# mlee03/FRE-NCtools

Hardware: AMD Instinct MI355X
Metric: exchange-cells/s (higher is better)
Workload: dtype f64; 1 GPU; C384 cubed sphere (6 tiles) -> 1440x720 lat-lon, conservative_order2: exchange-grid search + centroid pass + CSR build per step; nxgrid=4160000, parallelism=1 latitude band(s) of the target, one per GPU, world_size=1

## Files before the change

### fre-nctools_amd/_lib.py

```python
import ctypes as C
import os

_HERE = os.path.dirname(os.path.abspath(__file__))
_LIB = None


class FregridHipError(RuntimeError):
    def __init__(self, code, msg):
        super().__init__(f"libfregrid_hip error {code}: {msg}")
        self.code = code


def lib_path():
    return os.environ.get("FREGRID_HIP_LIB") or os.path.join(_HERE, "libfregrid_hip.so")


EXPORTS = [
    "get_maxxgrid", "get_grid_area", "create_xgrid_2dx2d_order1", "create_xgrid_2dx2d_order2", "conserve_interp",
    "clip_2dx2d", "poly_area", "poly_ctrlon", "poly_ctrlat", "fix_lon", "pimod",
    "fg_clip_2dx2d_batch", "fg_poly_op_batch",
    "get_maxxgrid_", "get_grid_area_", "create_xgrid_2dx2d_order1_", "create_xgrid_2dx2d_order2_",
    "fg_last_error", "fg_device_count", "fg_plan_create", "fg_plan_create_dev", "fg_plan_create_empty",
    "fg_plan_destroy", "fg_plan_set_stream", "fg_pool_release", "fg_plan_nxgrid", "fg_plan_ncells_in",
    "fg_plan_cell_sums_dev", "fg_plan_copy_cell_sums", "fg_plan_accumulate_cell_sums", "fg_plan_accumulate_cell_sums_async", "fg_dev_gather_f64", "fg_dev_scatter_f64", "fg_plan_finalize", "fg_plan_get_xgrid", "fg_plan_get_polygons", "fg_plan_create_polylist", "fg_plan_get_cell_struct",
    "fg_plan_get_cell_area", "fg_plan_set_xgrid", "fg_plan_apply", "fg_plan_apply_interleaved", "fg_plan_apply_records", "fg_plan_apply_levels", "fg_plan_apply_records_levels", "fg_plan_levels_capacity", "fg_plan_apply_levels_ex", "fg_plan_apply_records_levels_ex", "fg_plan_levels_ex_capacity", "fg_plan_apply_ex", "fg_plan_mono_begin",
    "fg_plan_mono_minmax_dev", "fg_plan_mono_copy_minmax", "fg_plan_mono_end",
    "fg_plan_apply_levels_mono", "fg_plan_mono_levels_begin", "fg_plan_mono_levels_copy_minmax", "fg_plan_mono_levels_end",
    "fg_plan_apply_records_levels_mono", "fg_plan_mono_records_reset", "fg_plan_mono_records_begin", "fg_plan_mono_records_copy_minmax",
    "fg_plan_mono_records_end", "fg_c2l_records_levels_mono", "fg_sweep_run_levels_mono",
    "fg_plan_create_great_circle", "fg_plan_create_great_circle_dev", "fg_latlon2xyz", "create_xgrid_great_circle",
    "create_xgrid_great_circle_", "get_grid_great_circle_area", "get_grid_great_circle_area_", "clip_2dx2d_great_circle",
    "great_circle_area", "fg_gc_clip_batch", "conserve_interp_great_circle", "fg_sincos_batch",
    "create_xgrid_1dx2d_order1", "create_xgrid_1dx2d_order2", "create_xgrid_2dx1d_order1", "create_xgrid_2dx1d_order2",
    "create_xgrid_1dx2d_order1_", "create_xgrid_1dx2d_order2_", "create_xgrid_2dx1d_order1_", "create_xgrid_2dx1d_order2_",
    "clip", "box_ctrlat", "box_ctrlon", "get_grid_area_no_adjust", "get_grid_area_no_adjust_", "fg_plan_stream", "fg_plan_sync",
    "fg_c2l_create", "fg_c2l_destroy", "fg_c2l_ncells", "fg_c2l_halo_size", "fg_c2l_set_stream", "fg_c2l_sync",
    "fg_c2l_get_centres", "fg_c2l_fill_halo", "fg_c2l_gradient", "fg_c2l_gradient_records", "fg_c2l_records", "fg_c2l_records_levels", "fg_c2l_grid_info", "fg_find_contacts", "fg_halo_map",
    "fg_gnomonic_ed_grid", "fg_tripolar_corners", "fg_remap_write", "fg_remap_write_interp", "fg_remap_read_size", "fg_remap_read", "fg_remap_last_error",
    "fg_plan_trim", "fg_plan_ncells_out", "fg_plan_order", "fg_plan_device", "fg_dev_alloc", "fg_dev_free", "fg_dev_upload", "fg_dev_download",
    "fg_nc_open", "fg_nc_create", "fg_nc_def_dim", "fg_nc_def_var", "fg_nc_put_att_text", "fg_nc_put_att_double", "fg_nc_enddef",
    "fg_nc_inq_ndims", "fg_nc_inq_nvars", "fg_nc_inq_numrecs", "fg_nc_inq_dimid", "fg_nc_inq_dim", "fg_nc_inq_varid", "fg_nc_inq_var",
    "fg_nc_get_att_double", "fg_nc_get_att_text", "fg_nc_get_vara", "fg_nc_get_vara_double", "fg_nc_put_vara", "fg_nc_put_vara_double",
    "fg_nc_close", "fg_nc_last_error", "fg_dev_widen", "fg_dev_narrow", "fg_sweep_create", "fg_sweep_run", "fg_sweep_run_levels", "fg_sweep_run_levels_ex", "fg_sweep_destroy", "fg_host_alloc", "fg_host_free",
    "fg_plan_stats", "fg_set_search_mode", "fg_set_search_cull", "fg_set_search_finalize", "fg_set_search_async", "fg_set_search_rect", "fg_set_search_wide_cap", "fg_set_search_frame", "fg_set_apply_xcd", "fg_set_apply_vec", "fg_set_apply_ep", "fg_set_gc_split", "fg_set_profiling", "fg_plan_phase_ms", "fg_gnomonic_ed_corners", "fg_latlon_corners",
    "fg_bilin_create", "fg_bilin_create_from_weights", "fg_bilin_destroy", "fg_bilin_get_index_weight", "fg_bilin_npoints_fine",
    "fg_bilin_nlon_fine", "fg_bilin_nlat_fine", "fg_bilin_nlon", "fg_bilin_nlat", "fg_bilin_ncells", "fg_bilin_set_stream",
    "fg_bilin_sync", "fg_bilin_apply_scalar", "fg_bilin_apply_vector", "fg_bilin_remap_write", "fg_bilin_remap_read",
    "fg_unit_vect_latlon", "fg_bilin_fine_grid", "fg_bilin_ambiguous_ties",
    "fg_bilin_sweep_create", "fg_bilin_sweep_run_scalar", "fg_bilin_sweep_run_vector", "fg_bilin_sweep_destroy",
    "fg_extrap_create", "fg_extrap_destroy", "fg_extrap_set_stream", "fg_extrap_stream", "fg_extrap_run_dev", "fg_extrap_run",
    "fg_extrap_last_syncs", "fg_extrap_get_coef", "fg_extrap_coef_host", "fg_set_extrap_batch", "fg_set_extrap_coef",
    "fg_setup_vertical_interp", "fg_dev_vertical_interp",
    "fg_extrap_run_batch_dev", "fg_column_create", "fg_column_run", "fg_column_destroy", "fg_set_column_records",
    "fg_dev_latlon2xyz", "fg_plan_create_great_circle_lonlat", "fg_plan_create_great_circle_lonlat_dev",
    "fg_plan_create_polylist_gc",
    "fg_runoff_create", "fg_runoff_create_from_xgrid", "fg_runoff_destroy", "fg_runoff_nxgrid", "fg_runoff_get_xgrid",
    "fg_runoff_get_maps", "fg_runoff_get_xyz", "fg_runoff_search_stats", "fg_runoff_phase_ms", "fg_runoff_stream", "fg_runoff_apply", "fg_runoff_apply_dev",
    "fg_nearest_unmasked", "fg_set_runoff_prune", "fg_runoff_tile",
    "fg_rland_create", "fg_rland_destroy", "fg_rland_stream", "fg_rland_search", "fg_rland_search_sface", "fg_rland_stats",
    "fg_rland_phase_ms", "fg_set_rland_prune", "fg_rland_tile",
    "fg_river_create", "fg_river_destroy", "fg_river_stream", "fg_river_run", "fg_river_get", "fg_river_get_max_suba",
    "fg_river_stats", "fg_river_phase_ms", "fg_set_river_prune", "fg_river_qsort_index",
    "fg_topog_default_opts", "fg_topog_create", "fg_topog_destroy", "fg_topog_stream", "fg_topog_set_source", "fg_topog_get_source",
    "fg_topog_remap", "fg_topog_filter", "fg_topog_process", "fg_topog_run", "fg_topog_set_depth", "fg_topog_get", "fg_topog_stats",
    "fg_topog_phase_ms", "fg_plan_apply_frac_dev", "fg_set_topog_sweep",
    "fg_coupler_create", "fg_coupler_create_gc", "fg_coupler_destroy", "fg_coupler_stream", "fg_coupler_run", "fg_coupler_count", "fg_coupler_get",
    "fg_coupler_get_cells", "fg_coupler_write", "fg_coupler_write_xgrid", "fg_coupler_write_mask", "fg_coupler_stats", "fg_coupler_phase_ms",
]


class TopogOpts(C.Structure):
    _fields_ = [("scale_factor", C.c_double)] + \
        [(k, C.c_int) for k in ("tripolar_grid", "cyclic_x", "cyclic_y", "fill_first_row", "filter_topog", "num_filter_pass",
                                "smooth_topo_allow_deepening", "round_shallow", "fill_shallow", "deepen_shallow", "full_cell", "flat_bottom",
                                "adjust_topo", "fill_isolated_cells", "dont_change_landmask", "kmt_min")] + \
        [("min_thickness", C.c_double), ("open_very_this_cell", C.c_int), ("fraction_full_cell", C.c_double),
         ("use_great_circle_algorithm", C.c_int), ("on_grid", C.c_int)]


class FieldConv(C.Structure):
    _fields_ = [("scale", C.c_double), ("offset", C.c_double), ("missing", C.c_double)]


class ApplyOpts(C.Structure):
    _fields_ = [("has_missing", C.c_int), ("missing", C.c_double), ("weight", C.c_void_p),
                ("cell_methods_sum", C.c_int), ("field_area", C.c_void_p), ("area_missing", C.c_double),
                ("cell_area_in", C.c_void_p), ("cell_area_out", C.c_void_p), ("monotonic", C.c_int)]


def lib():
    global _LIB
    if _LIB is not None:
        return _LIB
    path = lib_path()
    if not os.path.exists(path):
        raise ImportError(
            f"{path} not found: build the HIP extension first (make -C fre-nctools_amd/csrc, or "
            "python -c 'import __graft_entry__ as g; g.build()').  There is no CPU fallback.")
    try:
        import torch
    except ImportError:
        pass
    L = C.CDLL(path)
    dp, ip, vp = C.POINTER(C.c_double), C.POINTER(C.c_int), C.c_void_p
    dpp = C.POINTER(dp)
    cip = C.POINTER(C.c_int)

    L.get_maxxgrid.restype = C.c_int
    L.get_grid_area.argtypes = [cip, cip, dp, dp, dp]
    L.get_grid_area.restype = None
    L.create_xgrid_2dx2d_order1.argtypes = [cip] * 4 + [dp] * 5 + [ip] * 4 + [dp]
    L.create_xgrid_2dx2d_order1.restype = C.c_int
    L.create_xgrid_2dx2d_order2.argtypes = [cip] * 4 + [dp] * 5 + [ip] * 4 + [dp] * 3
    L.create_xgrid_2dx2d_order2.restype = C.c_int
    L.conserve_interp.argtypes = [C.c_int] * 4 + [dp] * 7
    L.conserve_interp.restype = None

    L.clip_2dx2d.argtypes = [dp, dp, C.c_int, dp, dp, C.c_int, dp, dp]
    L.clip_2dx2d.restype = C.c_int
    L.poly_area.argtypes = [dp, dp, C.c_int]
    L.poly_area.restype = C.c_double
    L.poly_ctrlon.argtypes = [dp, dp, C.c_int, C.c_double]
    L.poly_ctrlon.restype = C.c_double
    L.poly_ctrlat.argtypes = [dp, dp, C.c_int]
    L.poly_ctrlat.restype = C.c_double
    L.fix_lon.argtypes = [dp, dp, C.c_int, C.c_double]
    L.fix_lon.restype = C.c_int
# ... 470 lines not shown
```

### fre-nctools_amd/conserve_interp.py

```python
import ctypes as C
from dataclasses import dataclass, field
from typing import List, Optional

import numpy as np

from . import _lib
from ._lib import lib, check

CONSERVE_ORDER1 = 1
CONSERVE_ORDER2 = 2
TARGET = 16
READ = 256
WRITE = 512
CHECK_CONSERVE = 1024
LEGACY_CLIP = 2048
GREAT_CIRCLE = 4096
MONOTONIC = 16384
CELL_METHODS_MEAN = 0
CELL_METHODS_SUM = 1
MAXVAL = 1.0e20


def _f64(a):
    return np.ascontiguousarray(a, dtype=np.float64)
# ... 111 lines not shown
                                                              (lon_out_t, lat_out_t), mean_dlat, mean_dlon, device, stream), C.byref(h)))
        return cls(h.value, order, device)

    @classmethod
    def create_great_circle(cls, grids_in, grid_out, masks=None, device=0):
        _lib.require_gpu()
        args, keep = _host_grid_args(grids_in, grid_out, masks)
        h = C.c_void_p()
        check(lib().fg_plan_create_great_circle(*args, device, C.byref(h)))
        return cls(h.value, 1, device, True)

    @classmethod
    def create_great_circle_dev(cls, nx_in, ny_in, xyz_in_t, nx_out, ny_out, xyz_out_t, mean_dlat=0.0, mean_dlon=0.0,
                                device=0, stream=None, masks_t=None):
        h = C.c_void_p()
        tables = [[t[k] for t in xyz_in_t] for k in range(3)]
        check(lib().fg_plan_create_great_circle_dev(*_dev_grid_args(nx_in, ny_in, tables, masks_t, nx_out, ny_out, [xyz_out_t[k] for k in range(3)],
                                                                    mean_dlat, mean_dlon, device, stream), C.byref(h)))
        return cls(h.value, 1, device, True)

    @classmethod
    def create_great_circle_lonlat(cls, grids_in, grid_out, masks=None, device=0):
        _lib.require_gpu()
        args, keep = _host_grid_args(grids_in, grid_out, masks)
        h = C.c_void_p()
        check(lib().fg_plan_create_great_circle_lonlat(*args, device, C.byref(h)))
        return cls(h.value, 1, device, True)

    @classmethod
    def create_great_circle_lonlat_dev(cls, nx_in, ny_in, lon_in_t, lat_in_t, nx_out, ny_out, lon_out_t, lat_out_t,
                                       mean_dlat=0.0, mean_dlon=0.0, device=0, stream=None, masks_t=None):
        h = C.c_void_p()
        check(lib().fg_plan_create_great_circle_lonlat_dev(*_dev_grid_args(nx_in, ny_in, (lon_in_t, lat_in_t), masks_t, nx_out, ny_out,
                                                                           (lon_out_t, lat_out_t), mean_dlat, mean_dlon, device, stream),
                                                           C.byref(h)))
        return cls(h.value, 1, device, True)

    @classmethod
    def create_empty(cls, order, nx_in, ny_in, nx_out, ny_out, device=0):
        _lib.require_gpu()
        nt = len(nx_in)
        h = C.c_void_p()
        check(lib().fg_plan_create_empty(order, nt, (C.c_int * nt)(*nx_in), (C.c_int * nt)(*ny_in),
                                         nx_out, ny_out, device, C.byref(h)))
        return cls(h.value, order, device)

    def destroy(self):
        if self._h is not None and self._h.value:
            lib().fg_plan_destroy(self._h)
        self._h = None

    def __del__(self):
        try:
            self.destroy()
        except Exception:
            pass

    @property
    def nxgrid(self):
        return int(lib().fg_plan_nxgrid(self._h))

    @property
    def ncells_in(self):
        return int(lib().fg_plan_ncells_in(self._h))

    def cell_sums_ptr(self):
        return lib().fg_plan_cell_sums_dev(self._h)

    def copy_cell_sums(self, dst_t):
        check(lib().fg_plan_copy_cell_sums(self._h, C.c_void_p(dst_t.data_ptr())))

    def accumulate_cell_sums(self, total_t, cells_t=None):
        args = (self._h, C.c_void_p(total_t.data_ptr()), C.c_void_p(cells_t.data_ptr()) if cells_t is not None else None,
                int(cells_t.numel()) if cells_t is not None else 0)
        if getattr(total_t, "is_cuda", False):
            cur = _torch().cuda.current_stream(total_t.device)
            if int(self.stream() or 0) == int(cur.cuda_stream):
                check(lib().fg_plan_accumulate_cell_sums_async(*args))
                return
            cur.synchronize()
        check(lib().fg_plan_accumulate_cell_sums(*args))

    def stats(self):
        s = (C.c_long * 11)()
        check(lib().fg_plan_stats(self._h, s, 11))
        names = ["pairs", "nonempty", "nxgrid", "borderline", "bins", "bin_entries", "deferred", "heavy", "below", "exact_mode", "rare"]
        return dict(zip(names, [int(v) for v in s]))

    PHASES = ["cell_struct", "bins", "candidates", "clip_quad", "clip_general", "compact", "rows",
              "search_total", "finalize", "apply"]

    def phase_ms(self):
        ms = (C.c_float * 10)()
        check(lib().fg_plan_phase_ms(self._h, ms, 10))
        return dict(zip(self.PHASES, [float(v) for v in ms]))

    def finalize(self, total_sums_ptr=None):
        check(lib().fg_plan_finalize(self._h, C.c_void_p(total_sums_ptr or 0)))

    def sync(self):
        check(lib().fg_plan_sync(self._h))

    def stream(self):
        return lib().fg_plan_stream(self._h)

    def set_stream(self, stream):
        check(lib().fg_plan_set_stream(self._h, C.c_void_p(int(stream))))

    def get_xgrid(self):
        n = self.nxgrid
        ints = {k: np.empty(n, dtype=np.int32) for k in ("t_in", "i_in", "j_in", "i_out", "j_out")}
        area = np.empty(n, dtype=np.float64)
        c1 = np.empty(n, dtype=np.float64) if self.order == 2 else None
        c2 = np.empty(n, dtype=np.float64) if self.order == 2 else None
        check(lib().fg_plan_get_xgrid(self._h, _ip(ints["t_in"]), _ip(ints["i_in"]), _ip(ints["j_in"]),
                                      _ip(ints["i_out"]), _ip(ints["j_out"]), _dp(area), _dp(c1), _dp(c2)))
        out = dict(ints)
        out["area"] = area
        if self.order == 2:
            out["c1"], out["c2"] = c1, c2
        return out

    def get_polygons(self, maxv=16):
        nx = self.nxgrid
        n = np.zeros(nx, dtype=np.int32)
        v = [np.zeros((nx, maxv)) for _ in range(3)]
        check(lib().fg_plan_get_polygons(self._h, maxv, _ip(n), _dp(v[0]), _dp(v[1]), _dp(v[2])))
        if self.great_circle:
            return {"n": n, "x": v[0], "y": v[1], "z": v[2]}
        return {"n": n, "lon": v[0], "lat": v[1]}

    @classmethod
    def create_polylist(cls, order, n, lon, lat, lon_avg, area_ref, grid_out, device=0):
        _lib.require_gpu()
        n = np.ascontiguousarray(n, dtype=np.int32)
        lon, lat = _f64(lon), _f64(lat)
        assert lon.shape == (n.size, 8) == lat.shape
        lon_avg, area_ref = _f64(lon_avg), _f64(area_ref)
        lo, la = _f64(grid_out.lonc).reshape(-1), _f64(grid_out.latc).reshape(-1)
        h = C.c_void_p()
        check(lib().fg_plan_create_polylist(order, n.size, _ip(n), _dp(lon), _dp(lat), _dp(lon_avg), _dp(area_ref), grid_out.nx, grid_out.ny,
                                            _dp(lo), _dp(la), device, C.byref(h)))
        return cls(h.value, order, device)

    @classmethod
    def create_polylist_gc(cls, n, x, y, z, area_ref, grid_out, device=0):
        _lib.require_gpu()
        n = np.ascontiguousarray(n, dtype=np.int32)
        x, y, z = (_f64(v).reshape(n.size, 8) for v in (x, y, z))
        area_ref = _f64(area_ref).reshape(n.size)
        lo, la = _f64(grid_out.lonc).reshape(-1), _f64(grid_out.latc).reshape(-1)
        h = C.c_void_p()
        check(lib().fg_plan_create_polylist_gc(n.size, _ip(n), _dp(x), _dp(y), _dp(z), _dp(area_ref), grid_out.nx, grid_out.ny,
                                               _dp(lo), _dp(la), device, C.byref(h)))
        return cls(h.value, 1, device, True)

    @classmethod
    def create_polylist_gc_dev(cls, n_t, x_t, y_t, z_t, area_ref_t, nx_out, ny_out, xyz_out_t, mean_dlat=0.0, mean_dlon=0.0,
                               device=0, stream=None):
        h = C.c_void_p()
        ptr = lambda t: C.c_void_p(t.data_ptr())
        check(lib().fg_plan_create_polylist_gc_dev(int(n_t.numel()), ptr(n_t), ptr(x_t), ptr(y_t), ptr(z_t), ptr(area_ref_t), nx_out, ny_out,
                                                   ptr(xyz_out_t[0]), ptr(xyz_out_t[1]), ptr(xyz_out_t[2]), mean_dlat, mean_dlon, device,
                                                   C.c_void_p(int(stream or 0)), 0 if stream is None else 1, C.byref(h)))
        return cls(h.value, 1, device, True)

    def get_cell_area(self, ncells_out):
        a_in = np.empty(self.ncells_in, dtype=np.float64)
        a_out = np.empty(ncells_out, dtype=np.float64)
# ... 438 lines not shown
```

### fre-nctools_amd/csrc/geom.hip.h

```cpp
#pragma once
#include <hip/hip_runtime.h>

#define G_PI      3.14159265358979323846
#define G_TPI     (2.0 * G_PI)
#define G_HPI     (0.5 * G_PI)
#define G_RADIUS  6371000.0
#define G_SMALL   1.e-10
#define G_POLETOL 1.e-6
#define G_MAXV    8
#define G_FIXCAP  12

#define G_ERRBIT_MAXV     1u
#define G_ERRBIT_PARALLEL 2u
#define G_ERRBIT_OVERFLOW 4u
#define G_ERRBIT_BADLAT   8u

#include "sincos_glibc.h"
__device__ __forceinline__ double d_sin_lat(double x) { return fgs_sin(x); }
__device__ __forceinline__ double d_cos_lat(double x) { return fgs_cos(x); }
__device__ __forceinline__ void d_sincos_lat(double x, double *s, double *c) { fgs_sincos(x, s, c); }

__device__ __forceinline__ bool d_is_pole(double lat) { return fabs(lat) >= G_HPI - G_POLETOL; }

__device__ inline int d_fix_lon(double *x, double *y, int n, double tlon)
// ... 1 lines not shown
  int nn = n;
  for (int i = 0; i < nn; i++) {
    if (!d_is_pole(y[i])) continue;
    int im = (i + nn - 1) % nn, ip = (i + 1) % nn;
    if (y[im] == y[i] && y[ip] == y[i]) {
      for (int k = i; k < nn - 1; k++) { x[k] = x[k + 1]; y[k] = y[k + 1]; }
      nn--; i--;
    } else if (y[im] != y[i] && y[ip] != y[i]) {
      if (nn + 1 > G_FIXCAP) return -1;
      for (int k = nn - 1; k >= i; k--) { x[k + 1] = x[k]; y[k + 1] = y[k]; }
      nn++; i++;
    }
  }
  for (int i = 0; i < nn; i++) {
    if (!d_is_pole(y[i])) continue;
    int im = (i + nn - 1) % nn, ip = (i + 1) % nn;
    if (y[im] != y[i]) x[i] = x[im];
    if (y[ip] != y[i]) x[i] = x[ip];
  }
  for (int i = 0; i < nn; i++) {
    int im = (i + nn - 1) % nn;
    double dx = x[i] - x[im];
    if (fabs(dx + G_PI) < G_SMALL || fabs(dx - G_PI) < G_SMALL) {
      if (nn + 2 > G_FIXCAP) return -1;
      double xa = x[im], xb = x[i];
      double ypole = G_HPI;
      if (y[i] < 0.0) ypole = -G_HPI;
      for (int k = nn - 1; k >= i; k--) { x[k + 2] = x[k]; y[k + 2] = y[k]; }
      x[i] = xa; y[i] = ypole;
      x[i + 1] = xb; y[i + 1] = ypole;
      nn += 2;
      break;
    }
  }
  if (!nn) return 0;
  double x_sum = x[0];
  for (int i = 1; i < nn; i++) {
    double dx = x[i] - x[i - 1];
    if (dx < -G_PI)     dx = dx + G_TPI;
    else if (dx > G_PI) dx = dx - G_TPI;
    x_sum += (x[i] = x[i - 1] + dx);
  }
  double d = (x_sum / nn) - tlon;
  if (d < -G_PI)     for (int i = 0; i < nn; i++) x[i] += G_TPI;
  else if (d > G_PI) for (int i = 0; i < nn; i++) x[i] -= G_TPI;
  return nn;
}

__device__ __forceinline__ int d_fix_lon_quad_fast(double *x, const double *y, double tlon)
{
  if (d_is_pole(y[0]) || d_is_pole(y[1]) || d_is_pole(y[2]) || d_is_pole(y[3])) return -1;
  {
    const double d0 = x[0] - x[3], d1 = x[1] - x[0], d2 = x[2] - x[1], d3 = x[3] - x[2];
    if (fabs(d0 + G_PI) < G_SMALL || fabs(d0 - G_PI) < G_SMALL || fabs(d1 + G_PI) < G_SMALL || fabs(d1 - G_PI) < G_SMALL ||
        fabs(d2 + G_PI) < G_SMALL || fabs(d2 - G_PI) < G_SMALL || fabs(d3 + G_PI) < G_SMALL || fabs(d3 - G_PI) < G_SMALL) return -1;
  }
  double x_sum = x[0];
#pragma unroll
  for (int i = 1; i < 4; i++) {
    double dx = x[i] - x[i - 1];
    if (dx < -G_PI)     dx = dx + G_TPI;
    else if (dx > G_PI) dx = dx - G_TPI;
    x_sum += (x[i] = x[i - 1] + dx);
  }
  const double d = (x_sum / 4) - tlon;
  if (d < -G_PI)     { x[0] += G_TPI; x[1] += G_TPI; x[2] += G_TPI; x[3] += G_TPI; }
  else if (d > G_PI) { x[0] -= G_TPI; x[1] -= G_TPI; x[2] -= G_TPI; x[3] -= G_TPI; }
  return 4;
}

__device__ __forceinline__ int d_inside_edge(double x0, double y0, double x1, double y1, double x, double y)
{
  double product = (x - x0) * (y1 - y0) + (x0 - x1) * (y - y0);
  return (product <= 1.e-12) ? 1 : 0;
}

__device__ __forceinline__ double d_pimod1(double v)
{
  if (v < -G_PI)     v += G_TPI;
  else if (v > G_PI) v -= G_TPI;
  return v;
}

template <int S>
__device__ inline double d_poly_area(const double *x, const double *y, int n)
{
  double area = 0.0;
  for (int i = 0; i < n; i++) {
    int ip = (i + 1 == n) ? 0 : i + 1;
    double dx = (x[ip * S] - x[i * S]);
    double lat1 = y[ip * S], lat2 = y[i * S];
    if (dx > G_PI)  dx = dx - 2.0 * G_PI;
    if (dx < -G_PI) dx = dx + 2.0 * G_PI;
    if (fabs(dx + G_PI) < G_SMALL || fabs(dx - G_PI) < G_SMALL) { area += G_PI; continue; }
    if (fabs(lat1 - lat2) < G_SMALL)
      area -= dx * d_sin_lat(0.5 * (lat1 + lat2));
    else {
      double dy = 0.5 * (lat1 - lat2);
      double dat = d_sin_lat(dy) / dy;
      area -= dx * d_sin_lat(0.5 * (lat1 + lat2)) * dat;
    }
  }
  if (area < 0) return -area * G_RADIUS * G_RADIUS;
  return area * G_RADIUS * G_RADIUS;
}

template <int S>
__device__ inline double d_poly_ctrlat(const double *x, const double *y, int n)
{
  double ctrlat = 0.0;
  for (int i = 0; i < n; i++) {
    int ip = (i + 1 == n) ? 0 : i + 1;
    double dx = (x[ip * S] - x[i * S]);
    double lat1 = y[ip * S], lat2 = y[i * S];
    double dy = lat2 - lat1;
    double hdy = dy * 0.5;
    double avg_y = (lat1 + lat2) * 0.5;
    if (dx == 0.0) continue;
    if (dx > G_PI)   dx = dx - 2.0 * G_PI;
    if (dx <= -G_PI) dx = dx + 2.0 * G_PI;
    const double cl1 = d_cos_lat(lat1);
    if (fabs(hdy) < G_SMALL)
      ctrlat -= dx * (2 * d_cos_lat(avg_y) + lat2 * d_sin_lat(avg_y) - cl1);
    else {
      double sa, ca;
      d_sincos_lat(avg_y, &sa, &ca);
      ctrlat -= dx * ((d_sin_lat(hdy) / hdy) * (2 * ca + lat2 * sa) - cl1);
    }
  }
  return (ctrlat * G_RADIUS * G_RADIUS);
}

template <int S>
__device__ inline double d_poly_ctrlon(const double *x, const double *y, int n, double clon)
{
  double ctrlon = 0.0;
  for (int i = 0; i < n; i++) {
    int ip = (i + 1 == n) ? 0 : i + 1;
    double phi1 = x[ip * S], phi2 = x[i * S];
    double lat1 = y[ip * S], lat2 = y[i * S];
    double dphi = phi1 - phi2;
    if (dphi == 0.0) continue;
    double sl1, cl1, sl2, cl2;
    d_sincos_lat(lat1, &sl1, &cl1);
    d_sincos_lat(lat2, &sl2, &cl2);
    double f1 = 0.5 * (cl1 * sl1 + lat1);
    double f2 = 0.5 * (cl2 * sl2 + lat2);
    if (dphi > G_PI)  dphi = dphi - 2.0 * G_PI;
    if (dphi < -G_PI) dphi = dphi + 2.0 * G_PI;
    double dphi1 = phi1 - clon;
    if (dphi1 > G_PI)  dphi1 -= 2.0 * G_PI;
    if (dphi1 < -G_PI) dphi1 += 2.0 * G_PI;
    double dphi2 = phi2 - clon;
    if (dphi2 > G_PI)  dphi2 -= 2.0 * G_PI;
    if (dphi2 < -G_PI) dphi2 += 2.0 * G_PI;
    if (fabs(dphi2 - dphi1) < G_PI) {
      ctrlon -= dphi * (dphi1 * f1 + dphi2 * f2) / 2.0;
    } else {
      double fac = (dphi1 > 0.0) ? G_PI : -G_PI;
      double fint = f1 + (f2 - f1) * (fac - dphi1) / fabs(dphi);
      ctrlon -= 0.5 * dphi1 * (dphi1 - fac) * f1 - 0.5 * dphi2 * (dphi2 + fac) * f2
                + 0.5 * fac * (dphi1 + dphi2) * fint;
    }
  }
  return (ctrlon * G_RADIUS * G_RADIUS);
}

__device__ __forceinline__ double d_dphi_clon(double phi, double clon)
{
  double d = phi - clon;
  if (d > G_PI)  d -= 2.0 * G_PI;
  if (d < -G_PI) d += 2.0 * G_PI;
  return d;
}

template <int S>
__device__ inline void d_poly_area_ctr(const double *x, const double *y, int n, double clon,
                                       double *area_out, double *ctrlon_out, double *ctrlat_out)
{
  double area = 0.0, ctrlat = 0.0, ctrlon = 0.0;
  double s0, c0, cp_first;
  fgs_trig<FGS_COS_F | FGS_SIN_N | FGS_COS_N>(y[0], nullptr, &cp_first, &s0, &c0);
  const double f_first = 0.5 * (c0 * s0 + y[0]), dphi_first = d_dphi_clon(x[0], clon);
  double f2 = f_first, dphi2 = dphi_first;
  for (int i = 0; i < n; i++) {
    const bool last = (i + 1 == n);
    int ip = last ? 0 : i + 1;
    double phi1 = x[ip * S], phi2 = x[i * S];
    double lat1 = y[ip * S], lat2 = y[i * S];
    double f1, dphi1, cp1;
    if (last) { f1 = f_first; dphi1 = dphi_first; cp1 = cp_first; }
    else {
      double s1, c1;
      fgs_trig<FGS_COS_F | FGS_SIN_N | FGS_COS_N>(lat1, nullptr, &cp1, &s1, &c1);
      f1 = 0.5 * (c1 * s1 + lat1);
      dphi1 = d_dphi_clon(phi1, clon);
    }
    double dx0 = phi1 - phi2;
    double avg_y = (lat1 + lat2) * 0.5;
    double savg, cavg, sa, ca;
    fgs_trig<FGS_ALL>(avg_y, &savg, &cavg, &sa, &ca);
    double dyh = 0.5 * (lat1 - lat2);
    bool flat = fabs(lat1 - lat2) < G_SMALL;
    double dat = flat ? 1.0 : d_sin_lat(dyh) / dyh;

    {
      double dx = dx0;
      if (dx > G_PI)  dx = dx - 2.0 * G_PI;
      if (dx < -G_PI) dx = dx + 2.0 * G_PI;
      if (fabs(dx + G_PI) < G_SMALL || fabs(dx - G_PI) < G_SMALL) area += G_PI;
      else area -= dx * savg * dat;
    }
    if (dx0 != 0.0) {
      double dx = dx0;
      if (dx > G_PI)   dx = dx - 2.0 * G_PI;
      if (dx <= -G_PI) dx = dx + 2.0 * G_PI;
      double hdy = (lat2 - lat1) * 0.5;
      const double t = (fabs(hdy) < G_SMALL) ? (2 * cavg + lat2 * savg) : dat * (2 * ca + lat2 * sa);
      ctrlat -= dx * (t - cp1);
    }
    if (dx0 != 0.0) {
      double dphi = dx0;
      if (dphi > G_PI)  dphi = dphi - 2.0 * G_PI;
      if (dphi < -G_PI) dphi = dphi + 2.0 * G_PI;
      if (fabs(dphi2 - dphi1) < G_PI) {
        ctrlon -= dphi * (dphi1 * f1 + dphi2 * f2) / 2.0;
      } else {
        double fac = (dphi1 > 0.0) ? G_PI : -G_PI;
        double fint = f1 + (f2 - f1) * (fac - dphi1) / fabs(dphi);
        ctrlon -= 0.5 * dphi1 * (dphi1 - fac) * f1 - 0.5 * dphi2 * (dphi2 + fac) * f2
                  + 0.5 * fac * (dphi1 + dphi2) * fint;
      }
    }
    f2 = f1; dphi2 = dphi1;
  }
  *area_out = (area < 0) ? -area * G_RADIUS * G_RADIUS : area * G_RADIUS * G_RADIUS;
  *ctrlat_out = ctrlat * G_RADIUS * G_RADIUS;
  *ctrlon_out = ctrlon * G_RADIUS * G_RADIUS;
}
```

### fre-nctools_amd/csrc/plan.hip

```cpp
#include <hip/hip_runtime.h>
#include <math.h>
#include <stdio.h>
#include <stdlib.h>
#include <string.h>
#include <algorithm>
#include <map>
#include <mutex>
#include <string>
#include <type_traits>
#include <vector>
#include "fg_host.h"
#include "plan_internal.h"
#include "xgrid_device.h"

static thread_local std::string g_err;
extern "C" const char *fg_last_error(void) { return g_err.c_str(); }
void fg_set_last_error(const char *msg) { g_err = msg ? msg : ""; }

extern "C" int fg_device_count(void)
{
  int n = 0;
  hipError_t e = hipGetDeviceCount(&n);
  if (e != hipSuccess) { fg_fail(FG_ERR_HIP, "hipGetDeviceCount: %s", hipGetErrorString(e)); return FG_ERR_HIP; }
  return n;
// ... 381 lines not shown
  c->lon_avg = pl->alloc<double>(n); c->area = pl->alloc<double>(n);
  c->nv = pl->alloc<int>(n);
  c->verts = pl->alloc<double>(n * (compact ? FG_VSTRIDE_QUAD : 16));
  if (compact) {
    const size_t cap = n / 16 + 64;
    c->vstride = FG_VSTRIDE_QUAD;
    c->wide_cap = (int)(g_wide_cap >= 0 ? std::min<size_t>((size_t)g_wide_cap, cap) : cap);
    c->wide = pl->alloc<double>(16 * (size_t)std::max(c->wide_cap, 1));
    if (!c->wide) return false;
  }
  return c->lat_min && c->lat_max && (compact || (c->lon_min && c->lon_max)) && c->lon_avg && c->area && c->nv && c->verts;
}

static int plan_base(int order, int ntiles_in, const int *nx_in, const int *ny_in, int nx_out, int ny_out,
                     int device, fg_plan **out)
{
  if (order != FG_CONSERVE_ORDER1 && order != FG_CONSERVE_ORDER2) return fg_fail(FG_ERR_ARG, "order must be 1 or 2");
  if (ntiles_in < 1 || !nx_in || !ny_in || nx_out < 1 || ny_out < 1 || !out) return fg_fail(FG_ERR_ARG, "bad grid sizes");
  if (int rc = fg_use_device("fg_plan", device)) return rc;
  fg_plan *pl = new fg_plan();
  pl->order = order; pl->device = device; pl->ntiles = ntiles_in;
  long off = 0, foff = 0;
  for (int m = 0; m < ntiles_in; m++) {
    if (nx_in[m] < 1 || ny_in[m] < 1) { delete pl; return fg_fail(FG_ERR_ARG, "bad source tile size"); }
    pl->nx_in.push_back(nx_in[m]); pl->ny_in.push_back(ny_in[m]); pl->cell_off.push_back((int)off);
    off += (long)nx_in[m] * ny_in[m];
    foff += (order == 2) ? (long)(nx_in[m] + 2) * (ny_in[m] + 2) : (long)nx_in[m] * ny_in[m];
  }
  if (off > 2000000000L || (long)nx_out * ny_out > 2000000000L) { delete pl; return fg_fail(FG_ERR_ARG, "grid too large for 32-bit cell indices"); }
  pl->nsrc = (int)off; pl->f_stride = foff;
  pl->nx_out = nx_out; pl->ny_out = ny_out; pl->ndst = nx_out * ny_out;
  pl->stream = g_handles.get_stream(device);
  if (!pl->stream) { delete pl; return fg_fail(FG_ERR_HIP, "hipStreamCreate failed"); }
  *out = pl;
  return 0;
}

extern "C" void fg_plan_destroy(fg_plan *pl)
{
  if (!pl) return;
  (void)hipSetDevice(pl->device);
  const bool drain = !pl->async || !pl->apply_pt.spans.empty();
  if (drain && (pl->stream || !pl->own_stream)) (void)hipStreamSynchronize(pl->stream);
  if (pl->stream_b) { if (drain) (void)hipStreamSynchronize(pl->stream_b); g_handles.put_stream(pl->device, pl->stream_b); }
  { float junk[PH_COUNT] = {0}; pl->apply_pt.collect(junk); }
  if (pl->async) g_pool.put(pl->owned, pl->stream, !pl->own_stream);
  else for (void *p : pl->owned) g_pool.put(p);
  if (pl->stream && pl->own_stream) g_handles.put_stream(pl->device, pl->stream);
  delete pl;
}

static void choose_bins(const fg_plan *pl, double mean_dlat, double mean_dlon, FgBins *b)
{
  const double PI = 3.14159265358979323846;
  double h = 1.25 * mean_dlat, w = 1.25 * mean_dlon;
  int nblat = (h > 0) ? (int)ceil(PI / h) : 1;
  int nblon = (w > 0) ? (int)ceil(2.0 * PI / w) : 1;
  if (nblat < 1) nblat = 1; if (nblat > 8192) nblat = 8192;
  if (nblon < 1) nblon = 1; if (nblon > 16384) nblon = 16384;
  (void)pl;
  b->nblat = nblat; b->nblon = nblon;
  b->inv_wlat = nblat / PI;
  b->inv_wlon = nblon / (2.0 * PI);
}

struct PinnedCounters { FgCounters c; unsigned long long mark; };
static FgCounters *pinned_counters()
{
  static thread_local PinnedCounters *h = nullptr;
  if (!h) { if (hipHostMalloc((void **)&h, sizeof(PinnedCounters), hipHostMallocCoherent) != hipSuccess) h = nullptr; else h->mark = 0; }
  return h ? &h->c : nullptr;
}

struct GcXyz { const double *x, *y, *z; };
struct BoxMode { FgBox box; const double *mask_quad; int no_adjust; };
struct SearchIn {
  const double *const *lon_in = nullptr, *const *lat_in = nullptr, *const *mask_in = nullptr;
  const double *lon_out = nullptr, *lat_out = nullptr;
  const GcXyz *gc_in = nullptr, *gc_out = nullptr;
  const BoxMode *boxm = nullptr;
  double mean_dlat = 0, mean_dlon = 0;
  int rect_hint = 1;
};
struct SearchOpts { bool exact, cull, finalize, rect, dst_frame; int gc_split; bool profile, async; };
__global__ __launch_bounds__(64) void k_counters_out(const unsigned *src, unsigned *dst, int nwords, unsigned long long *mark, unsigned long long seq)
{
  for (int k = threadIdx.x; k < nwords; k += 64) dst[k] = src[k];
  __threadfence_system();
  __syncthreads();
  if (threadIdx.x == 0) __hip_atomic_store(mark, seq, __ATOMIC_RELEASE, __HIP_MEMORY_SCOPE_SYSTEM);
}
static_assert(sizeof(FgCounters) % sizeof(unsigned) == 0 && offsetof(PinnedCounters, mark) == sizeof(FgCounters), "FgCounters travels as 32-bit words, the mark behind them");
static hipError_t wait_counters(const FgCounters *hc, unsigned long long seq, hipStream_t st)
{
  const unsigned long long *mark = &((const PinnedCounters *)hc)->mark;
  for (unsigned spin = 1;; spin++) {
    if (__atomic_load_n(mark, __ATOMIC_ACQUIRE) == seq) return hipSuccess;
    __builtin_ia32_pause();
    if (spin % 65536 == 0) {
      const hipError_t e = hipStreamQuery(st);
      if (e == hipErrorNotReady) (void)hipGetLastError();
      if (e == hipSuccess) return __atomic_load_n(mark, __ATOMIC_ACQUIRE) == seq ? hipSuccess : hipErrorUnknown;
      if (e != hipErrorNotReady) return e;
    }
  }
}
static const char *gc_clip_error(int code)
{
  switch (code) {
    case 3: return "firstIntersect is not in the grid1List";
    case 4: return " not found the next intersection ";
    case 5: return "not return back to the first intersection";
    case 6: return "After clipping, nintersect should be 0";
    case 7: return "inserAfter: point (x,y,z) is not found in the list";
    case 8: return "Error from create_xgrid.c: temp is not in list1";
    case 11: return "clip_2dx2d_great_circle: insertIntersect finds no node that is not an intersection (the reference's loop over "
                    "the list, mosaic_util.c:1352, does not end on this pair of cells)";
    default: return "clip_2dx2d_great_circle: more intersections than two convex polygons can have (the list capacity of the device "
                    "clip, not a check of the reference)";
  }
}

static int g_search_cull = 0;
static int g_search_finalize = 0;
static int g_gc_split = 1;
extern "C" void fg_set_gc_split(int on) { g_gc_split = on < 0 ? 0 : on; }
struct SearchCaps { unsigned long long entries; int regcap, nreg; bool rect; };
static int g_search_rect = 1;
extern "C" void fg_set_search_rect(int on) { g_search_rect = on ? 1 : 0; }
static int g_dst_frame = 0;
extern "C" void fg_set_search_frame(int coupler) { g_dst_frame = coupler ? 1 : 0; }
static thread_local int tl_dst_frame = -1;
static bool host_says_not_rect(int nx, int ny, const double *lon, const double *lat)
{
  const long nxp = nx + 1;
  const int js[3] = {ny, ny / 2, 1}, is[3] = {nx, nx / 2, 1};
  for (int a = 0; a < 3; a++)
    for (int b = 0; b < 3; b++) {
      const long e = (long)js[a] * nxp + is[b];
      if (memcmp(&lon[e], &lon[is[b]], sizeof(double)) || memcmp(&lat[e], &lat[(long)js[a] * nxp], sizeof(double))) return true;
    }
  return false;
}
#define FG_RETRY (-1000L)
struct Carve {
  size_t n = 0;
  size_t operator()(size_t size) { const size_t at = n; n += size; return at; }
};
struct SearchBlocks {
  fg_plan *pl;
  bool ok = true;
  std::vector<void *> scratch;
  template <typename T> T *keep(size_t count) { T *p = pl->alloc<T>(count); ok = ok && p; return p; }
  template <typename T> T *get(size_t count) { T *p = keep<T>(count); if (p) scratch.push_back(p); return p; }
  void release() { for (void *p : scratch) pl->release(p); scratch.clear(); }
};
static long plan_search_core(fg_plan *pl, const SearchIn &in, const SearchOpts &opt, SearchCaps *caps)
{
  const bool gc = in.gc_in != nullptr;
  const BoxMode *const boxm = in.boxm;
  pl->great_circle = gc;
  hipStream_t st = pl->stream;
  const int nsrc = pl->nsrc, ndst = pl->ndst, order = pl->order;
  FgCounters *hc = pinned_counters();
  if (!hc) return fg_fail(FG_ERR_HIP, "hipHostMalloc failed");

  std::vector<FgTile> &th = pl->tiles_host;
  th.resize(pl->ntiles + 1);
  for (int m = 0; m < pl->ntiles; m++) th[m] = FgTile{gc ? nullptr : in.lon_in[m], gc ? nullptr : in.lat_in[m], pl->nx_in[m], pl->ny_in[m], pl->cell_off[m]};
  th[pl->ntiles] = FgTile{in.lon_out, in.lat_out, pl->nx_out, pl->ny_out, 0};
  pl->tiles_dev = pl->alloc<FgTile>(pl->ntiles + 1);
  if (!pl->tiles_dev) return fg_fail(FG_ERR_HIP, "out of device memory");
  FgTileSet ts; ts.n = 0;
  const bool by_value = !gc && pl->ntiles + 1 <= FG_TILESET_MAX;
  if (by_value) { ts.n = pl->ntiles + 1; for (int m = 0; m <= pl->ntiles; m++) ts.t[m] = th[m]; }
  else FGCHK(hipMemcpyAsync(pl->tiles_dev, th.data(), sizeof(FgTile) * th.size(), hipMemcpyHostToDevice, st));
  FgTileXyz *gct_dev = nullptr;
  std::vector<FgTileXyz> gct;
  if (gc) {
    gct.resize(pl->ntiles + 1);
    for (int m = 0; m < pl->ntiles; m++) gct[m] = FgTileXyz{in.gc_in[m].x, in.gc_in[m].y, in.gc_in[m].z, pl->nx_in[m], pl->ny_in[m], pl->cell_off[m]};
    gct[pl->ntiles] = FgTileXyz{in.gc_out->x, in.gc_out->y, in.gc_out->z, pl->nx_out, pl->ny_out, 0};
    gct_dev = pl->alloc<FgTileXyz>(pl->ntiles + 1);
    if (!gct_dev) return fg_fail(FG_ERR_HIP, "out of device memory");
    FGCHK(hipMemcpyAsync(gct_dev, gct.data(), sizeof(FgTileXyz) * gct.size(), hipMemcpyHostToDevice, st));
  }

  bool any_mask = false;
  if (in.mask_in) for (int m = 0; m < pl->ntiles; m++) if (in.mask_in[m]) any_mask = true;
  if (any_mask) {
    pl->mask_dev = pl->alloc<double>(nsrc);
    if (!pl->mask_dev) return fg_fail(FG_ERR_HIP, "out of device memory");
    std::vector<double> ones;
    for (int m = 0; m < pl->ntiles; m++) {
      size_t nc = (size_t)pl->nx_in[m] * pl->ny_in[m];
      if (in.mask_in[m]) FGCHK(hipMemcpyAsync(pl->mask_dev + pl->cell_off[m], in.mask_in[m], nc * sizeof(double), hipMemcpyDeviceToDevice, st));
      else {
        ones.assign(nc, 1.0);
        FGCHK(hipMemcpyAsync(pl->mask_dev + pl->cell_off[m], ones.data(), nc * sizeof(double), hipMemcpyHostToDevice, st));
        FGCHK(hipStreamSynchronize(st));
      }
    }
  }

  const bool rect = caps->rect && !gc && !boxm;
  pl->rect = rect;
  const double dst_tlon = opt.dst_frame ? (double)NAN : 3.14159265358979323846;
  FgBins bins;
  choose_bins(pl, in.mean_dlat, in.mean_dlon, &bins);
  if (rect) { bins.nblat = 0; bins.nblon = 0; }
  const long nbins = (long)bins.nblat * bins.nblon;
  const long nslots = nbins + bins.nblat;
  const unsigned long long nentries = rect ? 0ull : caps->entries;
  const int ecap = (int)std::min<unsigned long long>(nentries, 2147483647ull);
  FgPairSpace ps{};
  ps.nreg = caps->nreg; ps.regcap = caps->regcap;
  const long npairs = fgd_pairs_total(ps);
  const long nx_alloc = npairs;

  if (!alloc_cells(pl, &pl->S, nsrc, rect && !pl->polys.npoly)) return fg_fail(FG_ERR_HIP, "out of device memory");
  SearchBlocks blk{pl};
  const bool gc_poly = gc && pl->gcpolys.npoly > 0;
  if (gc_poly) pl->gc_prec = blk.keep<double>((size_t)nsrc * FG_GC_PREC);
  struct { double *hdr, *lat_ax, *lon_ax, *col, *row, *col_min, *col_max, *col_avg; } rt{};
  if (rect) {
    pl->D = FgCells{};
    pl->D.area = blk.keep<double>(ndst);
    Carve at;
    const size_t o_hdr = at(8), o_lat = at((size_t)pl->ny_out + 1), o_lon = at((size_t)pl->nx_out + 1), o_col = at(8 * (size_t)pl->nx_out),
                 o_row = at(4 * ((size_t)pl->ny_out + 1)), o_cmin = at((size_t)pl->nx_out), o_cmax = at((size_t)pl->nx_out), o_cavg = at((size_t)pl->nx_out);
    double *rect_blk = blk.keep<double>(at.n);
    if (!blk.ok) return fg_fail(FG_ERR_HIP, "out of device memory");
    rt = {rect_blk + o_hdr, rect_blk + o_lat, rect_blk + o_lon, rect_blk + o_col, rect_blk + o_row, rect_blk + o_cmin, rect_blk + o_cmax, rect_blk + o_cavg};
  } else if (!alloc_cells(pl, &pl->D, ndst)) return fg_fail(FG_ERR_HIP, "out of device memory");
  const long t_bins = fgd_scan_tiles(nslots), t_rows = fgd_scan_tiles(ndst), t_comp = fgd_scan_tiles(nsrc);
  const size_t zreg = (size_t)FG_NREG * FG_FILL_STRIDE * sizeof(unsigned);
  Carve z;
  const size_t z_dc = z((sizeof(FgCounters) + 127) / 128 * 128), z_fill = z(zreg), z_tick = z(128);
  const size_t z_lb_bins = z(t_bins * sizeof(unsigned long long)), z_lb_rows = z(t_rows * sizeof(unsigned long long)),
               z_lb_comp = z(t_comp * sizeof(unsigned long long));
  const size_t z_bin_cnt = z((size_t)(nslots + 1) * sizeof(int)), z_bin_fill = z((size_t)(nslots + 1) * sizeof(int)),
               z_row_cnt = z((size_t)(ndst + 1) * sizeof(int)), z_nacc = z((size_t)(nsrc + 1) * sizeof(int));
  z((16 - (z.n - z_bin_cnt) % 16) % 16);
  const size_t z_gc_ntask = z(gc ? zreg : 0), z_gc_ocnt = z(gc ? zreg : 0);
  const size_t zbytes = z.n;
  char *zero_blk = blk.get<char>(zbytes);
  int *bin_start = blk.get<int>(nslots + 1);
  int *heavy_list = blk.get<int>(nsrc + 1);
  int *rare_list = blk.get<int>(rect ? nsrc + 1 : 1);
  int *big_list = blk.get<int>(nsrc + 1);
  int *pair_beg = blk.get<int>(nsrc + 1), *pair_cnt = blk.get<int>(nsrc + 1);
  FgBinEntry *bin_entries = blk.get<FgBinEntry>(nentries ? nentries : 1);
  ps.src = blk.get<int>(npairs + 1); ps.dst = blk.get<int>(npairs + 1);
  double *tmp_area = blk.get<double>(npairs + 1);
  double *tmp_clon = (order == 2) ? blk.get<double>(npairs + 1) : nullptr;
  double *tmp_clat = (order == 2) ? blk.get<double>(npairs + 1) : nullptr;
  int *defer_list = blk.get<int>(npairs + 1);
  const bool early_rows = !gc && !boxm;
  int *tmp_rowpos = early_rows ? blk.get<int>(npairs + 1) : nullptr;
  const bool gc_split = gc && !gc_poly && opt.gc_split && npairs < (1L << 28);
  const long tcap_want = (opt.gc_split == 2) ? npairs / 64 : 3 * npairs;
  const long tcap_reg = gc_split ? std::min<long>((tcap_want / FG_NREG + 255) / 256 * 256, 0x7ffffff0L / FG_NREG) : 0;
  const long tcap_all = tcap_reg * FG_NREG;
  unsigned *gc_meta = gc_split ? blk.get<unsigned>(npairs + 1) : nullptr;
  int *gc_tbase = gc_split ? blk.get<int>(npairs + 1) : nullptr;
  int *gc_order = gc_split ? blk.get<int>(npairs + 1) : nullptr;
  unsigned *gc_task = gc_split ? blk.get<unsigned>(tcap_all + 1) : nullptr;
  double *gc_res = gc_split ? blk.get<double>(2 * (size_t)tcap_all + 2) : nullptr;
  pl->xoff = blk.keep<int>(nsrc + 1);
  pl->x_src = blk.keep<int>(nx_alloc + 1); pl->x_dst = blk.keep<int>(nx_alloc + 1);
  pl->x_area = blk.keep<double>(nx_alloc + 1);
  if (order == 2) { pl->x_c1 = blk.keep<double>(nx_alloc + 1); pl->x_c2 = blk.keep<double>(nx_alloc + 1); pl->sums = blk.keep<double>(3 * (size_t)nsrc); }
  int *x_rowpos = blk.get<int>(nx_alloc + 1);
  pl->perm = blk.keep<FgRowEnt>(nx_alloc + 1);
  pl->csr.row_ptr = blk.keep<int>(ndst + 1);
  if (!pl->src_idx_f) pl->src_idx_f = blk.keep<int>(nsrc + 1);
  if (!blk.ok) return fg_fail(FG_ERR_HIP, "out of device memory");
  FgCounters *dc = (FgCounters *)(zero_blk + z_dc);
  ps.fill = (unsigned *)(zero_blk + z_fill);
  unsigned *tickets = (unsigned *)(zero_blk + z_tick);
  unsigned long long *lb_bins = (unsigned long long *)(zero_blk + z_lb_bins), *lb_rows = (unsigned long long *)(zero_blk + z_lb_rows),
                     *lb_comp = (unsigned long long *)(zero_blk + z_lb_comp);
  int *bin_cnt = (int *)(zero_blk + z_bin_cnt), *bin_fill = (int *)(zero_blk + z_bin_fill), *row_cnt = (int *)(zero_blk + z_row_cnt);
  int *nacc = (int *)(zero_blk + z_nacc);
  FGCHK(hipMemsetAsync(zero_blk, 0, zbytes, st));
  if (pl->ll_err) FGCHK(hipMemcpyAsync(&dc->err[2], pl->ll_err, sizeof(unsigned), hipMemcpyDeviceToDevice, st));

  PhaseTimer pt, ptot;
  pt.start(opt.profile, st); ptot.start(opt.profile, st);
  for (int k = 0; k < PH_COUNT; k++) pl->phase_ms[k] = 0;
  ptot.begin(PH_SEARCH_TOTAL);
  pt.begin(PH_CELL_STRUCT);
  if (gc) {
    fgd_gc_cell_struct(gct_dev + pl->ntiles, 1, ndst, pl->D, st, opt.cull ? dc->band_keys : nullptr, 1);
    if (gc_poly) fgd_gc_poly_records(pl->gcpolys, pl->S, pl->gc_prec, dc->err, st);
    else fgd_gc_cell_struct(gct_dev, pl->ntiles, nsrc, pl->S, st, opt.cull ? dc->band_keys : nullptr, 2);
    fgd_src_field_index(order, pl->tiles_dev, pl->ntiles, nsrc, pl->src_idx_f, st);
  } else if (rect) {
    FgRect &R = pl->rect_tab;
    R.hdr = rt.hdr; R.lat_ax = rt.lat_ax; R.lon_ax = rt.lon_ax; R.col = rt.col; R.row = rt.row;
    R.col_min = rt.col_min; R.col_max = rt.col_max; R.col_avg = rt.col_avg;
    R.bad = &dc->rect_bad; R.nx = pl->nx_out; R.ny = pl->ny_out;
    fgd_rect_tables(in.lon_out, in.lat_out, pl->nx_out, pl->ny_out, rt.hdr, rt.lat_ax, rt.lon_ax, rt.col, rt.col_min, rt.col_max, rt.col_avg, rt.row,
                    &dc->rect_bad, dc->err, st, dst_tlon);
    if (pl->polys.npoly) fgd_polylist_records(pl->polys, pl->S, pl->src_idx_f, pl->sums, &R, heavy_list, &dc->heavy_cnt, dc->err, st);
    fgd_cell_struct2r(ts, pl->tiles_dev, pl->tiles_dev, pl->ntiles, pl->polys.npoly ? 0 : nsrc, ndst, pl->S, pl->D.area, R, pl->mask_dev, order,
                      pl->src_idx_f, pl->sums, dc->err, st, dc->band_keys, (opt.cull && !pl->polys.npoly) ? 2 : 0, heavy_list, &dc->heavy_cnt,
                      rare_list, &dc->rare_cnt, ps, pair_beg, pair_cnt, big_list, &dc->big_cnt);
  } else if (opt.cull && !boxm && !pl->polys.npoly) {
    fgd_band_keys(in.lat_out, (long)(pl->nx_out + 1) * (pl->ny_out + 1), dc->band_keys, st);
    fgd_cell_struct2(ts, pl->tiles_dev, pl->tiles_dev, pl->ntiles, nsrc, ndst, pl->S, pl->D, bins, bin_cnt, order, pl->src_idx_f, pl->sums, dc->err, st, dc->band_keys, 2, dst_tlon);
  } else if (pl->polys.npoly) {
    fgd_polylist_records(pl->polys, pl->S, pl->src_idx_f, pl->sums, nullptr, nullptr, nullptr, dc->err, st);
    fgd_cell_struct2(ts, pl->tiles_dev, pl->tiles_dev, pl->ntiles, 0, ndst, pl->S, pl->D, bins, bin_cnt, order, pl->src_idx_f, pl->sums, dc->err, st, nullptr, 0, dst_tlon);
  } else
    fgd_cell_struct2(ts, pl->tiles_dev, pl->tiles_dev, pl->ntiles, nsrc, ndst, pl->S, pl->D, bins, bin_cnt, order, pl->src_idx_f, pl->sums, dc->err, st, nullptr, 0, dst_tlon);
  if (boxm) fgd_box_cell_boxes(boxm->box, pl->S, st);
  if (boxm && boxm->no_adjust) fgd_box_area_no_adjust(boxm->box, pl->S.area, st);
  pt.end();
  pl->have_geom = true;

  if (!rect) {
    pt.begin(PH_BINS);
    if (gc) fgd_bin_count(ndst, pl->D, bins, bin_cnt, st);
    fgd_exclusive_scan1(bin_cnt, nslots, bin_start, lb_bins, &tickets[0], &dc->total[0], dc->err, st);
    fgd_bin_fill(ndst, pl->D, bins, bin_fill, bin_start, bin_entries, ecap, nsrc, pl->S, pl->mask_dev, heavy_list, &dc->heavy_cnt, st);
    pt.end();
  }

  pt.begin(PH_CANDIDATES);
  if (rect)
    fgd_candidates_rect(nsrc, pl->S, pl->mask_dev, pl->rect_tab, ps, pair_beg, pair_cnt, heavy_list, &dc->heavy_cnt, big_list, &dc->big_cnt, st,
                        pl->polys.npoly ? 0 : 1,
                        rare_list, &dc->rare_cnt, dc->err, pl->polys.npoly ? nullptr : pl->sums);
  else
    fgd_candidates1(nsrc, pl->S, pl->mask_dev, bins, bin_start, bin_entries, ecap, ps, pair_beg, pair_cnt, heavy_list, &dc->heavy_cnt, big_list,
                    &dc->big_cnt, st);
  pt.end();
  hipEvent_t gc_e1 = nullptr, gc_e2 = nullptr;
  struct EvReturn {
    hipEvent_t &a, &b;
    ~EvReturn() { g_handles.put_sync_event(a); g_handles.put_sync_event(b); a = b = nullptr; }
  } ev_return{gc_e1, gc_e2};
  if (boxm) {
    pt.begin(PH_CLIP_GENERAL);
    fgd_clip_box(order, ps, boxm->box, th[pl->ntiles], pl->S, pl->D, pl->mask_dev, boxm->mask_quad, tmp_area, tmp_clon, tmp_clat, nacc, dc->stats, dc->err, st);
    pt.end();
  } else if (gc) {
    pt.begin(PH_CLIP_GENERAL);
    if (gc_poly)
      fgd_gc_clip_poly(ps, pl->S, pl->gc_prec, pl->D, tmp_area, nacc, dc->stats, dc->err, st);
    else if (gc_split) {
      if (!pl->stream_b) pl->stream_b = g_handles.get_stream(pl->device);
      gc_e1 = g_handles.get_sync_event(); gc_e2 = g_handles.get_sync_event();
      GcSplit g{gc_meta, gc_tbase, gc_task, gc_res, (unsigned)tcap_reg, (unsigned *)(zero_blk + z_gc_ntask), defer_list, &dc->defer_cnt,
                &dc->gc_list2_cnt, npairs, gc_order, (unsigned *)(zero_blk + z_gc_ocnt)};
      fgd_gc_clip_split(ps, pl->S, pl->mask_dev, pl->D, tmp_area, nacc, g, dc->stats, dc->err, st, pl->stream_b, gc_e1, gc_e2);
    } else
      fgd_gc_clip(ps, pl->S, pl->mask_dev, pl->D, tmp_area, nacc, defer_list, &dc->defer_cnt, dc->stats, dc->err, st);
    pt.end();
  } else {
    pt.begin(PH_CLIP_QUAD);
    fgd_clip_quad(order, ps, pl->S, pl->mask_dev, pl->D, tmp_area, tmp_clon, tmp_clat, nacc, defer_list, &dc->defer_cnt, dc->stats, dc->err, st,
                  rect ? &pl->rect_tab : nullptr, row_cnt, tmp_rowpos);
    pt.end();
    pt.begin(PH_CLIP_GENERAL);
    fgd_clip_general(order, ps, pl->S, pl->mask_dev, pl->D, tmp_area, tmp_clon, tmp_clat, nacc, defer_list, &dc->defer_cnt, dc->stats, dc->err, st,
                     rect ? &pl->rect_tab : nullptr, row_cnt, tmp_rowpos);
    pt.end();
  }
  pt.begin(PH_COMPACT);
  FgCompactIo io{};
  io.pair_beg = pair_beg; io.pair_cnt = pair_cnt;
  io.tmp_area = tmp_area; io.tmp_clon = tmp_clon; io.tmp_clat = tmp_clat;
  io.xoff = pl->xoff; io.x_src = pl->x_src; io.x_dst = pl->x_dst; io.x_area = pl->x_area; io.x_c1 = pl->x_c1; io.x_c2 = pl->x_c2;
  io.row_cnt = row_cnt; io.x_rowpos = x_rowpos; io.sums = pl->sums; io.big_list = big_list; io.big_cnt = &dc->big_cnt;
  io.tmp_rowpos = tmp_rowpos; io.row_ptr = pl->csr.row_ptr; io.perm = pl->perm;
  io.dc = dc; io.xcap = nx_alloc;
  if (early_rows)
    fgd_exclusive_scan2(nacc, nsrc, pl->xoff, lb_comp, &tickets[2], &dc->xtot, row_cnt, ndst, pl->csr.row_ptr, lb_rows, &tickets[1], &dc->rows_total, dc->err, st);
  else
    fgd_exclusive_scan1(nacc, nsrc, pl->xoff, lb_comp, &tickets[2], &dc->xtot, dc->err, st);
  fgd_compact(order, nsrc, ps, io, st);
  pt.end();
  if (!early_rows) {
    pt.begin(PH_ROWS);
    fgd_exclusive_scan1(row_cnt, ndst, pl->csr.row_ptr, lb_rows, &tickets[1], &dc->rows_total, dc->err, st);
    fgd_csr_fill_pos(nx_alloc, &dc->xtot, pl->x_src, pl->x_dst, pl->csr.row_ptr, x_rowpos, pl->perm, st);
    pt.end();
  }
  ptot.end();
  const bool fuse = opt.finalize && early_rows && !pl->polys.npoly;
  const bool stream_ordered = fuse && opt.async && !opt.profile;
  static thread_local unsigned long long rb_seq = 0;
  int *fused_tmp = nullptr;
  if (fuse) {
    if (order == 2) { pl->cen = pl->alloc<FgSrcRec>((size_t)nsrc + 1); pl->csr.e2 = pl->alloc<FgCsrEntry2>(nx_alloc + 1); }
    else pl->csr.e1 = pl->alloc<FgCsrEntry1>(nx_alloc + 1);
    if ((order == 2 && !pl->cen) || (!pl->csr.e1 && !pl->csr.e2)) return fg_fail(FG_ERR_HIP, "out of device memory");
    fused_tmp = pl->alloc<int>(3 * (size_t)(nx_alloc + 1));
  }
  if (stream_ordered) {
    unsigned *hc_dev = nullptr;
    if (hipHostGetDevicePointer((void **)&hc_dev, hc, 0) != hipSuccess || !hc_dev) return fg_fail(FG_ERR_HIP, "the counters' host block is not mapped");
    const int nwords = (int)(sizeof(FgCounters) / sizeof(unsigned));
    k_counters_out<<<1, 64, 0, st>>>((const unsigned *)dc, hc_dev, nwords, (unsigned long long *)(hc_dev + nwords), ++rb_seq);
    FGCHK(hipGetLastError());
  }
  if (fuse) {
    pt.begin(PH_FINALIZE);
    if (order == 2) fgd_centroids(nsrc, pl->S, pl->sums, pl->cen, st);
    fgd_csr_sortgather(order, ndst, (long)nsrc + ndst, pl->perm, pl->x_area, pl->x_c1, pl->x_c2, pl->src_idx_f,
                       order == 2 ? pl->cen : nullptr, pl->csr, st, fused_tmp, nx_alloc + 1);
    pt.end();
  }
  if (stream_ordered) {
    if (hipError_t e = hipGetLastError()) {
      (void)hipStreamSynchronize(st);
      return fg_fail(FG_ERR_HIP, "a launch of the search failed: %s", hipGetErrorString(e));
    }
    FGCHK(wait_counters(hc, rb_seq, st));
  } else {
    FGCHK(hipMemcpyAsync(hc, dc, sizeof(FgCounters), hipMemcpyDeviceToHost, st));
    FGCHK(hipStreamSynchronize(st));
  }
  pt.collect(pl->phase_ms); ptot.collect(pl->phase_ms);
  FGCHK(hipGetLastError());
  if (rect && hc->rect_bad) { caps->rect = false; return FG_RETRY; }
  if (rect && (hc->err[0] & G_ERRBIT_WIDECAP)) { caps->rect = false; return FG_RETRY; }
  if (hc->total[0] > nentries) { caps->entries = hc->total[0]; return FG_RETRY; }
  if (hc->total[0] > 2000000000ull) return fg_fail(FG_ERR_ARG, "bin table too large");
  if (hc->total[3] > (unsigned long long)ps.regcap) {
    if (hc->total[3] > 2000000000ull / (unsigned long long)ps.nreg) return fg_fail(FG_ERR_CAPACITY, "candidate pair list exceeds 2^31 entries");
    caps->regcap = (int)((hc->total[3] + FG_REG_ALIGN - 1) / FG_REG_ALIGN * FG_REG_ALIGN);
    return FG_RETRY;
  }
  if (hc->err[2] & G_ERRBIT_LL2X) return fg_fail(FG_ERR_ARG, "latlon2xyz: a grid corner is not finite, or its latitude (|lat| >= 2.4262) or longitude "
                                                          "(|lon| > 1024) lies outside the range of the device trig (radians expected)");
  if (hc->err[0] & 8u) return fg_fail(FG_ERR_ARG, "a grid corner latitude lies outside [-pi/2, pi/2] (radians expected)");
  if (hc->err[0] & 1u) return fg_fail(FG_ERR_MAXV, "create_xgrid.c: n2_in is greater than MAX_V");
  if (hc->err[0] & 2u) return fg_fail(FG_ERR_PARALLEL, "the line between <x1_0,y1_0> and  <x1_1,y1_1> should not parallel to "
                                                    "the line between <x2_0,y2_0> and  <x2_1,y2_1>");
  if (hc->err[0] & 4u) return fg_fail(FG_ERR_MAXV, "clipped polygon exceeds 16 vertices");
  if (hc->err[0] & G_ERRBIT_GC_CONVEX1) return fg_fail(FG_ERR_GEOM, "create_xgrid.c(clip_2dx2d_great_circle): grid box 1 is not convex");
  if (hc->err[0] & G_ERRBIT_GC_CONVEX2) return fg_fail(FG_ERR_GEOM, "create_xgrid.c(clip_2dx2d_great_circle): grid box 2 is not convex");
  if (hc->err[0] & G_ERRBIT_GC_POLYN) return fg_fail(FG_ERR_MAXV, "a polygon of the list has more than 8 vertices");
  if (hc->err[0] & G_ERRBIT_GC_CLIP) return fg_fail(FG_ERR_GEOM, "%s", gc_clip_error((int)hc->err[1]));
  if (hc->err[0] & G_ERRBIT_LOOKBACK) return fg_fail(FG_ERR_HIP, "single-pass scan: a tile waited too long for its predecessor");
  pl->nx = (long)hc->xtot;
  pl->stats[FG_STAT_PAIRS] = (long)hc->total[1];
  pl->stats[FG_STAT_NONEMPTY] = (long)(hc->xtot + hc->stats[FG_STAT_BELOW]);
  pl->stats[FG_STAT_NXGRID] = pl->nx;
  pl->stats[FG_STAT_BORDERLINE] = (long)hc->stats[FG_STAT_BORDERLINE];
  pl->stats[FG_STAT_BINS] = nbins;
  pl->stats[FG_STAT_BIN_ENTRIES] = (long)hc->total[0];
  pl->stats[FG_STAT_DEFERRED] = hc->defer_cnt + hc->gc_list2_cnt;
  pl->stats[FG_STAT_HEAVY] = hc->heavy_cnt;
  pl->stats[FG_STAT_RARE] = hc->rare_cnt;
  pl->stats[FG_STAT_BELOW] = (long)hc->stats[FG_STAT_BELOW];

  pl->rect_tab.bad = nullptr;
  if (stream_ordered) {
    blk.scratch.push_back(pl->perm); blk.scratch.push_back(fused_tmp);
    pl->release_on_stream(blk.scratch); blk.scratch.clear();
    pl->perm = nullptr; fused_tmp = nullptr;
  }
  blk.release();
  pl->rows_built = true;
  pl->searched = true;
  if (fuse) {
    pl->release(pl->perm); pl->perm = nullptr; pl->release(fused_tmp);
    if (!pl->red_partial) { pl->red_partial = pl->alloc<double>(1024); pl->red_result = pl->alloc<double>(260); }
    if (!pl->red_partial || !pl->red_result) return fg_fail(FG_ERR_HIP, "out of device memory");
    pl->dist_pending = (order == 2);
    pl->finalized = true; pl->fused = true;
  }
  return pl->nx;
}

static int g_search_exact = 0;
extern "C" void fg_set_search_mode(int exact) { g_search_exact = exact; }
extern "C" void fg_set_search_cull(int on) { g_search_cull = on ? 1 : 0; }
extern "C" void fg_set_search_finalize(int on) { g_search_finalize = on ? 1 : 0; }
static int g_search_async = 1;
extern "C" void fg_set_search_async(int on) { g_search_async = on ? 1 : 0; }
static long plan_search(fg_plan *pl, const SearchIn &in)
{
  static const bool env_exact = getenv("FREGRID_HIP_EXACT_SEARCH") && atoi(getenv("FREGRID_HIP_EXACT_SEARCH")) != 0;
  const SearchOpts opt{.exact = g_search_exact || env_exact, .cull = g_search_cull != 0, .finalize = g_search_finalize != 0,
                       .rect = g_search_rect != 0, .dst_frame = (tl_dst_frame >= 0 ? tl_dst_frame : g_dst_frame) != 0, .gc_split = g_gc_split, .profile = g_profiling != 0, .async = g_search_async != 0};
  const long big = std::max((long)pl->nsrc, (long)pl->ndst);
  if (big > (1L << 28)) return fg_fail(FG_ERR_CAPACITY, "grid of %ld cells: more than 2^28 cells per search are not supported", big);
  SearchCaps caps;
  caps.entries = opt.exact ? 0ull : 3ull * (unsigned long long)pl->ndst + 4096ull;
  const unsigned long long cap_pairs = std::min<unsigned long long>(8ull * (unsigned long long)big + 65536ull, 2000000000ull);
  caps.nreg = (int)std::max(1L, std::min((long)FG_NREG, ((long)pl->nsrc + 1023) / 1024));
  caps.regcap = opt.exact ? 0 : (int)((cap_pairs / caps.nreg + FG_REG_ALIGN - 1) / FG_REG_ALIGN * FG_REG_ALIGN);
  caps.rect = opt.rect && in.rect_hint && !in.gc_in && !in.boxm && pl->nx_out <= 8192 && pl->nx_out >= 2;
  const size_t keep = pl->owned.size();
  long rc = FG_RETRY;
  int attempts = 0;
  pl->async = opt.async;
  pl->on_stream = pl->async;
  for (; attempts < 4 && rc == FG_RETRY; attempts++) {
    if (attempts) {
      (void)hipStreamSynchronize(pl->stream);
      pl->drop_search(keep);
    }
    rc = plan_search_core(pl, in, opt, &caps);
  }
  pl->on_stream = false;
  if (rc == FG_RETRY) return fg_fail(FG_ERR_CAPACITY, "exchange-grid search: capacities did not settle");
  if (rc >= 0) pl->stats[FG_STAT_EXACT] = (attempts > 1) ? 1 : 0;
  pl->search_d2h = (long)attempts * (long)sizeof(FgCounters);
  return rc;
}

struct CornerSample {
  int nsamp = 0;
  std::vector<double> q;
  const double *corners(int a, int k) const { return &q[((size_t)a * nsamp + k) * 4]; }
};
static long sample_step(int nx, int ny, int *nsamp)
{
  const long ncell = (long)nx * ny;
  long step = ncell / 4096; if (step < 1) step = 1;
  *nsamp = (int)((ncell + step - 1) / step);
  return step;
}
__host__ __device__ static inline void sample_nodes(int nx, long step, int k, long n[4])
{
  const long c = (long)k * step;
  const int i = (int)(c % nx), j = (int)(c / nx);
  n[0] = (long)j * (nx + 1) + i; n[1] = n[0] + 1; n[3] = n[0] + nx + 1; n[2] = n[3] + 1;
}
static CornerSample sample_corners_host(int nx, int ny, int narr, const double *const *arr)
{
  CornerSample s;
  const long step = sample_step(nx, ny, &s.nsamp);
  s.q.resize((size_t)s.nsamp * narr * 4);
  for (int k = 0; k < s.nsamp; k++) {
    long n[4];
    sample_nodes(nx, step, k, n);
    for (int a = 0; a < narr; a++)
      for (int v = 0; v < 4; v++) s.q[((size_t)a * s.nsamp + k) * 4 + v] = arr[a][n[v]];
  }
  return s;
}
__global__ void k_sample_corners(int nx, long step, int nsamp, int narr, const double *a0, const double *a1, const double *a2, double *out)
{
  const int k = blockIdx.x * blockDim.x + threadIdx.x;
  if (k >= nsamp) return;
  long n[4];
  sample_nodes(nx, step, k, n);
  const double *arr[3] = {a0, a1, a2};
  for (int a = 0; a < narr; a++) {
    double *o = out + ((size_t)a * nsamp + k) * 4;
    o[0] = arr[a][n[0]]; o[1] = arr[a][n[1]]; o[2] = arr[a][n[2]]; o[3] = arr[a][n[3]];
  }
}
static int sample_corners_dev(fg_plan *pl, int nx, int ny, int narr, const double *d_a0, const double *d_a1, const double *d_a2, CornerSample *s)
{
  const long step = sample_step(nx, ny, &s->nsamp);
  s->q.resize((size_t)s->nsamp * narr * 4);
  double *d_q = (double *)g_pool.get(pl->device, s->q.size() * sizeof(double));
  if (!d_q) return fg_fail(FG_ERR_HIP, "out of device memory");
  k_sample_corners<<<(s->nsamp + 255) / 256, 256, 0, pl->stream>>>(nx, step, s->nsamp, narr, d_a0, d_a1, d_a2, d_q);
  hipError_t e = hipMemcpyAsync(s->q.data(), d_q, s->q.size() * sizeof(double), hipMemcpyDeviceToHost, pl->stream);
  if (e == hipSuccess) e = hipStreamSynchronize(pl->stream);
  g_pool.put(d_q);
  if (e != hipSuccess) return fg_fail(FG_ERR_HIP, "sampling the destination corners failed: %s", hipGetErrorString(e));
  return 0;
}
// ... 1773 lines not shown
static int plan_apply_frac(fg_plan *pl, const double *data, double *out)
{
  fgd_apply_frac(pl->ndst, pl->csr, data, out, pl->stream);
  FGCHK(hipStreamSynchronize(pl->stream));
  FGCHK(hipGetLastError());
  return 0;
}

extern "C" int fg_plan_apply_frac_dev(fg_plan *pl, const double *data_dev, double *out_dev)
{
  if (!pl || !data_dev || !out_dev) return fg_fail(FG_ERR_ARG, "fg_plan_apply_frac_dev: null argument");
  if (!pl->finalized || pl->order != 1) return fg_fail(FG_ERR_STATE, "fg_plan_apply_frac_dev: needs a finalized first-order plan");
  FGCHK(hipSetDevice(pl->device));
  return plan_apply_frac(pl, data_dev, out_dev);
}

static void b1_conserve_interp(bool great_circle, int nx_src, int ny_src, int nx_dst, int ny_dst, const double *x_src,
                               const double *y_src, const double *x_dst, const double *y_dst,
                               const double *mask_src, const double *data_src, double *data_dst)
{
  const double *lons[1] = {x_src}, *lats[1] = {y_src}, *masks[1] = {mask_src};
  fg_plan *pl = nullptr;
  long nx = great_circle ? fg_plan_create_great_circle(1, &nx_src, &ny_src, lons, lats, masks, nx_dst, ny_dst, x_dst, y_dst, fg_env_device(), &pl)
                         : fg_plan_create(FG_CONSERVE_ORDER1, 1, &nx_src, &ny_src, lons, lats, masks, nx_dst, ny_dst, x_dst, y_dst, fg_env_device(), &pl);
  if (nx < 0) fatal(fg_last_error());
  if (great_circle && nx > (long)MAXXGRID) fatal("nxgrid is greater than MAXXGRID, increase MAXXGRID");
  if (!great_circle && nx >= (long)MAXXGRID)
    fatal("The xgrid size is too large for resources.\n nxgrid is greater than MAXXGRID/nthreads; increase MAXXGRID,\n"
          " decrease nthreads, or increase number of MPI ranks.");
  if (fg_plan_finalize(pl, nullptr)) fatal(fg_last_error());
  size_t ns = (size_t)nx_src * ny_src, nd = (size_t)nx_dst * ny_dst;
  double *dsrc = nullptr, *ddst = nullptr;
  if (hipMalloc(&dsrc, ns * sizeof(double)) != hipSuccess || hipMalloc(&ddst, nd * sizeof(double)) != hipSuccess) fatal("hipMalloc failed");
  if (hipMemcpy(dsrc, data_src, ns * sizeof(double), hipMemcpyHostToDevice) != hipSuccess) fatal("hipMemcpy failed");
  if (plan_apply_frac(pl, dsrc, ddst)) fatal(fg_last_error());
  if (hipMemcpy(data_dst, ddst, nd * sizeof(double), hipMemcpyDeviceToHost) != hipSuccess) fatal("hipMemcpy failed");
  (void)hipFree(dsrc); (void)hipFree(ddst);
  fg_plan_destroy(pl);
}
extern "C" void conserve_interp(int nx_src, int ny_src, int nx_dst, int ny_dst, const double *x_src,
                                const double *y_src, const double *x_dst, const double *y_dst,
                                const double *mask_src, const double *data_src, double *data_dst)
{
  b1_conserve_interp(false, nx_src, ny_src, nx_dst, ny_dst, x_src, y_src, x_dst, y_dst, mask_src, data_src, data_dst);
}
extern "C" void conserve_interp_great_circle(int nx_src, int ny_src, int nx_dst, int ny_dst, const double *x_src,
                                             const double *y_src, const double *x_dst, const double *y_dst,
                                             const double *mask_src, const double *data_src, double *data_dst)
{
  b1_conserve_interp(true, nx_src, ny_src, nx_dst, ny_dst, x_src, y_src, x_dst, y_dst, mask_src, data_src, data_dst);
}

namespace {
struct DevBuf {
  void *p = nullptr;
  DevBuf(size_t n) { if (hipMalloc(&p, n ? n : 1) != hipSuccess) p = nullptr; }
  ~DevBuf() { if (p) (void)hipFree(p); }
};
}

extern "C" int fg_clip_2dx2d_batch(int npoly, const double *lon1, const double *lat1, const int *n1,
                                   const double *lon2, const double *lat2, const int *n2,
                                   double *lon_out, double *lat_out, int *n_out)
{
  if (npoly < 0 || !lon1 || !lat1 || !n1 || !lon2 || !lat2 || !n2 || !lon_out || !lat_out || !n_out) return fg_fail(FG_ERR_ARG, "null argument");
  if (npoly == 0) return 0;
  FGCHK(hipSetDevice(fg_env_device()));
  size_t nb = (size_t)npoly * FG_POLY_STRIDE * sizeof(double), ni = (size_t)npoly * sizeof(int);
  DevBuf a(nb), b(nb), c(nb), d(nb), xo(nb), yo(nb), m1(ni), m2(ni), mo(ni);
  if (!a.p || !b.p || !c.p || !d.p || !xo.p || !yo.p || !m1.p || !m2.p || !mo.p) return fg_fail(FG_ERR_HIP, "out of device memory");
  FGCHK(hipMemcpy(a.p, lon1, nb, hipMemcpyHostToDevice)); FGCHK(hipMemcpy(b.p, lat1, nb, hipMemcpyHostToDevice));
  FGCHK(hipMemcpy(c.p, lon2, nb, hipMemcpyHostToDevice)); FGCHK(hipMemcpy(d.p, lat2, nb, hipMemcpyHostToDevice));
  FGCHK(hipMemcpy(m1.p, n1, ni, hipMemcpyHostToDevice)); FGCHK(hipMemcpy(m2.p, n2, ni, hipMemcpyHostToDevice));
  fgd_poly_clip(npoly, (double *)a.p, (double *)b.p, (int *)m1.p, (double *)c.p, (double *)d.p, (int *)m2.p,
                (double *)xo.p, (double *)yo.p, (int *)mo.p, 0);
  FGCHK(hipDeviceSynchronize());
  FGCHK(hipMemcpy(lon_out, xo.p, nb, hipMemcpyDeviceToHost)); FGCHK(hipMemcpy(lat_out, yo.p, nb, hipMemcpyDeviceToHost));
  FGCHK(hipMemcpy(n_out, mo.p, ni, hipMemcpyDeviceToHost));
  return 0;
}

extern "C" int fg_poly_op_batch(int op, int npoly, double *lon, double *lat, int *n, const double *clon, double *result)
{
  if (op < 0 || op > 6 || npoly < 0 || !lon || !lat || !n) return fg_fail(FG_ERR_ARG, "bad argument");
  if ((op == 1 || op == 3 || op == 5) && !clon) return fg_fail(FG_ERR_ARG, "clon/tlon array required");
  if (op != 3 && !result) return fg_fail(FG_ERR_ARG, "result array required");
  if (npoly == 0) return 0;
  FGCHK(hipSetDevice(fg_env_device()));
  size_t nb = (size_t)npoly * FG_POLY_STRIDE * sizeof(double), ni = (size_t)npoly * sizeof(int), nd = (size_t)npoly * sizeof(double);
  DevBuf a(nb), b(nb), m(ni), cl(nd), r(nd);
  if (!a.p || !b.p || !m.p || !cl.p || !r.p) return fg_fail(FG_ERR_HIP, "out of device memory");
  FGCHK(hipMemcpy(a.p, lon, nb, hipMemcpyHostToDevice)); FGCHK(hipMemcpy(b.p, lat, nb, hipMemcpyHostToDevice));
  FGCHK(hipMemcpy(m.p, n, ni, hipMemcpyHostToDevice));
  if (clon) FGCHK(hipMemcpy(cl.p, clon, nd, hipMemcpyHostToDevice));
  fgd_poly_op(op, npoly, (double *)a.p, (double *)b.p, (int *)m.p, (double *)cl.p, (double *)r.p, 0);
  FGCHK(hipDeviceSynchronize());
  if (op == 3) {
    FGCHK(hipMemcpy(lon, a.p, nb, hipMemcpyDeviceToHost)); FGCHK(hipMemcpy(lat, b.p, nb, hipMemcpyDeviceToHost));
    FGCHK(hipMemcpy(n, m.p, ni, hipMemcpyDeviceToHost));
  } else FGCHK(hipMemcpy(result, r.p, nd, hipMemcpyDeviceToHost));
  return 0;
}

extern "C" int clip_2dx2d(const double lon1_in[], const double lat1_in[], int n1_in, const double lon2_in[],
                          const double lat2_in[], int n2_in, double lon_out[], double lat_out[])
{
  double a[FG_POLY_STRIDE] = {0}, b[FG_POLY_STRIDE] = {0}, c[FG_POLY_STRIDE] = {0}, d[FG_POLY_STRIDE] = {0};
  double xo[FG_POLY_STRIDE], yo[FG_POLY_STRIDE];
  if (n1_in > 12 || n2_in > 12 || n1_in < 1 || n2_in < 1) fatal("clip_2dx2d: this build supports 1..12 vertices per polygon");
  for (int k = 0; k < n1_in; k++) { a[k] = lon1_in[k]; b[k] = lat1_in[k]; }
  for (int k = 0; k < n2_in; k++) { c[k] = lon2_in[k]; d[k] = lat2_in[k]; }
  int no = 0;
  if (fg_clip_2dx2d_batch(1, a, b, &n1_in, c, d, &n2_in, xo, yo, &no)) fatal(fg_last_error());
  if (no == -1) fatal("the line between <x1_0,y1_0> and  <x1_1,y1_1> should not parallel to "
                      "the line between <x2_0,y2_0> and  <x2_1,y2_1>");
  if (no < 0) fatal("clip_2dx2d: clipped polygon exceeds 24 vertices");
  for (int k = 0; k < no; k++) { lon_out[k] = xo[k]; lat_out[k] = yo[k]; }
  return no;
}
static double poly_single(int op, const double x[], const double y[], int n, double clon)
{
  double a[FG_POLY_STRIDE] = {0}, b[FG_POLY_STRIDE] = {0}, r = 0;
  if (n < 1 || n > FG_POLY_STRIDE) fatal("polygon primitive: this build supports 1..24 vertices");
  for (int k = 0; k < n; k++) { a[k] = x[k]; b[k] = y[k]; }
  if (fg_poly_op_batch(op, 1, a, b, &n, &clon, &r)) fatal(fg_last_error());
  return r;
}
extern "C" double poly_area(const double x[], const double y[], int n) { return poly_single(0, x, y, n, 0.0); }
extern "C" double poly_ctrlon(const double x[], const double y[], int n, double clon) { return poly_single(1, x, y, n, clon); }
extern "C" double poly_ctrlat(const double x[], const double y[], int n) { return poly_single(2, x, y, n, 0.0); }
extern "C" int fix_lon(double x[], double y[], int n, double tlon)
{
  double a[FG_POLY_STRIDE] = {0}, b[FG_POLY_STRIDE] = {0};
  if (n < 1 || n > 8) fatal("fix_lon: this build supports 1..8 vertices");
  for (int k = 0; k < n; k++) { a[k] = x[k]; b[k] = y[k]; }
  if (fg_poly_op_batch(3, 1, a, b, &n, &tlon, nullptr)) fatal(fg_last_error());
  if (n < 0) fatal("fix_lon: vertex capacity exceeded");
  for (int k = 0; k < n; k++) { x[k] = a[k]; y[k] = b[k]; }
  return n;
}
extern "C" void pimod(double x[], int nn)
{
  const double PI = 3.14159265358979323846;
  for (int i = 0; i < nn; i++) { if (x[i] < -PI) x[i] += 2.0 * PI; else if (x[i] > PI) x[i] -= 2.0 * PI; }
}

extern "C" int fg_c2l_grid_info(int nx, int ny, const double *xt, const double *yt, const double *xc, const double *yc,
                                double *dx, double *dy, double *area, double *edge_w, double *edge_e, double *edge_s,
                                double *edge_n, double *en_n, double *en_e, double *vlon, double *vlat);
extern "C" int fg_halo_map(int ntiles, const int *nx, const int *ny, int ncontacts, const int *tile1, const int *tile2,
                           const int *istart1, const int *iend1, const int *jstart1, const int *jend1,
                           const int *istart2, const int *iend2, const int *jstart2, const int *jend2,
                           long *map_off, int *map);

struct fg_c2l {
  int device = 0, ntiles = 0;
  hipStream_t stream = nullptr;
  bool own_stream = true;
  long ncells = 0, F = 0;
  std::vector<int> nx, ny;
  std::vector<void *> owned;
  void *tiles_dev = nullptr;
  int *map_dev = nullptr;
  int *cell_of_dev = nullptr;
  double *geom_dev[11] = {nullptr};
  std::vector<double> lont_halo, latt_halo;
  template <typename T> T *alloc(size_t n) { void *p = g_pool.get(device, n * sizeof(T)); if (p) owned.push_back(p); return (T *)p; }
};
// ... 192 lines not shown
```

### fre-nctools_amd/csrc/poly_kernels.hip

```cpp
#include "xgrid_device.h"
#include "geom.hip.h"

#define PB_IN   12
#define PB_CAP  24

__device__ inline int d_clip_private(const double *lon1, const double *lat1, int n1,
                                     const double *lon2, const double *lat2, int n2,
                                     double *lon_out, double *lat_out)
{
  double cx[PB_CAP], cy[PB_CAP], ex[PB_IN], ey[PB_IN];
  bool wrap = false;
  for (int k = 0; k < n1; k++) { cx[k] = lon1[k]; cy[k] = lat1[k]; if (cx[k] > G_TPI || cx[k] < 0.0) wrap = true; }
  for (int k = 0; k < n2; k++) { ex[k] = lon2[k]; ey[k] = lat2[k]; }
  if (wrap) {
    for (int k = 0; k < n1; k++) cx[k] = d_pimod1(cx[k]);
    for (int k = 0; k < n2; k++) ex[k] = d_pimod1(ex[k]);
  }
  int n_cur = n1;
  double x2_0 = ex[n2 - 1], y2_0 = ey[n2 - 1];
  for (int e = 0; e < n2; e++) {
    double x2_1 = ex[e], y2_1 = ey[e];
    double x1_0 = cx[n_cur - 1], y1_0 = cy[n_cur - 1];
    int inside_last = d_inside_edge(x2_0, y2_0, x2_1, y2_1, x1_0, y1_0);
    int n_new = 0;
    for (int k = 0; k < n_cur; k++) {
      double x1_1 = cx[k], y1_1 = cy[k];
      int inside = d_inside_edge(x2_0, y2_0, x2_1, y2_1, x1_1, y1_1);
      if (inside != inside_last) {
        double dy1 = y1_1 - y1_0;
        double dy2 = y2_1 - y2_0;
        double dx1 = x1_1 - x1_0;
        double dx2 = x2_1 - x2_0;
        double ds1 = y1_0 * x1_1 - y1_1 * x1_0;
        double ds2 = y2_0 * x2_1 - y2_1 * x2_0;
        double determ = dy2 * dx1 - dy1 * dx2;
        if (fabs(determ) < 1.0e-30) return -1;
        if (n_new >= PB_CAP) return -2;
        lon_out[n_new] = (dx2 * ds1 - dx1 * ds2) / determ;
        lat_out[n_new++] = (dy2 * ds1 - dy1 * ds2) / determ;
      }
      if (inside) {
        if (n_new >= PB_CAP) return -2;
        lon_out[n_new] = x1_1; lat_out[n_new++] = y1_1;
      }
      x1_0 = x1_1; y1_0 = y1_1; inside_last = inside;
    }
    n_cur = n_new;
    if (!n_cur) return 0;
    for (int k = 0; k < n_cur; k++) { cx[k] = lon_out[k]; cy[k] = lat_out[k]; }
    x2_0 = x2_1; y2_0 = y2_1;
  }
  return n_cur;
}

__global__ __launch_bounds__(64) void k_poly_clip(int npoly, const double *lon1, const double *lat1, const int *n1,
                                                   const double *lon2, const double *lat2, const int *n2,
                                                   double *lon_out, double *lat_out, int *n_out)
{
  int p = blockIdx.x * blockDim.x + threadIdx.x;
  if (p >= npoly) return;
  double a[PB_IN], b[PB_IN], c[PB_IN], d[PB_IN], xo[PB_CAP], yo[PB_CAP];
  int m1 = n1[p], m2 = n2[p];
  if (m1 < 1 || m1 > PB_IN || m2 < 1 || m2 > PB_IN) { n_out[p] = -2; return; }
  for (int k = 0; k < m1; k++) { a[k] = lon1[(size_t)p * PB_CAP + k]; b[k] = lat1[(size_t)p * PB_CAP + k]; }
  for (int k = 0; k < m2; k++) { c[k] = lon2[(size_t)p * PB_CAP + k]; d[k] = lat2[(size_t)p * PB_CAP + k]; }
  int n = d_clip_private(a, b, m1, c, d, m2, xo, yo);
  n_out[p] = n;
  for (int k = 0; k < PB_CAP; k++) {
    lon_out[(size_t)p * PB_CAP + k] = (k < n) ? xo[k] : 0.0;
    lat_out[(size_t)p * PB_CAP + k] = (k < n) ? yo[k] : 0.0;
  }
}

__global__ __launch_bounds__(64) void k_poly_op(int op, int npoly, double *lon, double *lat, int *n, const double *clon,
                                                 double *result)
{
  int p = blockIdx.x * blockDim.x + threadIdx.x;
  if (p >= npoly) return;
  double x[PB_CAP], y[PB_CAP];
  int m = n[p];
  if (m < 1 || m > PB_CAP || (op == 3 && m > G_FIXCAP - 4)) { if (result) result[p] = 0; if (op == 3) n[p] = -2; return; }
  for (int k = 0; k < m; k++) { x[k] = lon[(size_t)p * PB_CAP + k]; y[k] = lat[(size_t)p * PB_CAP + k]; }
  if (op == 0) result[p] = d_poly_area<1>(x, y, m);
  else if (op == 1) result[p] = d_poly_ctrlon<1>(x, y, m, clon[p]);
  else if (op == 2) result[p] = d_poly_ctrlat<1>(x, y, m);
  else if (op >= 4) {
    double pa, pclon, pclat;
    d_poly_area_ctr<1>(x, y, m, op == 5 ? clon[p] : 0.0, &pa, &pclon, &pclat);
    result[p] = (op == 4) ? pa : (op == 5) ? pclon : pclat;
  } else {
    int mm = d_fix_lon(x, y, m, clon[p]);
    n[p] = mm;
    for (int k = 0; k < PB_CAP; k++) {
      lon[(size_t)p * PB_CAP + k] = (k < mm) ? x[k] : 0.0;
      lat[(size_t)p * PB_CAP + k] = (k < mm) ? y[k] : 0.0;
    }
  }
}

void fgd_poly_clip(int npoly, const double *lon1, const double *lat1, const int *n1, const double *lon2, const double *lat2,
                   const int *n2, double *lon_out, double *lat_out, int *n_out, hipStream_t st)
{
  if (npoly > 0) k_poly_clip<<<(npoly + 63) / 64, 64, 0, st>>>(npoly, lon1, lat1, n1, lon2, lat2, n2, lon_out, lat_out, n_out);
}
void fgd_poly_op(int op, int npoly, double *lon, double *lat, int *n, const double *clon, double *result, hipStream_t st)
{
  if (npoly > 0) k_poly_op<<<(npoly + 63) / 64, 64, 0, st>>>(op, npoly, lon, lat, n, clon, result);
}

__global__ __launch_bounds__(256) void k_sincos_probe(long n, const double *x, double *s, double *c)
{
  long i = (long)blockIdx.x * blockDim.x + threadIdx.x;
  if (i >= n) return;
  s[i] = d_sin_lat(x[i]); c[i] = d_cos_lat(x[i]);
}
void fgd_sincos_probe(long n, const double *x, double *s, double *c, hipStream_t st)
{
  if (n > 0) k_sincos_probe<<<(int)((n + 255) / 256), 256, 0, st>>>(n, x, s, c);
}

__global__ __launch_bounds__(64) void k_xgrid_polygons(long n, const int *x_src, const int *x_dst, FgCells S, FgCells D, FgRect R, int rect,
                                                        int maxv, int *n_out, double *lon_out, double *lat_out)
{
  const long k = (long)blockIdx.x * blockDim.x + threadIdx.x;
  if (k >= n) return;
  const int s = x_src[k], d = x_dst[k];
  double a[PB_IN], b[PB_IN], c[PB_IN], e[PB_IN], xo[PB_CAP], yo[PB_CAP];
  const int n1 = S.nv[s];
  int n2;
  const FgVerts sv = d_cell_verts(S, s, n1);
  for (int q = 0; q < 8; q++) { a[q] = q < n1 ? sv.x[q] : 0.0; b[q] = q < n1 ? sv.y[q] : 0.0; }
  double lon_out_avg;
  if (rect) {
    const int j = d / R.nx, i = d - j * R.nx;
    const double *cr = R.col + (size_t)i * RECT_COLW;
    const double ya = R.lat_ax[j], yb = R.lat_ax[j + 1];
    c[0] = cr[0]; c[1] = cr[1]; c[2] = cr[2]; c[3] = cr[3]; lon_out_avg = cr[6];
    e[0] = ya; e[1] = ya; e[2] = yb; e[3] = yb;
    n2 = 4;
  } else {
    const FgVerts dv = d_cell_verts(D, d, 0);
    for (int q = 0; q < 8; q++) { c[q] = dv.x[q]; e[q] = dv.y[q]; }
    lon_out_avg = D.lon_avg[d];
    n2 = D.nv[d];
  }
  const double dx = lon_out_avg - S.lon_avg[s];
  const double shift = (dx < -G_PI) ? G_TPI : ((dx > G_PI) ? -G_TPI : 0.0);
  if (shift != 0.0) for (int q = 0; q < n2; q++) c[q] += shift;
  int m = (n1 < 1 || n2 < 1) ? 0 : d_clip_private(a, b, n1, c, e, n2, xo, yo);
  n_out[k] = m;
  for (int q = 0; q < maxv; q++) {
    lon_out[(size_t)k * maxv + q] = (q < m && q < PB_CAP) ? xo[q] : 0.0;
    lat_out[(size_t)k * maxv + q] = (q < m && q < PB_CAP) ? yo[q] : 0.0;
  }
}
void fgd_xgrid_polygons(long n, const int *x_src, const int *x_dst, FgCells S, FgCells D, const FgRect *rect, int maxv,
                        int *n_out, double *lon_out, double *lat_out, hipStream_t st)
{
  if (n > 0) k_xgrid_polygons<<<(unsigned)((n + 63) / 64), 64, 0, st>>>(n, x_src, x_dst, S, D, rect ? *rect : FgRect{}, rect ? 1 : 0, maxv,
                                                                      n_out, lon_out, lat_out);
}
__global__ __launch_bounds__(256) void k_xgrid_gather_gc(long n, const int *x_src, const int *x_dst, FgCells S, FgCells D, double *a, double *b)
{
  const long t = (long)blockIdx.x * blockDim.x + threadIdx.x;
  if (t >= n * 12) return;
  const long k = t / 12; const int q = (int)(t - k * 12);
  a[t] = S.verts[(size_t)x_src[k] * 16 + q];
  b[t] = D.verts[(size_t)x_dst[k] * 16 + q];
}
// ... 19 lines not shown
```

### fre-nctools_amd/csrc/xgrid_device.h

```cpp
#pragma once
#include <hip/hip_runtime.h>

struct FgTile {
  const double *lon;
  const double *lat;
  int nx, ny;
  int cell_off;
};

struct FgTileXyz {
  const double *x, *y, *z;
  int nx, ny;
  int cell_off;
};
#define G_ERRBIT_GC_CONVEX1 16u
#define G_ERRBIT_GC_CONVEX2 32u
#define G_ERRBIT_GC_CLIP    64u

#define FG_VSTRIDE_QUAD 8
struct FgCells {
  double *lat_min, *lat_max, *lon_min, *lon_max, *lon_avg, *area;
  int *nv;
  double *verts;
  int vstride;
  int wide_cap;
  double *wide;
};
#ifdef __HIPCC__
struct FgVerts { const double *x, *y; };
__device__ __forceinline__ FgVerts d_cell_verts(const FgCells &c, int s, int n)
{
  if (c.vstride == FG_VSTRIDE_QUAD) {
    const double *v = c.verts + (size_t)s * FG_VSTRIDE_QUAD;
    if (n > 4) {
      const int k = *(const int *)v;
      const double *w = c.wide + (size_t)((unsigned)k < (unsigned)c.wide_cap ? k : 0) * 16;
      return FgVerts{w, w + 8};
    }
    return FgVerts{v, v + 4};
  }
  const double *v = c.verts + (size_t)s * 16;
  return FgVerts{v, v + 8};
}
__device__ __forceinline__ double *d_cell_quad(const FgCells &c, int s) { return c.verts + (size_t)s * FG_VSTRIDE_QUAD; }
#endif

struct FgBins {
  int nblat, nblon;
  double inv_wlat, inv_wlon;
};

struct FgBinEntry {
  double lat_min, lat_max, lon_min, lon_max, lon_avg;
  int d;
  int row0;
};

enum {
  FG_STAT_PAIRS = 0,
  FG_STAT_NONEMPTY = 1,
  FG_STAT_NXGRID = 2,
  FG_STAT_BORDERLINE = 3,
  FG_STAT_BINS = 4,
  FG_STAT_BIN_ENTRIES = 5,
  FG_STAT_DEFERRED = 6,
  FG_STAT_HEAVY = 7,
  FG_STAT_BELOW = 8,
  FG_STAT_EXACT = 9,
  FG_STAT_RARE = 10,
  FG_NSTATS = 11
};

#define FG_REG_ALIGN 512
#define FG_NREG 64
#define FG_FILL_STRIDE 32
struct FgPairSpace {
  int *src, *dst;
  unsigned *fill;
  int regcap, nreg;
};
#ifdef __HIPCC__
__device__ __forceinline__ bool d_pair_live(const FgPairSpace &ps, int p)
{
  const unsigned first = blockIdx.x * blockDim.x;
  const unsigned r = first / (unsigned)ps.regcap;
  const unsigned f = ps.fill[r * FG_FILL_STRIDE];
  return (unsigned)p - r * (unsigned)ps.regcap < (f < (unsigned)ps.regcap ? f : (unsigned)ps.regcap);
}
#endif
static inline long fgd_pairs_total(const FgPairSpace &ps) { return (long)ps.regcap * ps.nreg; }
#ifdef __HIPCC__
__device__ __forceinline__ unsigned long long d_ord_key(double v)
{
  const unsigned long long b = (unsigned long long)__double_as_longlong(v);
  return (b >> 63) ? ~b : (b | 0x8000000000000000ull);
}
__device__ __forceinline__ double d_ord_val(unsigned long long k)
{
  const unsigned long long b = (k >> 63) ? (k & 0x7fffffffffffffffull) : ~k;
  return __longlong_as_double((long long)b);
}
#endif

#define FG_TILESET_MAX 8
struct FgTileSet { FgTile t[FG_TILESET_MAX]; int n; };

struct FgLl2xGrid { const double *lon, *lat; double *x, *y, *z; long n; };
struct FgLl2xSet { FgLl2xGrid g[FG_TILESET_MAX]; int n; };
#define G_ERRBIT_LL2X 256u
#define G_ERRBIT_WIDECAP 512u
void fgd_latlon2xyz(const FgLl2xGrid *grids, int ngrids, unsigned *err, hipStream_t st);

struct FgCounters {
  unsigned long long total[4];
  unsigned long long rows_total;
  unsigned long long band_keys[2];
  unsigned long long xtot;
  unsigned err[4];
  int heavy_cnt;
  unsigned rect_bad;
  int defer_cnt, big_cnt;
  int gc_list2_cnt;
  int rare_cnt;
  unsigned long long stats[FG_NSTATS];
};
#define G_ERRBIT_LOOKBACK 128u

long fgd_scan_tiles(long n);
void fgd_exclusive_scan1(const int *in, long n, int *out, unsigned long long *status, unsigned *ticket,
                         unsigned long long *total_dev, unsigned *err, hipStream_t st);

void fgd_exclusive_scan2(const int *in_a, long n_a, int *out_a, unsigned long long *status_a, unsigned *ticket_a, unsigned long long *total_a,
                         const int *in_b, long n_b, int *out_b, unsigned long long *status_b, unsigned *ticket_b, unsigned long long *total_b,
                         unsigned *err, hipStream_t st);

void fgd_cell_struct2(const FgTileSet &ts, const FgTile *tiles_in, FgTile *tiles_out, int ntiles, int nsrc, int ndst, FgCells S, FgCells D,
                      FgBins b, int *slot_cnt, int order, int *src_idx_f, double *sums, unsigned *err, hipStream_t st,
                      unsigned long long *band_keys = nullptr, int cull = 0, double dst_tlon = 3.14159265358979323846);
void fgd_cell_struct(const FgTile *tiles_dev, int ntiles, int ncells, FgCells c, unsigned *err, hipStream_t st);
void fgd_band_keys(const double *lat, long n, unsigned long long *band_keys, hipStream_t st);
void fgd_bin_count(int ncells, FgCells c, FgBins b, int *slot_cnt, hipStream_t st);
void fgd_bin_fill(int ndst, FgCells D, FgBins b, int *slot_fill, const int *slot_start, FgBinEntry *entries, int cap,
                  int nsrc, FgCells S, const double *mask, int *heavy_list, int *heavy_cnt, hipStream_t st);
void fgd_candidates1(int nsrc, FgCells S, const double *mask, FgBins b, const int *slot_start, const FgBinEntry *entries, int ecap,
                     FgPairSpace ps, int *pair_beg, int *pair_cnt, const int *heavy_list, const int *heavy_cnt, int *big_list, int *big_cnt,
                     hipStream_t st);
#define RECT_COLW 8
struct FgRect {
  const double *lon_ax;
  const double *lat_ax;
  const double *col;
  const double *col_min, *col_max, *col_avg;
  const double *hdr;
  const double *row;
  const unsigned *bad;
  int nx, ny;
};
void fgd_rect_tables(const double *lon, const double *lat, int nx, int ny, double *hdr, double *lat_ax, double *lon_ax, double *col,
                     double *col_min, double *col_max, double *col_avg, double *row, unsigned *bad, unsigned *err, hipStream_t st,
                     double dst_tlon = 3.14159265358979323846);
void fgd_cell_struct2r(const FgTileSet &ts, const FgTile *tiles_in, FgTile *tiles_out, int ntiles, int nsrc, int ndst, FgCells S, double *area_out,
                       FgRect R, const double *mask, int order, int *src_idx_f, double *sums, unsigned *err, hipStream_t st,
                       unsigned long long *band_keys, int cull, int *heavy_list, int *heavy_cnt, int *rare_list, int *rare_cnt, FgPairSpace ps,
                       int *pair_beg, int *pair_cnt, int *big_list, int *big_cnt);
void fgd_rect_materialize(int ndst, FgRect R, FgCells D, hipStream_t st);
void fgd_quad_materialize(int nsrc, FgCells S, double *lon_min, double *lon_max, double *verts, hipStream_t st);
struct FgPolyList { const int *n; const double *lon, *lat; const double *lon_avg, *area; int npoly; };
void fgd_polylist_records(FgPolyList P, FgCells S, int *src_idx_f, double *sums, const FgRect *rect, int *heavy_list, int *heavy_cnt,
                          unsigned *err, hipStream_t st);
void fgd_candidates_rect(int nsrc, FgCells S, const double *mask, FgRect R, FgPairSpace ps, int *pair_beg, int *pair_cnt,
                         const int *heavy_list, const int *heavy_cnt, int *big_list, int *big_cnt, hipStream_t st, int listed_only,
                         const int *rare_list = nullptr, const int *rare_cnt = nullptr, unsigned *err = nullptr,
                         double *sums = nullptr);
void fgd_clip_general(int order, FgPairSpace ps, FgCells S, const double *mask, FgCells D,
              double *tmp_area, double *tmp_clon, double *tmp_clat, int *nacc, int *defer_list, int *defer_cnt,
              unsigned long long *stats, unsigned *err, hipStream_t st, const FgRect *rect = nullptr, int *row_cnt = nullptr,
              int *tmp_rowpos = nullptr);
void fgd_clip_quad(int order, FgPairSpace ps, FgCells S, const double *mask, FgCells D,
              double *tmp_area, double *tmp_clon, double *tmp_clat, int *nacc, int *defer_list, int *defer_cnt,
              unsigned long long *stats, unsigned *err, hipStream_t st, const FgRect *rect = nullptr, int *row_cnt = nullptr,
              int *tmp_rowpos = nullptr);
struct alignas(8) FgRowEnt { int n, s; };
struct alignas(16) FgSrcRec { double cen_lon, cen_lat; };
struct FgCompactIo {
  const int *pair_beg, *pair_cnt;
  const double *tmp_area, *tmp_clon, *tmp_clat;
  const int *xoff;
  int *x_src, *x_dst;
  double *x_area, *x_c1, *x_c2;
  int *row_cnt, *x_rowpos;
  const int *tmp_rowpos;
  const int *row_ptr; FgRowEnt *perm;
  double *sums;
  const int *big_list;
  const int *big_cnt;
  FgCounters *dc;
  long xcap;
};
void fgd_compact(int order, int nsrc, FgPairSpace ps, const FgCompactIo &io, hipStream_t st);
void fgd_centroids(int nsrc, FgCells S, const double *sums, FgSrcRec *cen, hipStream_t st);
void fgd_distances(long nx, const int *x_src, const double *x_area, const FgSrcRec *cen, double *x_c1, double *x_c2, hipStream_t st);

struct FgCsrEntry1 { int idx_f; int pad; double area; };
struct FgCsrEntry2 { int idx_f; int idx_g; double area, di, dj; };
struct FgCsr {
  int *row_ptr;
  FgCsrEntry1 *e1;
  FgCsrEntry2 *e2;
};
void fgd_csr_count(long nx, const int *x_dst, int *row_cnt, hipStream_t st);
void fgd_csr_fill(long nx, const int *x_src, const int *x_dst, const int *row_ptr, int *row_fill, FgRowEnt *perm, hipStream_t st);
void fgd_csr_fill_pos(long nx_cap, const unsigned long long *nx_dev, const int *x_src, const int *x_dst, const int *row_ptr, const int *x_rowpos,
                      FgRowEnt *perm, hipStream_t st);
void fgd_csr_sortgather(int order, int ndst, long nx, const FgRowEnt *perm, const double *x_area, const double *x_c1, const double *x_c2,
                        const int *src_idx_f, const FgSrcRec *cen, FgCsr csr, hipStream_t st, int *tmp = nullptr, long ntmp = 0,
                        int long_rows = 0);
void fgd_src_field_index(int order, const FgTile *tiles_dev, int ntiles, int nsrc, int *src_idx_f, hipStream_t st);
void fgd_apply1(int order, int ndst, FgCsr csr, const double *f, const double *gx, const double *gy, const int *gmask,
                int has_missing, double missing, double *out, double *row_sum, hipStream_t st, long nx = -1);
void fgd_apply_il(int order, int nb, int ndst, FgCsr csr, const double *f, const double *gx, const double *gy, double missing,
                  double *out, double *row_sum, long out_ld, int nb_valid, hipStream_t st, long nx = -1);
void fgd_interleave(int nb_pad, long n, const double *in, long ld, int nb_valid, double *out, hipStream_t st);
void fgd_apply_il_merged(int nb, int ndst, long nx, FgCsr csr, const double *rec, double missing, double *out, double *row_sum, long out_ld,
                         int nb_valid, hipStream_t st);
void fgd_merge3(int nb_pad, long n, const int *src_idx_f, const double *f, long ld_f, const double *gx, const double *gy, long ld_g,
                int nb_valid, double *out, hipStream_t st);
void fgd_interleave3(int nb_pad, int narr, const double *const *in, const long *ld, const long *n, double *const *out, int nb_valid,
                     hipStream_t st);
void fgd_deinterleave(int nb_pad, long n, const double *in, long ld, int nb_valid, double *out, hipStream_t st);
#define FG_LEVELS_CAP 256
void fgd_apply_levels8(int order, int ndst, long nx, FgCsr csr, const double *rec, const unsigned char *gbits, double missing, double *out,
                       double *row_sum, long ld, int nb_valid, hipStream_t st);
void fgd_gmask_bits(long n, const int *gmask, long ld, int nb, unsigned char *bits, hipStream_t st);
void fgd_apply_frac(int ndst, FgCsr csr, const double *data, double *out, hipStream_t st);
void fgd_reduce_sum(const double *v, long n, double *partial, double *result, hipStream_t st);
void fgd_xgrid_indices(long nx, const int *x_src, const int *x_dst, const FgTile *tiles_dev, int ntiles, int nx_out,
                       int *t_in, int *i_in, int *j_in, int *i_out, int *j_out, hipStream_t st);

struct FgApplyEx {
  const double *weight;
  const double *cell_area;
  const double *field_area;
  const double *cell_area_out;
  const int *gmask;
  const double *xdata;
  double area_missing, missing;
  int has_missing, sum;
};
#define FG_XERR_AREA_MISSING 1
#define FG_XERR_ABOVE 2
#define FG_XERR_BELOW 4
void fgd_apply_ex(int order, int ndst, FgCsr csr, const double *f, const double *gx, const double *gy, FgApplyEx o,
                  double *out, double *row_sum, int *err, hipStream_t st, long nx = -1);
#define FG_LEVELS_EX_CAP 256
#define FG_LEVELS_EX_CAP_Z 128
void fgd_apply_levels8x(int order, int ndst, long nx, FgCsr csr, const double *rec, const unsigned char *gbits, FgApplyEx o, const double *fa8,
                        double *out, double *row_sum, long ld, int nb_valid, int *err, hipStream_t st);
void fgd_mono_bounds(const FgTile *tiles_dev, int ntiles, int nsrc, const int *src_idx_f, const double *f, double missing,
                     double *fbmax, double *fbmin, double *fmax, double *fmin, hipStream_t st);
void fgd_mono_xdata(long nx, FgCsr csr, const double *f, const double *gx, const double *gy, const int *gmask, double missing,
                    double *xdata, double *fmax, double *fmin, hipStream_t st);
void fgd_mono_limit(long nx, FgCsr csr, const double *f, double missing, const double *fbmax, const double *fbmin,
                    const double *fmax, const double *fmin, double *xdata, int *err, hipStream_t st);
#define FG_LEVELS_MONO_CAP 128
// ... 80 lines not shown
```

### fre-nctools_amd/csrc/xgrid_kernels.hip

```cpp
#include <algorithm>
#include "xgrid_device.h"
#ifndef FG_EXP
#define FG_EXP 0
#endif
static __shared__ double fgs_lds_tab[112 * 4];
#define FGS_TAB(k, j) fgs_lds_tab[(k) * 4 + (j)]
#include "geom.hip.h"
__device__ __forceinline__ void d_load_trig_table()
{
  for (int i = threadIdx.x; i < 112 * 4; i += blockDim.x) fgs_lds_tab[i] = FG_SINCOS_TAB[i >> 2][i & 3];
  __syncthreads();
}

#define SCAN_THREADS 256
#define SCAN_ITEMS   8
#define SCAN_CHUNK   (SCAN_THREADS * SCAN_ITEMS)
#define LB_AGG   (1ull << 62)
#define LB_INC   (2ull << 62)
#define LB_MASK  ((1ull << 62) - 1ull)
#define LB_SPIN_LIMIT (1u << 22)

__device__ __forceinline__ unsigned wave_incl_scan(unsigned v, int lane)
{
#pragma unroll
// ... 1212 lines not shown
    int i = 0; bool pass = false;
    if (k < nwc) { i = d_rect_col(q, k); pass = d_rect_col_pass(R, i, lon_in_min, lon_in_max, lon_in_avg); }
    const unsigned long long m = __ballot(pass);
    const int at = cbase + __popcll(m & ((1ull << lane) - 1ull));
    if (pass)
      for (int jr = 0; jr < nr; jr++) {
        const long kk = (long)jr * nc + at;
        if (kk < n_ok) { ps.src[wbase + kk] = s; ps.dst[wbase + kk] = (q.j0 + jr) * R.nx + i; }
      }
    cbase += __popcll(m);
  }
  if (lane == 0) { pair_beg[s] = wbase; pair_cnt[s] = n_ok; if (n_ok > CP_SMALL) big_list[atomicAdd(big_cnt, 1)] = s; }
  if (zero_sums && n_ok == 0 && lane < 3) zero_sums[(size_t)lane * nsrc + s] = 0.0;
}

#define RARE_BLOCKS 64
template <bool FINISH>
__global__ __launch_bounds__(64) void k_candidates_rect(int nsrc, int H, FgCells S, const double *mask, FgRect R, FgPairSpace ps,
                                                         int *pair_beg, int *pair_cnt, const int *heavy_list, const int *heavy_cnt,
                                                         int *big_list, int *big_cnt, const int *rare_list, const int *rare_cnt, unsigned *err,
                                                         double *sums )
{
  const int lane = threadIdx.x;
  __shared__ unsigned wl[64 * RECT_WL_WORDS];
  if (FINISH && (int)blockIdx.x < RARE_BLOCKS) d_load_trig_table();
  const unsigned bad = *R.bad;
  const int nrare = FINISH ? *rare_cnt : 0;
  if (bad) return;
  const int hb = FINISH ? (int)blockIdx.x - RARE_BLOCKS : (int)blockIdx.x;
  if (hb >= 0 && hb < H) {
    const int nheavy = *heavy_cnt;
    for (int h = hb; h < nheavy; h += H) {
      const int s = heavy_list[h];
      double xmin, xmax;
      if constexpr (FINISH) {
        const double *q = d_cell_quad(S, s);
        const int n = S.nv[s];
        double x[G_MAXV];
#pragma unroll
        for (int k = 0; k < G_MAXV; k++) x[k] = k < 4 ? q[k] : 0.0;
        if (n > 4) {
          const FgVerts v = d_cell_verts(S, s, n);
#pragma unroll
          for (int k = 0; k < G_MAXV; k++) x[k] = v.x[k];
        }
        xmin = x[0]; xmax = x[0];
#pragma unroll
        for (int k = 1; k < G_MAXV; k++) if (k < n) { if (x[k] < xmin) xmin = x[k]; if (x[k] > xmax) xmax = x[k]; }
      } else { xmin = S.lon_min[s]; xmax = S.lon_max[s]; }
      d_rect_cell_candidates(R, ps, s, lane, S.lat_min[s], S.lat_max[s], xmin, xmax, S.lon_avg[s], pair_beg, pair_cnt, big_list, big_cnt,
                             FINISH ? sums : nullptr, nsrc);
    }
    return;
  }
  if constexpr (FINISH) {
    for (int h = blockIdx.x; h < nrare; h += RARE_BLOCKS) {
      const int s = rare_list[h];
      const double mk = mask ? mask[s] : 1.0;
      double b[5] = {0, 0, 0, 0, 0};
      const int nv = d_finish_rare_cell(S, err, s, h, lane, b);
      if (!(nv > 0 && mk > 0.5)) {
        if (sums && lane < 3) sums[(size_t)lane * nsrc + s] = 0.0;
        continue;
      }
      if (d_rect_heavy(R, b[0], b[1], b[2], b[3])) d_rect_cell_candidates(R, ps, s, lane, b[0], b[1], b[2], b[3], b[4], pair_beg, pair_cnt, big_list, big_cnt, sums, nsrc);
      else {
        int npair = 0;
        (void)d_rect_wave_candidates<true>(R, ps, lane == 0, s, nsrc, (unsigned)(s >> 6), b[0], b[1], b[2], b[3], b[4], pair_beg, pair_cnt, big_list, big_cnt, wl, &npair);
        npair = __shfl(npair, 0);
        if (sums && npair == 0 && lane < 3) sums[(size_t)lane * nsrc + s] = 0.0;
      }
    }
  } else {
    const int bR = (int)blockIdx.x - H;
    const int s = bR * 64 + lane;
    const bool active = s < nsrc && d_src_active(S, mask, s);
    double b[5] = {0, 0, 0, 0, 0};
    if (active) { b[0] = S.lat_min[s]; b[1] = S.lat_max[s]; b[2] = S.lon_min[s]; b[3] = S.lon_max[s]; b[4] = S.lon_avg[s]; }
    (void)d_rect_wave_candidates(R, ps, active, s, nsrc, (unsigned)bR, b[0], b[1], b[2], b[3], b[4], pair_beg, pair_cnt, big_list, big_cnt, wl);
  }
}

struct ClipOut { double area, clon, clat; };

template <int ORDER, int S>
__device__ __forceinline__ void d_finish_pair(const double *px, const double *py, int n_out, double maskv,
                                              double area_in, double area_out, double lon_in_avg,
                                              ClipOut *o, unsigned long long *stats)
{
  double pa, clon = 0, clat = 0;
  if (ORDER == 2) d_poly_area_ctr<S>(px, py, n_out, lon_in_avg, &pa, &clon, &clat);
  else pa = d_poly_area<S>(px, py, n_out);
  double xarea = pa * maskv;
  double min_area = (area_in < area_out) ? area_in : area_out;
  double ratio = xarea / min_area;
  if (fabs(ratio - 1.e-6) < 1.e-15) atomicAdd(&stats[FG_STAT_BORDERLINE], 1ull);
  if (ratio > 1.e-6) { o->area = xarea; o->clon = clon; o->clat = clat; }
  else o->area = -2.0;
}

#ifndef CLIP_THREADS
#define CLIP_THREADS 256
#endif
#ifndef CLIP_SLOTS
#define CLIP_SLOTS 8
#endif
#ifndef CLIP_WAVES
#define CLIP_WAVES 4
#endif
#ifndef CLIP_PAD_LDS
#define CLIP_PAD_LDS 0
#endif

template <bool RECT, int T, bool QSRC = false>
__device__ __forceinline__ int d_clip_quad_sh(double2 (*sh_poly)[T], const int tid, const int s, const int d,
                                              const FgCells &S, const FgCells &D, const FgRect &R, unsigned *err)
{
  constexpr int NV1 = RECT ? CLIP_SLOTS : 4;
  double x1[NV1], y1[NV1], x2[4], y2[4];
  double lon_out_avg;
  int n1 = S.nv[s], n2 = RECT ? 4 : D.nv[d];
  double lon_in_avg = S.lon_avg[s];
  if constexpr (QSRC) {
    const double *sq = d_cell_quad(S, s);
#pragma unroll
    for (int k = 0; k < NV1; k++) { x1[k] = k < 4 ? sq[k] : 0.0; y1[k] = k < 4 ? sq[4 + k] : 0.0; }
  } else {
    const FgVerts sv = d_cell_verts(S, s, 0);
#pragma unroll
    for (int k = 0; k < NV1; k++) { x1[k] = sv.x[k]; y1[k] = sv.y[k]; }
  }
  if (RECT) {
    const int j = d / R.nx, i = d - j * R.nx;
    const double *c = R.col + (size_t)i * RECT_COLW;
    double ya = R.lat_ax[j], yb = R.lat_ax[j + 1];
    x2[0] = c[0]; x2[1] = c[1]; x2[2] = c[2]; x2[3] = c[3]; lon_out_avg = c[6];
    asm volatile("" : "+v"(ya), "+v"(yb));
    y2[0] = ya; y2[1] = ya; y2[2] = yb; y2[3] = yb;
  } else {
    const FgVerts dv = d_cell_verts(D, d, 0);
#pragma unroll
    for (int k = 0; k < 4; k++) { x2[k] = dv.x[k]; y2[k] = dv.y[k]; }
    lon_out_avg = D.lon_avg[d];
#pragma unroll
    for (int k = 0; k < 4; k++) asm volatile("" : "+v"(y2[k]));
    asm volatile("" : "+v"(n2));
  }
#pragma unroll
  for (int k = 0; k < NV1; k++) asm volatile("" : "+v"(x1[k]), "+v"(y1[k]));
#pragma unroll
  for (int k = 0; k < 4; k++) asm volatile("" : "+v"(x2[k]));
  asm volatile("" : "+v"(n1), "+v"(lon_in_avg), "+v"(lon_out_avg));
  if (n1 > NV1 || n2 > 4) return -1;
  if (RECT && !(x2[3] == x2[0] && x2[1] == x2[2])) return -1;
  if constexpr (QSRC) {
    if (n1 > 4) {
      const FgVerts sv = d_cell_verts(S, s, n1);
#pragma unroll
      for (int k = 0; k < NV1; k++) { x1[k] = sv.x[k]; y1[k] = sv.y[k]; }
    }
  }
  double shift = 0.0;
  {
    double dx = lon_out_avg - lon_in_avg;
    if (dx < -G_PI) shift = G_TPI; else if (dx > G_PI) shift = -G_TPI;
  }
  bool wrap = false;
#pragma unroll
  for (int k = 0; k < NV1; k++) {
    if (!(k < 4 || k < n1)) { x1[k] = 0.0; y1[k] = 0.0; }
    if (k < n1 && (x1[k] > G_TPI || x1[k] < 0.0)) wrap = true;
  }
#pragma unroll
  for (int k = 0; k < 4; k++) if (shift != 0.0) x2[k] += shift;
  if (wrap) {
#pragma unroll
    for (int k = 0; k < NV1; k++) x1[k] = d_pimod1(x1[k]);
#pragma unroll
    for (int k = 0; k < 4; k++) x2[k] = d_pimod1(x2[k]);
  }
#pragma unroll
  for (int k = 0; k < NV1; k++) if (k < 4 || k < n1) sh_poly[k][tid] = make_double2(x1[k], y1[k]);
  const long long b0x = __double_as_longlong(x2[0]), b1x = __double_as_longlong(x2[1]);
  const long long b2x = __double_as_longlong(x2[2]), b3x = __double_as_longlong(x2[3]);
  const long long b0y = __double_as_longlong(y2[0]), b1y = __double_as_longlong(y2[1]);
  const long long b2y = __double_as_longlong(y2[2]), b3y = __double_as_longlong(y2[3]);
  auto cut = [=](int e) -> double2 {
    const long long m0 = -(long long)(e == 0), m1 = -(long long)(e == 1), m2 = -(long long)(e == 2), m3 = -(long long)(e == 3);
    return make_double2(__longlong_as_double((b0x & m0) | (b1x & m1) | (b2x & m2) | (b3x & m3)),
                        __longlong_as_double((b0y & m0) | (b1y & m1) | (b2y & m2) | (b3y & m3)));
  };
  int n_cur = n1;
  bool overflow = false, parallel = false;
  double2 e0 = cut(n2 - 1);
#if FG_EXP == 2
  for (int e = 0; e < 0; e++) {
#else
#pragma unroll
  for (int e = 0; e < 4; e++) {
    if ((!RECT && e >= n2) || n_cur <= 0) break;
#endif
    double2 e1 = cut(e);
    const double x2_0 = e0.x, y2_0 = e0.y, x2_1 = e1.x, y2_1 = e1.y;
    double2 c[CLIP_SLOTS];
    unsigned inmask = 0u;
#pragma unroll
    for (int k = 0; k < CLIP_SLOTS; k++) c[k] = sh_poly[k][tid];
    const double axis = (e & 1) ? x2_0 - x2_1 : y2_1 - y2_0;
#pragma unroll
    for (int k = 0; k < CLIP_SLOTS; k++)
      if (k < n_cur) {
        int in;
        if (RECT) in = (((e & 1) ? axis * (c[k].y - y2_0) : (c[k].x - x2_0) * axis) <= 1.e-12) ? 1 : 0;
        else in = d_inside_edge(x2_0, y2_0, x2_1, y2_1, c[k].x, c[k].y);
        inmask |= (unsigned)in << k;
      }
    const unsigned full = (1u << n_cur) - 1u;
    const unsigned prevmask = ((inmask << 1) | (inmask >> (n_cur - 1))) & full;
    const unsigned tmask = inmask ^ prevmask;
    const int ncross = __popc(tmask);
    if (ncross > 2 || ncross + __popc(inmask) > CLIP_SLOTS) { overflow = true; break; }
    if (tmask) {
      const int ka = __ffs((int)tmask) - 1, kb = 31 - __clz((int)tmask);
      double2 I[2];
#pragma unroll
      for (int j = 0; j < 2; j++) {
        const int k = j ? kb : ka;
        const double2 p0 = sh_poly[k ? k - 1 : n_cur - 1][tid], p1 = sh_poly[k][tid];
        const double x1_0 = p0.x, y1_0 = p0.y, x1_1 = p1.x, y1_1 = p1.y;
        double dy1 = y1_1 - y1_0;
        double dy2 = y2_1 - y2_0;
        double dx1 = x1_1 - x1_0;
        double dx2 = x2_1 - x2_0;
        double ds1 = y1_0 * x1_1 - y1_1 * x1_0;
        double ds2 = y2_0 * x2_1 - y2_1 * x2_0;
        double determ = dy2 * dx1 - dy1 * dx2;
        if (fabs(determ) < 1.0e-30) parallel = true;
        I[j] = make_double2((dx2 * ds1 - dx1 * ds2) / determ, (dy2 * ds1 - dy1 * ds2) / determ);
      }
#pragma unroll
      for (int k = 0; k < CLIP_SLOTS; k++)
        if (k < n_cur && ((inmask >> k) & 1u))
          sh_poly[__popc(inmask & ((1u << k) - 1u)) + __popc(tmask & ((2u << k) - 1u))][tid] = c[k];
      sh_poly[__popc(inmask & ((1u << ka) - 1u))][tid] = I[0];
      sh_poly[__popc(inmask & ((1u << kb) - 1u)) + 1][tid] = I[1];
    }
    n_cur = ncross + __popc(inmask);
    e0 = e1;
  }
  if (overflow) return -1;
  if (parallel) atomicOr(err, G_ERRBIT_PARALLEL);
  return n_cur;
}

#ifndef CLIP_COMPACT
#define CLIP_COMPACT 0
#endif
__device__ __forceinline__ int d_row_slot(int *row_cnt, bool take, int d, int lane);
template <int ORDER, bool RECT, bool QSRC = false>
__global__ __launch_bounds__(CLIP_THREADS) __attribute__((amdgpu_waves_per_eu(CLIP_WAVES, CLIP_WAVES))) void k_clip_quad(FgPairSpace ps, FgCells S, const double *mask, FgCells D, FgRect R,
                                                 double *tmp_area, double *tmp_clon, double *tmp_clat, int *nacc,
                                                 int *defer_list, int *defer_cnt,
                                                 unsigned long long *stats, unsigned *err, int *row_cnt, int *tmp_rowpos)
{
  constexpr int T = CLIP_THREADS;
  __shared__ double2 sh_poly[CLIP_SLOTS][T];
#if CLIP_PAD_LDS
  __shared__ char sh_pad[CLIP_PAD_LDS];
  if (nacc == (int *)16) sh_pad[threadIdx.x * 7 % CLIP_PAD_LDS] = 1;
#endif
#if CLIP_COMPACT
  __shared__ unsigned short sh_perm[T];
  __shared__ unsigned char sh_n[T];
  __shared__ int sh_wtot[T / 64];
#endif
  const int tid = threadIdx.x, lane = tid & 63;
  const int p0 = blockIdx.x * T;
  const unsigned first = blockIdx.x * T, reg = first / (unsigned)ps.regcap;
  const unsigned fill = ps.fill[reg * FG_FILL_STRIDE];
  const unsigned bad = RECT ? *R.bad : 0u;
  if ((RECT && bad != 0u) | (first - reg * (unsigned)ps.regcap >= fill)) return;
  static_assert(2 * T >= 112 * 4, "at most two table values per lane");
  const int t0 = min(tid, 112 * 4 - 1), t1 = min(tid + T, 112 * 4 - 1);
  int s_in = ps.src[p0 + tid], d_in = ps.dst[p0 + tid];
  double tab0 = FG_SINCOS_TAB[t0 >> 2][t0 & 3], tab1 = FG_SINCOS_TAB[t1 >> 2][t1 & 3];
  asm volatile("" : "+v"(s_in), "+v"(d_in), "+v"(tab0), "+v"(tab1));
  fgs_lds_tab[t0] = tab0; fgs_lds_tab[t1] = tab1;
  __syncthreads();
  bool defer = false;
  int n_cur = 0;
  if ((unsigned)(p0 + tid) - reg * (unsigned)ps.regcap < min(fill, (unsigned)ps.regcap)) {
    n_cur = d_clip_quad_sh<RECT, T, QSRC>(sh_poly, tid, s_in, d_in, S, D, R, err);
    if (n_cur < 0) { defer = true; n_cur = 0; }
    else if (n_cur == 0) ps.dst[p0 + tid] = -1;
  }
  int src = tid;
#if CLIP_COMPACT
  {
    const int wave = tid >> 6;
    const unsigned long long hm = __ballot(n_cur > 0);
    if (lane == 0) sh_wtot[wave] = __popcll(hm);
    sh_n[tid] = (unsigned char)n_cur;
    __syncthreads();
    int base = 0, total = 0;
#pragma unroll
    for (int w = 0; w < T / 64; w++) { const int c = sh_wtot[w]; if (w < wave) base += c; total += c; }
    if (n_cur > 0) sh_perm[base + __popcll(hm & ((1ull << lane) - 1ull))] = (unsigned short)tid;
    __syncthreads();
    if (tid < total) { src = sh_perm[tid]; n_cur = sh_n[src]; } else n_cur = 0;
  }
#endif
  bool below = false, acc = false;
  int s = -1, d_acc = -1;
  if (n_cur > 0) {
    const int p = p0 + src;
    s = CLIP_COMPACT ? ps.src[p] : s_in;
    const int d = CLIP_COMPACT ? ps.dst[p] : d_in;
    ClipOut o; o.area = -1.0; o.clon = 0; o.clat = 0;
    const double *px = (const double *)&sh_poly[0][src];
#if FG_EXP == 1
    o.area = n_cur + px[0] + px[1];
#else
    d_finish_pair<ORDER, 2 * T>(px, px + 1, n_cur, mask ? mask[s] : 1.0, S.area[s], D.area[d], S.lon_avg[s], &o, stats);
#endif
    if (o.area >= 0) {
      acc = true;
      tmp_area[p] = o.area;
      if (ORDER == 2) { tmp_clon[p] = o.clon; tmp_clat[p] = o.clat; }
      d_acc = d;
    } else {
      ps.dst[p] = -1;
      below = (o.area == -2.0);
    }
  }
  if (row_cnt) {
    const int slot = d_row_slot(row_cnt, acc, d_acc, lane);
    if (acc) tmp_rowpos[p0 + src] = slot;
  }
  if (__ballot(s >= 0)) {
    const int s_prev = __shfl_up(s, 1, 64);
    const bool head = (lane == 0) || (s != s_prev);
    const unsigned long long hm = __ballot(head), am = __ballot(acc);
    if (head && s >= 0) {
      const unsigned long long above = (lane == 63) ? 0ull : (hm >> (lane + 1)) << (lane + 1);
      const int end = above ? (__ffsll((long long)above) - 1) : 64;
      const unsigned long long upto = (end == 64) ? ~0ull : ((1ull << end) - 1ull);
      const int cnt = __popcll(am & upto & ~((1ull << lane) - 1ull));
      if (cnt) atomicAdd(&nacc[s], cnt);
    }
  }
  const unsigned long long dm = __ballot(defer), bm = __ballot(below);
  if (dm) {
    int q = 0;
    if (lane == 0) q = atomicAdd(defer_cnt, __popcll(dm));
    q = __shfl(q, 0);
    if (defer) defer_list[q + __popcll(dm & ((1ull << lane) - 1ull))] = p0 + tid;
  }
  if (bm && lane == 0) atomicAdd(&stats[FG_STAT_BELOW], (unsigned long long)__popcll(bm));
}

#define GEN_THREADS 64
#define GEN_CAP 16
template <int ORDER, bool RECT>
__global__ __launch_bounds__(GEN_THREADS) void k_clip_general(const int *defer_list, const int *defer_cnt,
                                                              const int *pair_src, int *pair_dst,
                                                              FgCells S, const double *mask, FgCells D, FgRect R,
                                                              double *tmp_area, double *tmp_clon, double *tmp_clat, int *nacc,
                                                              unsigned long long *stats, unsigned *err, int *row_cnt, int *tmp_rowpos)
{
  __shared__ double2 sh_a[GEN_CAP][GEN_THREADS];
  __shared__ double2 sh_b[GEN_CAP][GEN_THREADS];
  __shared__ double2 sh_cut[G_MAXV][GEN_THREADS];
  if (RECT && *R.bad) return;
  d_load_trig_table();
  const int tid = threadIdx.x;
  const int ndefer = *defer_cnt;
  for (int q = blockIdx.x * GEN_THREADS + tid; q < ndefer; q += gridDim.x * GEN_THREADS) {
    const int p = defer_list[q];
    const int s = pair_src[p], d = pair_dst[p];
    const int n1 = S.nv[s], n2 = RECT ? 4 : D.nv[d];
    const FgVerts sv = d_cell_verts(S, s, n1);
    const double lon_in_avg = S.lon_avg[s];
    double dvx[G_MAXV], dvy[G_MAXV], lon_out_avg;
    if (RECT) {
      const int j = d / R.nx, i = d - j * R.nx;
      const double *c = R.col + (size_t)i * RECT_COLW;
      const double ya = R.lat_ax[j], yb = R.lat_ax[j + 1];
      dvx[0] = c[0]; dvx[1] = c[1]; dvx[2] = c[2]; dvx[3] = c[3]; lon_out_avg = c[6];
      dvy[0] = ya; dvy[1] = ya; dvy[2] = yb; dvy[3] = yb;
#pragma unroll
      for (int k = 4; k < G_MAXV; k++) { dvx[k] = 0.0; dvy[k] = 0.0; }
    } else {
      const FgVerts dv = d_cell_verts(D, d, n2);
#pragma unroll
      for (int k = 0; k < G_MAXV; k++) { dvx[k] = dv.x[k]; dvy[k] = dv.y[k]; }
      lon_out_avg = D.lon_avg[d];
    }
    double shift = 0.0;
    {
      double dx = lon_out_avg - lon_in_avg;
      if (dx < -G_PI) shift = G_TPI; else if (dx > G_PI) shift = -G_TPI;
    }
    bool wrap = false;
    for (int k = 0; k < n1; k++) { double xv = sv.x[k]; if (xv > G_TPI || xv < 0.0) wrap = true; }
    for (int k = 0; k < n1; k++) {
      double xv = sv.x[k]; if (wrap) xv = d_pimod1(xv);
      sh_a[k][tid] = make_double2(xv, sv.y[k]);
    }
#pragma unroll
    for (int k = 0; k < G_MAXV; k++)
      if (k < n2) {
        double xv = dvx[k]; if (shift != 0.0) xv += shift; if (wrap) xv = d_pimod1(xv);
        sh_cut[k][tid] = make_double2(xv, dvy[k]);
      }
    double2 (*cur)[GEN_THREADS] = sh_a;
    double2 (*nxt)[GEN_THREADS] = sh_b;
    int n_cur = n1;
    bool overflow = false, parallel = false;
    double2 e0 = sh_cut[n2 - 1][tid];
    for (int e = 0; e < n2 && n_cur > 0 && !overflow; e++) {
      double2 e1 = sh_cut[e][tid];
      const double x2_0 = e0.x, y2_0 = e0.y, x2_1 = e1.x, y2_1 = e1.y;
      double2 lastv = cur[n_cur - 1][tid];
      double x1_0 = lastv.x, y1_0 = lastv.y;
      int inside_last = d_inside_edge(x2_0, y2_0, x2_1, y2_1, x1_0, y1_0);
      int n_new = 0;
      for (int k = 0; k < n_cur; k++) {
        double2 cv = cur[k][tid];
        double x1_1 = cv.x, y1_1 = cv.y;
        int inside = d_inside_edge(x2_0, y2_0, x2_1, y2_1, x1_1, y1_1);
        if (inside != inside_last) {
          double dy1 = y1_1 - y1_0;
          double dy2 = y2_1 - y2_0;
          double dx1 = x1_1 - x1_0;
          double dx2 = x2_1 - x2_0;
          double ds1 = y1_0 * x1_1 - y1_1 * x1_0;
          double ds2 = y2_0 * x2_1 - y2_1 * x2_0;
          double determ = dy2 * dx1 - dy1 * dx2;
          if (fabs(determ) < 1.0e-30) parallel = true;
          if (n_new < GEN_CAP) nxt[n_new][tid] = make_double2((dx2 * ds1 - dx1 * ds2) / determ,
// ... 262 lines not shown
  const int s = blockIdx.x * blockDim.x + threadIdx.x;
  double a = 0, ca = 1, cl = 0, ct = 0;
  int nv = 0;
  bool whole = false;
  if (s < nsrc && (a = sums[s]) > 0) {
    const double sl = sums[nsrc + s], st = sums[2 * (size_t)nsrc + s], sa = S.area[s];
    nv = S.nv[s];
    if (nv > 0) {
      ca = sa;
      if (fabs(a - ca) / ca < 1.e-3) {
        cl = sl / a;
        ct = st / a;
      } else whole = true;
    }
  }
  if (__syncthreads_or(whole)) {
    d_load_trig_table();
    if (whole) {
      double x[G_MAXV], y[G_MAXV];
      int n = nv;
      const FgVerts vp = d_cell_verts(S, s, n);
      for (int k = 0; k < G_MAXV; k++) { x[k] = k < n ? vp.x[k] : 0.0; y[k] = k < n ? vp.y[k] : 0.0; }
      cl = d_poly_ctrlon<1>(x, y, n, S.lon_avg[s]) / ca;
      ct = d_poly_ctrlat<1>(x, y, n) / ca;
    }
  }
  if (s < nsrc) cen[s] = FgSrcRec{cl, ct};
}

__global__ __launch_bounds__(256) void k_distances(long nx, const int *x_src, const double *x_area, const FgSrcRec *cen, double *x_c1,
                                                    double *x_c2)
{
  long n = (long)blockIdx.x * blockDim.x + threadIdx.x;
  if (n >= nx) return;
  int s = x_src[n];
  double a = x_area[n];
  double di = x_c1[n] / a, dj = x_c2[n] / a;
  di -= cen[s].cen_lon; dj -= cen[s].cen_lat;
  x_c1[n] = di; x_c2[n] = dj;
}

static inline int nblk(long n, int t) { return (int)((n + t - 1) / t); }

void fgd_cell_struct(const FgTile *tiles_dev, int ntiles, int ncells, FgCells c, unsigned *err, hipStream_t st)
{
  if (ncells > 0) k_cell_struct<<<nblk(ncells, 256), 256, 0, st>>>(tiles_dev, ntiles, ncells, c, err);
}

void fgd_cell_struct2(const FgTileSet &ts, const FgTile *tiles_in, FgTile *tiles_out, int ntiles, int nsrc, int ndst, FgCells S, FgCells D,
                      FgBins b, int *slot_cnt, int order, int *src_idx_f, double *sums, unsigned *err, hipStream_t st,
                      unsigned long long *band_keys, int cull, double dst_tlon)
{
  const int nbS = nblk(nsrc, 256), nbD = nblk(ndst, 256);
  if (nbS + nbD > 0)
    k_cell_struct2<<<nbS + nbD, 256, 0, st>>>(ts, tiles_in, tiles_out, ntiles, nsrc, ndst, nbS, S, D, b, slot_cnt, order, src_idx_f, sums, err,
                                              band_keys, cull, dst_tlon);
}

void fgd_bin_count(int ncells, FgCells c, FgBins b, int *slot_cnt, hipStream_t st)
{
  if (ncells > 0) k_bin_count<<<nblk(ncells, 256), 256, 0, st>>>(ncells, c, b, slot_cnt);
}

void fgd_bin_fill(int ndst, FgCells D, FgBins b, int *slot_fill, const int *slot_start, FgBinEntry *entries, int cap,
                  int nsrc, FgCells S, const double *mask, int *heavy_list, int *heavy_cnt, hipStream_t st)
{
  const int nbD = nblk(ndst, 256), nbS = nblk(nsrc, 256);
  if (nbD + nbS > 0)
    k_bin_fill<<<nbD + nbS, 256, 0, st>>>(ndst, nbD, D, b, slot_fill, slot_start, entries, cap, nsrc, S, mask, heavy_list, heavy_cnt);
}

void fgd_candidates1(int nsrc, FgCells S, const double *mask, FgBins b, const int *slot_start, const FgBinEntry *entries, int ecap,
                     FgPairSpace ps, int *pair_beg, int *pair_cnt, const int *heavy_list, const int *heavy_cnt, int *big_list, int *big_cnt,
                     hipStream_t st)
{
  if (nsrc <= 0) return;
  const int nbR = nblk((long)nsrc * CAND_G, 64);
  const int H = min(8 * HEAVY_BLOCKS, max(64, nblk(nsrc, 8)));
  k_candidates1<<<nbR + H, 64, 0, st>>>(nsrc, H, S, mask, b, slot_start, entries, ecap, ps, pair_beg, pair_cnt, heavy_list, heavy_cnt, big_list, big_cnt);
}

void fgd_clip_quad(int order, FgPairSpace ps, FgCells S, const double *mask, FgCells D,
                   double *tmp_area, double *tmp_clon, double *tmp_clat, int *nacc, int *defer_list, int *defer_cnt,
                   unsigned long long *stats, unsigned *err, hipStream_t st, const FgRect *rect, int *row_cnt, int *tmp_rowpos)
{
  const long np = fgd_pairs_total(ps);
  if (np <= 0) return;
  const FgRect R = rect ? *rect : FgRect{};
  const int g = nblk(np, CLIP_THREADS);
#define FG_LAUNCH_QUAD(O, RC, QS) k_clip_quad<O, RC, QS><<<g, CLIP_THREADS, 0, st>>>(ps, S, mask, D, R, tmp_area, tmp_clon, tmp_clat, nacc, defer_list, defer_cnt, stats, err, row_cnt, tmp_rowpos)
  const bool qsrc = rect && S.vstride == FG_VSTRIDE_QUAD;
  if (order == 2) { if (qsrc) FG_LAUNCH_QUAD(2, true, true); else if (rect) FG_LAUNCH_QUAD(2, true, false); else FG_LAUNCH_QUAD(2, false, false); }
  else            { if (qsrc) FG_LAUNCH_QUAD(1, true, true); else if (rect) FG_LAUNCH_QUAD(1, true, false); else FG_LAUNCH_QUAD(1, false, false); }
#undef FG_LAUNCH_QUAD
}

void fgd_clip_general(int order, FgPairSpace ps, FgCells S, const double *mask, FgCells D,
                      double *tmp_area, double *tmp_clon, double *tmp_clat, int *nacc, int *defer_list, int *defer_cnt,
                      unsigned long long *stats, unsigned *err, hipStream_t st, const FgRect *rect, int *row_cnt, int *tmp_rowpos)
{
  const long np = fgd_pairs_total(ps);
  if (np <= 0) return;
  int grid = nblk(np, GEN_THREADS); if (grid > 1024) grid = 1024;
  const FgRect R = rect ? *rect : FgRect{};
#define FG_LAUNCH_GEN(O, RC) k_clip_general<O, RC><<<grid, GEN_THREADS, 0, st>>>(defer_list, defer_cnt, ps.src, ps.dst, S, mask, D, R, tmp_area, tmp_clon, tmp_clat, nacc, stats, err, row_cnt, tmp_rowpos)
  if (order == 2) { if (rect) FG_LAUNCH_GEN(2, true); else FG_LAUNCH_GEN(2, false); }
  else            { if (rect) FG_LAUNCH_GEN(1, true); else FG_LAUNCH_GEN(1, false); }
#undef FG_LAUNCH_GEN
}

void fgd_rect_tables(const double *lon, const double *lat, int nx, int ny, double *hdr, double *lat_ax, double *lon_ax, double *col,
                     double *col_min, double *col_max, double *col_avg, double *row, unsigned *bad, unsigned *err, hipStream_t st, double dst_tlon)
{
  const long np = (long)(nx + 1) * (ny + 1);
  const int nbT = (std::max(nx, ny) + 1 + 255) / 256;
  const int nbV = (int)std::min<long>(RECT_VERIFY_BLOCKS, std::max<long>((np + 255) / 256, 1));
  k_rect_tables<<<nbT + nbV, 256, 0, st>>>(lon, lat, nx, ny, hdr, lat_ax, lon_ax, col, col_min, col_max, col_avg, row, bad, err, dst_tlon);
}
void fgd_cell_struct2r(const FgTileSet &ts, const FgTile *tiles_in, FgTile *tiles_out, int ntiles, int nsrc, int ndst, FgCells S, double *area_out,
                       FgRect R, const double *mask, int order, int *src_idx_f, double *sums, unsigned *err, hipStream_t st,
                       unsigned long long *band_keys, int cull, int *heavy_list, int *heavy_cnt, int *rare_list, int *rare_cnt, FgPairSpace ps,
                       int *pair_beg, int *pair_cnt, int *big_list, int *big_cnt)
{
  const int nbS = nblk(nsrc, 256), nbD = nblk(ndst, 256);
  if (nbS + nbD > 0)
    k_cell_struct2r<<<nbS + nbD, 256, 0, st>>>(ts, tiles_in, tiles_out, ntiles, nsrc, ndst, nbS, S, area_out, R, mask, order, src_idx_f, sums, err,
                                               band_keys, cull, heavy_list, heavy_cnt, rare_list, rare_cnt, ps, pair_beg, pair_cnt, big_list, big_cnt);
}
void fgd_polylist_records(FgPolyList P, FgCells S, int *src_idx_f, double *sums, const FgRect *rect, int *heavy_list, int *heavy_cnt,
                          unsigned *err, hipStream_t st)
{
  if (P.npoly > 0)
    k_polylist_records<<<nblk(P.npoly, 256), 256, 0, st>>>(P, S, src_idx_f, sums, rect ? *rect : FgRect{}, rect ? 1 : 0, heavy_list, heavy_cnt, err);
}
void fgd_rect_materialize(int ndst, FgRect R, FgCells D, hipStream_t st)
{
  if (ndst > 0) k_rect_materialize<<<nblk(ndst, 256), 256, 0, st>>>(ndst, R, D);
}
void fgd_quad_materialize(int nsrc, FgCells S, double *lon_min, double *lon_max, double *verts, hipStream_t st)
{
  if (nsrc > 0) k_quad_materialize<<<nblk(nsrc, 256), 256, 0, st>>>(nsrc, S, lon_min, lon_max, verts);
}
void fgd_candidates_rect(int nsrc, FgCells S, const double *mask, FgRect R, FgPairSpace ps, int *pair_beg, int *pair_cnt,
                         const int *heavy_list, const int *heavy_cnt, int *big_list, int *big_cnt, hipStream_t st, int listed_only,
                         const int *rare_list, const int *rare_cnt, unsigned *err, double *sums)
{
  if (nsrc <= 0) return;
  const int nbR = listed_only ? 0 : nblk(nsrc, 64);
  const int H = min(HEAVY_BLOCKS, max(64, nblk(nsrc, 8)));
  const int Hf = max(H - RARE_BLOCKS, RARE_BLOCKS);
  if (listed_only) k_candidates_rect<true><<<Hf + RARE_BLOCKS, 64, 0, st>>>(nsrc, Hf, S, mask, R, ps, pair_beg, pair_cnt, heavy_list, heavy_cnt, big_list, big_cnt,
                                                          rare_list, rare_cnt, err, sums);
  else k_candidates_rect<false><<<nbR + H, 64, 0, st>>>(nsrc, H, S, mask, R, ps, pair_beg, pair_cnt, heavy_list, heavy_cnt, big_list, big_cnt,
                                                       nullptr, nullptr, nullptr, nullptr);
}

void fgd_compact(int order, int nsrc, FgPairSpace ps, const FgCompactIo &io, hipStream_t st)
{
  if (nsrc <= 0) return;
  const long np = fgd_pairs_total(ps);
  if (order == 2) k_compact<2><<<BIG_BLOCKS + nblk(np, 256), 256, 0, st>>>(nsrc, ps, io);
  else            k_compact<1><<<BIG_BLOCKS + nblk(np, 256), 256, 0, st>>>(nsrc, ps, io);
}

void fgd_centroids(int nsrc, FgCells S, const double *sums, FgSrcRec *cen, hipStream_t st)
{
  if (nsrc > 0) k_centroids<<<nblk(nsrc, 256), 256, 0, st>>>(nsrc, S, sums, cen);
}

void fgd_distances(long nx, const int *x_src, const double *x_area, const FgSrcRec *cen, double *x_c1, double *x_c2, hipStream_t st)
{
  if (nx > 0) k_distances<<<nblk(nx, 256), 256, 0, st>>>(nx, x_src, x_area, cen, x_c1, x_c2);
}

__global__ __launch_bounds__(256) void k_accumulate_cell_sums(int n, const int *cells, int nsrc, const int *xoff, const double *xa,
                                                               const double *c1, const double *c2, double *total)
{
// ... 16 lines not shown
```

### include/fregrid_hip.h

```cpp
#ifndef FREGRID_HIP_H_
#define FREGRID_HIP_H_

#include <stddef.h>

#ifdef __cplusplus
extern "C" {
#endif

#define FG_ERR_ARG        (-1)
#define FG_ERR_HIP        (-2)
#define FG_ERR_MAXV       (-3)
#define FG_ERR_PARALLEL   (-4)
#define FG_ERR_CAPACITY   (-5)
#define FG_ERR_STATE      (-6)
#define FG_ERR_GEOM       (-8)
#define FG_ERR_IO         (-9)
#define FG_ERR_NOTFOUND   (-10)
#define FG_ERR_BILIN_NOTFOUND (-11)
#define FG_ERR_DATA       (-7)

#define FG_CONSERVE_ORDER1 1
#define FG_CONSERVE_ORDER2 2

int  get_maxxgrid(void);
// ... 74 lines not shown

int fg_plan_get_polygons(const fg_plan *plan, int maxv, int *n_out, double *v0, double *v1, double *v2);
long fg_plan_create_polylist(int order, int npoly, const int *n, const double *lon, const double *lat, const double *lon_avg,
                             const double *area_ref, int nx_out, int ny_out, const double *lon_out, const double *lat_out,
                             int device, fg_plan **plan_out);
long fg_plan_create_polylist_gc(int npoly, const int *n, const double *x, const double *y, const double *z, const double *area_ref,
                                int nx_out, int ny_out, const double *lon_out, const double *lat_out, int device, fg_plan **plan_out);
int fg_plan_get_cell_area(const fg_plan *plan, double *area_in, double *area_out);

int fg_plan_set_xgrid(fg_plan *plan, long nxgrid, const int *t_in, const int *i_in, const int *j_in,
                      const int *i_out, const int *j_out, const double *area,
                      const double *di_in, const double *dj_in);

int fg_plan_apply(fg_plan *plan, const double *data, const double *grad_x, const double *grad_y,
                  const int *grad_mask, int has_missing, double missing, int nz,
                  double *out, double *gsum_out);

int fg_plan_apply_interleaved(fg_plan *plan, int nb, const double *data_il, const double *grad_x_il,
                              const double *grad_y_il, double *out_il, double *gsum_out);

int fg_plan_apply_records(fg_plan *plan, int nz, const double *rec, double *out, double *gsum_out);

int fg_plan_apply_levels(fg_plan *plan, const double *data, const double *grad_x, const double *grad_y,
                         const int *grad_mask, double missing, int nlev, double *out, double *gsum_out);
int fg_plan_apply_records_levels(fg_plan *plan, int nz, const double *rec, const unsigned char *maskbits, double missing,
                                 double *out, double *gsum_out);
int fg_plan_levels_capacity(void);

typedef struct fg_apply_opts {
  int has_missing;
  double missing;
  const double *weight;
  int cell_methods_sum;
  const double *field_area;
  double area_missing;
  const double *cell_area_in;
  const double *cell_area_out;
  int monotonic;
} fg_apply_opts;
int fg_plan_apply_ex(fg_plan *plan, const fg_apply_opts *opts, const double *data, const double *grad_x,
                     const double *grad_y, const int *grad_mask, int nz, double *out, double *gsum_out);
int fg_plan_apply_levels_ex(fg_plan *plan, const fg_apply_opts *opts, const double *data, const double *grad_x,
                            const double *grad_y, const int *grad_mask, int nlev, long field_area_ld, double *out,
                            double *gsum_out);
int fg_plan_apply_records_levels_ex(fg_plan *plan, const fg_apply_opts *opts, int nz, const double *rec,
                                    const unsigned char *maskbits, long field_area_ld, double *out, double *gsum_out);
int fg_plan_levels_ex_capacity(int per_level_area);

int fg_plan_mono_begin(fg_plan *plan, const fg_apply_opts *opts, const double *data, const double *grad_x,
                       const double *grad_y, const int *grad_mask);
int fg_plan_mono_minmax_dev(fg_plan *plan, double **f_min, double **f_max);
int fg_plan_mono_copy_minmax(fg_plan *plan, int to_plan, double *f_min, double *f_max);
int fg_plan_mono_end(fg_plan *plan, const fg_apply_opts *opts, const double *data, double *out, double *gsum_out);

int fg_plan_apply_levels_mono(fg_plan *plan, const fg_apply_opts *opts, const double *data, const double *grad_x,
                              const double *grad_y, const int *grad_mask, int nlev, double *out, double *gsum_out);
int fg_plan_mono_levels_begin(fg_plan *plan, const fg_apply_opts *opts, const double *data, const double *grad_x,
                              const double *grad_y, const int *grad_mask, int nz);
int fg_plan_mono_levels_copy_minmax(fg_plan *plan, int to_plan, double *f_min, double *f_max);
int fg_plan_mono_levels_end(fg_plan *plan, const fg_apply_opts *opts, const double *data, const double *grad_x,
                            const double *grad_y, const int *grad_mask, double *out, double *gsum_out);

int fg_plan_apply_records_levels_mono(fg_plan *plan, const fg_apply_opts *opts, int nz, const double *rec,
                                      const unsigned char *maskbits, double *b8, double *out, double *gsum_out);
int fg_plan_mono_records_reset(fg_plan *plan, double *b8);
int fg_plan_mono_records_begin(fg_plan *plan, const fg_apply_opts *opts, int nz, const double *rec,
                               const unsigned char *maskbits, double *b8);
int fg_plan_mono_records_copy_minmax(fg_plan *plan, int to_plan, double *f_min, double *f_max);
int fg_plan_mono_records_end(fg_plan *plan, const fg_apply_opts *opts, const double *rec, const unsigned char *maskbits,
                             double *out, double *gsum_out);

void *fg_plan_stream(fg_plan *plan);
int fg_plan_sync(fg_plan *plan);

void fg_set_profiling(int on);
int  fg_plan_phase_ms(fg_plan *plan, float *ms, int n);

int fg_plan_stats(const fg_plan *plan, long *stats, int n);
void fg_set_search_mode(int exact);
void fg_set_search_cull(int on);
void fg_set_search_finalize(int on);
void fg_set_search_async(int on);
void fg_set_search_rect(int on);
void fg_set_search_wide_cap(int n);
void fg_set_search_frame(int coupler);
void fg_set_apply_ep(int on);
void fg_set_apply_vec(int v);
void fg_set_gc_split(int on);
void fg_set_apply_xcd(int on);

int fg_clip_2dx2d_batch(int npoly, const double *lon1, const double *lat1, const int *n1,
                        const double *lon2, const double *lat2, const int *n2,
                        double *lon_out, double *lat_out, int *n_out);
int fg_poly_op_batch(int op, int npoly, double *lon, double *lat, int *n, const double *clon, double *result);

typedef struct fg_c2l fg_c2l;

int  fg_c2l_create(int ntiles, const int *nx, const int *ny, const double *const *lonc, const double *const *latc,
                   const double *const *lont, const double *const *latt,
                   int ncontacts, const int *tile1, const int *tile2,
                   const int *istart1, const int *iend1, const int *jstart1, const int *jend1,
                   const int *istart2, const int *iend2, const int *jstart2, const int *jend2,
                   int device, fg_c2l **out);
void fg_c2l_destroy(fg_c2l *h);
long fg_c2l_ncells(const fg_c2l *h);
long fg_c2l_halo_size(const fg_c2l *h);
int  fg_c2l_set_stream(fg_c2l *h, void *stream);
int  fg_c2l_sync(fg_c2l *h);
int  fg_c2l_get_centres(const fg_c2l *h, double *lont_halo, double *latt_halo);
int  fg_c2l_fill_halo(fg_c2l *h, const double *src, double *halo_data, int nz);
int  fg_c2l_gradient(fg_c2l *h, const double *halo_data, int nz, int has_missing, double missing,
                     double *grad_x, double *grad_y, int *grad_mask);
int  fg_c2l_gradient_records(fg_c2l *h, const double *halo_data, int nz, double *rec);
int  fg_c2l_records(fg_c2l *h, const double *src, int nz, double *rec);
int  fg_c2l_records_levels(fg_c2l *h, const double *src, int nz, double missing, double *rec, unsigned char *maskbits);
int  fg_c2l_records_levels_mono(fg_c2l *h, const double *src, int nz, double missing, double *rec, unsigned char *maskbits,
                                double *b8);

int fg_c2l_grid_info(int nx, int ny, const double *xt, const double *yt, const double *xc, const double *yc,
                     double *dx, double *dy, double *area, double *edge_w, double *edge_e, double *edge_s,
                     double *edge_n, double *en_n, double *en_e, double *vlon, double *vlat);
int fg_find_contacts(int ntiles, const int *nx, const int *ny, const double *const *lonc, const double *const *latc,
                     int max_contacts, int *tile1, int *tile2, int *istart1, int *iend1, int *jstart1, int *jend1,
                     int *istart2, int *iend2, int *jstart2, int *jend2);
int fg_halo_map(int ntiles, const int *nx, const int *ny, int ncontacts, const int *tile1, const int *tile2,
                const int *istart1, const int *iend1, const int *jstart1, const int *jend1,
                const int *istart2, const int *iend2, const int *jstart2, const int *jend2,
                long *map_off, int *map);

int  fg_remap_write(const char *path, int order, long ncells, const int *tile1, const int *tile1_cell,
                    const int *tile2_cell, const double *xgrid_area, const double *tile1_distance);
int  fg_remap_write_interp(const char *path, int order, long n, const int *t_in, const int *i_in, const int *j_in,
                           const int *i_out, const int *j_out, const double *area, const double *di_in,
                           const double *dj_in, int isc, int jsc);
long fg_remap_read_size(const char *path);
int  fg_remap_read(const char *path, int order, long ncells, int *t_in, int *i_in, int *j_in, int *i_out, int *j_out,
                   double *area, double *di_in, double *dj_in);
const char *fg_remap_last_error(void);

#define FG_NC_BYTE 1
#define FG_NC_CHAR 2
#define FG_NC_SHORT 3
#define FG_NC_INT 4
#define FG_NC_FLOAT 5
#define FG_NC_DOUBLE 6
typedef struct fg_ncfile fg_ncfile;
int  fg_nc_open(const char *path, fg_ncfile **out);
int  fg_nc_create(const char *path, int version , fg_ncfile **out);
int  fg_nc_def_dim(fg_ncfile *f, const char *name, long len );
int  fg_nc_def_var(fg_ncfile *f, const char *name, int type, int ndims, const int *dimids);
int  fg_nc_put_att_text(fg_ncfile *f, int varid , const char *name, const char *val);
int  fg_nc_put_att_double(fg_ncfile *f, int varid, const char *name, int type, int n, const double *vals);
int  fg_nc_enddef(fg_ncfile *f);
int  fg_nc_inq_ndims(const fg_ncfile *f);
int  fg_nc_inq_nvars(const fg_ncfile *f);
long fg_nc_inq_numrecs(const fg_ncfile *f);
int  fg_nc_inq_dimid(const fg_ncfile *f, const char *name);
int  fg_nc_inq_dim(const fg_ncfile *f, int dimid, char *name, int cap, long *len);
int  fg_nc_inq_varid(const fg_ncfile *f, const char *name);
int  fg_nc_inq_var(const fg_ncfile *f, int varid, char *name, int cap, int *type, int *ndims, int *dimids, long *shape);
int  fg_nc_get_att_double(const fg_ncfile *f, int varid, const char *name, double *val, int cap);
int  fg_nc_get_att_text(const fg_ncfile *f, int varid, const char *name, char *buf, int cap);
int  fg_nc_get_vara(fg_ncfile *f, int varid, const long *start, const long *count, void *out);
int  fg_nc_get_vara_double(fg_ncfile *f, int varid, const long *start, const long *count, double *out);
int  fg_nc_put_vara(fg_ncfile *f, int varid, const long *start, const long *count, const void *data);
int  fg_nc_put_vara_double(fg_ncfile *f, int varid, const long *start, const long *count, const double *data);
// ... 274 lines not shown
```

Measured before the change: 6.035 billion exchange-cells/s.

## Offload long-polygon area/centroid tails from clip_quad to a separate compacted kernel

Result: slower. 5.656 billion exchange-cells/s (-6.3%).

```diff
diff --git a/fre-nctools_amd/_lib.py b/fre-nctools_amd/_lib.py
--- a/fre-nctools_amd/_lib.py
+++ b/fre-nctools_amd/_lib.py
@@ -42,7 +42,7 @@
     "fg_nc_inq_ndims", "fg_nc_inq_nvars", "fg_nc_inq_numrecs", "fg_nc_inq_dimid", "fg_nc_inq_dim", "fg_nc_inq_varid", "fg_nc_inq_var",
     "fg_nc_get_att_double", "fg_nc_get_att_text", "fg_nc_get_vara", "fg_nc_get_vara_double", "fg_nc_put_vara", "fg_nc_put_vara_double",
     "fg_nc_close", "fg_nc_last_error", "fg_dev_widen", "fg_dev_narrow", "fg_sweep_create", "fg_sweep_run", "fg_sweep_run_levels", "fg_sweep_run_levels_ex", "fg_sweep_destroy", "fg_host_alloc", "fg_host_free",
-    "fg_plan_stats", "fg_set_search_mode", "fg_set_search_cull", "fg_set_search_finalize", "fg_set_search_async", "fg_set_search_rect", "fg_set_search_wide_cap", "fg_set_search_frame", "fg_set_apply_xcd", "fg_set_apply_vec", "fg_set_apply_ep", "fg_set_gc_split", "fg_set_profiling", "fg_plan_phase_ms", "fg_gnomonic_ed_corners", "fg_latlon_corners",
+    "fg_plan_stats", "fg_set_search_mode", "fg_set_search_cull", "fg_set_search_finalize", "fg_set_search_async", "fg_set_search_rect", "fg_set_clip_tail_cap", "fg_set_search_wide_cap", "fg_set_search_frame", "fg_set_apply_xcd", "fg_set_apply_vec", "fg_set_apply_ep", "fg_set_gc_split", "fg_set_profiling", "fg_plan_phase_ms", "fg_gnomonic_ed_corners", "fg_latlon_corners",
     "fg_bilin_create", "fg_bilin_create_from_weights", "fg_bilin_destroy", "fg_bilin_get_index_weight", "fg_bilin_npoints_fine",
     "fg_bilin_nlon_fine", "fg_bilin_nlat_fine", "fg_bilin_nlon", "fg_bilin_nlat", "fg_bilin_ncells", "fg_bilin_set_stream",
     "fg_bilin_sync", "fg_bilin_apply_scalar", "fg_bilin_apply_vector", "fg_bilin_remap_write", "fg_bilin_remap_read",
diff --git a/fre-nctools_amd/conserve_interp.py b/fre-nctools_amd/conserve_interp.py
--- a/fre-nctools_amd/conserve_interp.py
+++ b/fre-nctools_amd/conserve_interp.py
@@ -217,9 +217,9 @@
         check(lib().fg_plan_accumulate_cell_sums(*args))
 
     def stats(self):
-        s = (C.c_long * 11)()
-        check(lib().fg_plan_stats(self._h, s, 11))
-        names = ["pairs", "nonempty", "nxgrid", "borderline", "bins", "bin_entries", "deferred", "heavy", "below", "exact_mode", "rare"]
+        s = (C.c_long * 12)()
+        check(lib().fg_plan_stats(self._h, s, 12))
+        names = ["pairs", "nonempty", "nxgrid", "borderline", "bins", "bin_entries", "deferred", "heavy", "below", "exact_mode", "rare", "tails"]
         return dict(zip(names, [int(v) for v in s]))
 
     PHASES = ["cell_struct", "bins", "candidates", "clip_quad", "clip_general", "compact", "rows",
diff --git a/fre-nctools_amd/csrc/geom.hip.h b/fre-nctools_amd/csrc/geom.hip.h
--- a/fre-nctools_amd/csrc/geom.hip.h
+++ b/fre-nctools_amd/csrc/geom.hip.h
@@ -107,27 +107,54 @@
   return v;
 }
 
-template <int S>
-__device__ inline double d_poly_area(const double *x, const double *y, int n)
-{
-  double area = 0.0;
-  for (int i = 0; i < n; i++) {
-    int ip = (i + 1 == n) ? 0 : i + 1;
-    double dx = (x[ip * S] - x[i * S]);
-    double lat1 = y[ip * S], lat2 = y[i * S];
-    if (dx > G_PI)  dx = dx - 2.0 * G_PI;
-    if (dx < -G_PI) dx = dx + 2.0 * G_PI;
-    if (fabs(dx + G_PI) < G_SMALL || fabs(dx - G_PI) < G_SMALL) { area += G_PI; continue; }
-    if (fabs(lat1 - lat2) < G_SMALL)
-      area -= dx * d_sin_lat(0.5 * (lat1 + lat2));
-    else {
-      double dy = 0.5 * (lat1 - lat2);
-      double dat = d_sin_lat(dy) / dy;
-      area -= dx * d_sin_lat(0.5 * (lat1 + lat2)) * dat;
-    }
-  }
+__device__ __forceinline__ double d_area_edge(double phi1, double lat1, double phi2, double lat2, double area)
+{
+  double dx = (phi1 - phi2);
+  if (dx > G_PI)  dx = dx - 2.0 * G_PI;
+  if (dx < -G_PI) dx = dx + 2.0 * G_PI;
+  if (fabs(dx + G_PI) < G_SMALL || fabs(dx - G_PI) < G_SMALL) return area + G_PI;
+  if (fabs(lat1 - lat2) < G_SMALL)
+    area -= dx * d_sin_lat(0.5 * (lat1 + lat2));
+  else {
+    double dy = 0.5 * (lat1 - lat2);
+    double dat = d_sin_lat(dy) / dy;
+    area -= dx * d_sin_lat(0.5 * (lat1 + lat2)) * dat;
+  }
+  return area;
+}
+__device__ __forceinline__ double d_area_sign_scale(double area)
+{
   if (area < 0) return -area * G_RADIUS * G_RADIUS;
   return area * G_RADIUS * G_RADIUS;
+}
+
+template <int S>
+__device__ inline double d_poly_area_edges(const double *x, const double *y, int n, int i0, int i1, double area)
+{
+  for (int i = i0; i < i1; i++) {
+    int ip = (i + 1 == n) ? 0 : i + 1;
+    area = d_area_edge(x[ip * S], y[ip * S], x[i * S], y[i * S], area);
+  }
+  return (i1 == n) ? d_area_sign_scale(area) : area;
+}
+
+template <int S>
+__device__ inline double d_poly_area(const double *x, const double *y, int n)
+{
+  return d_poly_area_edges<S>(x, y, n, 0, n, 0.0);
+}
+
+template <int I0, int CAP>
+__device__ __forceinline__ double d_poly_area_tail(const double *x, const double *y, int n, double area)
+{
+#pragma unroll
+  for (int i = I0; i < CAP; i++)
+    if (i < n) {
+      const bool last = (i + 1 == n) || (i + 1 == CAP);
+      const double phi1 = last ? x[0] : x[i + 1 < CAP ? i + 1 : 0], lat1 = last ? y[0] : y[i + 1 < CAP ? i + 1 : 0];
+      area = d_area_edge(phi1, lat1, x[i], y[i], area);
+    }
+  return d_area_sign_scale(area);
 }
 
 template <int S>
@@ -199,67 +226,110 @@
   return d;
 }
 
-template <int S>
-__device__ inline void d_poly_area_ctr(const double *x, const double *y, int n, double clon,
-                                       double *area_out, double *ctrlon_out, double *ctrlat_out)
-{
-  double area = 0.0, ctrlat = 0.0, ctrlon = 0.0;
-  double s0, c0, cp_first;
-  fgs_trig<FGS_COS_F | FGS_SIN_N | FGS_COS_N>(y[0], nullptr, &cp_first, &s0, &c0);
-  const double f_first = 0.5 * (c0 * s0 + y[0]), dphi_first = d_dphi_clon(x[0], clon);
+__device__ __forceinline__ void d_ctr_vertex(double phi, double lat, double clon, double *f, double *dphi, double *cp)
+{
+  double s, c;
+  fgs_trig<FGS_COS_F | FGS_SIN_N | FGS_COS_N>(lat, nullptr, cp, &s, &c);
+  *f = 0.5 * (c * s + lat);
+  *dphi = d_dphi_clon(phi, clon);
+}
+
+__device__ __forceinline__ void d_area_ctr_edge(double phi1, double lat1, double phi2, double lat2, double f1, double dphi1, double cp1,
+                                                double f2, double dphi2, double &area, double &ctrlon, double &ctrlat)
+{
+  double dx0 = phi1 - phi2;
+  double avg_y = (lat1 + lat2) * 0.5;
+  double savg, cavg, sa, ca;
+  fgs_trig<FGS_ALL>(avg_y, &savg, &cavg, &sa, &ca);
+  double dyh = 0.5 * (lat1 - lat2);
+  bool flat = fabs(lat1 - lat2) < G_SMALL;
+  double dat = flat ? 1.0 : d_sin_lat(dyh) / dyh;
+
+  {
+    double dx = dx0;
+    if (dx > G_PI)  dx = dx - 2.0 * G_PI;
+    if (dx < -G_PI) dx = dx + 2.0 * G_PI;
+    if (fabs(dx + G_PI) < G_SMALL || fabs(dx - G_PI) < G_SMALL) area += G_PI;
+    else area -= dx * savg * dat;
+  }
+  if (dx0 != 0.0) {
+    double dx = dx0;
+    if (dx > G_PI)   dx = dx - 2.0 * G_PI;
+    if (dx <= -G_PI) dx = dx + 2.0 * G_PI;
+    double hdy = (lat2 - lat1) * 0.5;
+    const double t = (fabs(hdy) < G_SMALL) ? (2 * cavg + lat2 * savg) : dat * (2 * ca + lat2 * sa);
+    ctrlat -= dx * (t - cp1);
+  }
+  if (dx0 != 0.0) {
+    double dphi = dx0;
+    if (dphi > G_PI)  dphi = dphi - 2.0 * G_PI;
+    if (dphi < -G_PI) dphi = dphi + 2.0 * G_PI;
+    if (fabs(dphi2 - dphi1) < G_PI) {
+      ctrlon -= dphi * (dphi1 * f1 + dphi2 * f2) / 2.0;
+    } else {
+      double fac = (dphi1 > 0.0) ? G_PI : -G_PI;
+      double fint = f1 + (f2 - f1) * (fac - dphi1) / fabs(dphi);
+      ctrlon -= 0.5 * dphi1 * (dphi1 - fac) * f1 - 0.5 * dphi2 * (dphi2 + fac) * f2
+                + 0.5 * fac * (dphi1 + dphi2) * fint;
+    }
+  }
+}
+
+template <int S>
+__device__ inline void d_poly_area_ctr_edges(const double *x, const double *y, int n, double clon, int i0, int i1,
+                                             double *area_io, double *ctrlon_io, double *ctrlat_io)
+{
+  double area = *area_io, ctrlat = *ctrlat_io, ctrlon = *ctrlon_io;
+  double f_first, dphi_first, cp_first;
+  d_ctr_vertex(x[0], y[0], clon, &f_first, &dphi_first, &cp_first);
   double f2 = f_first, dphi2 = dphi_first;
-  for (int i = 0; i < n; i++) {
+  if (i0 > 0) { double cp; d_ctr_vertex(x[i0 * S], y[i0 * S], clon, &f2, &dphi2, &cp); }
+  for (int i = i0; i < i1; i++) {
     const bool last = (i + 1 == n);
     int ip = last ? 0 : i + 1;
     double phi1 = x[ip * S], phi2 = x[i * S];
     double lat1 = y[ip * S], lat2 = y[i * S];
     double f1, dphi1, cp1;
     if (last) { f1 = f_first; dphi1 = dphi_first; cp1 = cp_first; }
-    else {
-      double s1, c1;
-      fgs_trig<FGS_COS_F | FGS_SIN_N | FGS_COS_N>(lat1, nullptr, &cp1, &s1, &c1);
-      f1 = 0.5 * (c1 * s1 + lat1);
-      dphi1 = d_dphi_clon(phi1, clon);
-    }
-    double dx0 = phi1 - phi2;
-    double avg_y = (lat1 + lat2) * 0.5;
-    double savg, cavg, sa, ca;
-    fgs_trig<FGS_ALL>(avg_y, &savg, &cavg, &sa, &ca);
-    double dyh = 0.5 * (lat1 - lat2);
-    bool flat = fabs(lat1 - lat2) < G_SMALL;
-    double dat = flat ? 1.0 : d_sin_lat(dyh) / dyh;
-
-    {
-      double dx = dx0;
-      if (dx > G_PI)  dx = dx - 2.0 * G_PI;
-      if (dx < -G_PI) dx = dx + 2.0 * G_PI;
-      if (fabs(dx + G_PI) < G_SMALL || fabs(dx - G_PI) < G_SMALL) area += G_PI;
-      else area -= dx * savg * dat;
-    }
-    if (dx0 != 0.0) {
-      double dx = dx0;
-      if (dx > G_PI)   dx = dx - 2.0 * G_PI;
-      if (dx <= -G_PI) dx = dx + 2.0 * G_PI;
-      double hdy = (lat2 - lat1) * 0.5;
-      const double t = (fabs(hdy) < G_SMALL) ? (2 * cavg + lat2 * savg) : dat * (2 * ca + lat2 * sa);
-      ctrlat -= dx * (t - cp1);
-    }
-    if (dx0 != 0.0) {
-      double dphi = dx0;
-      if (dphi > G_PI)  dphi = dphi - 2.0 * G_PI;
-      if (dphi < -G_PI) dphi = dphi + 2.0 * G_PI;
-      if (fabs(dphi2 - dphi1) < G_PI) {
-        ctrlon -= dphi * (dphi1 * f1 + dphi2 * f2) / 2.0;
-      } else {
-        double fac = (dphi1 > 0.0) ? G_PI : -G_PI;
-        double fint = f1 + (f2 - f1) * (fac - dphi1) / fabs(dphi);
-        ctrlon -= 0.5 * dphi1 * (dphi1 - fac) * f1 - 0.5 * dphi2 * (dphi2 + fac) * f2
-                  + 0.5 * fac * (dphi1 + dphi2) * fint;
-      }
-    }
+    else d_ctr_vertex(phi1, lat1, clon, &f1, &dphi1, &cp1);
+    d_area_ctr_edge(phi1, lat1, phi2, lat2, f1, dphi1, cp1, f2, dphi2, area, ctrlon, ctrlat);
     f2 = f1; dphi2 = dphi1;
   }
-  *area_out = (area < 0) ? -area * G_RADIUS * G_RADIUS : area * G_RADIUS * G_RADIUS;
-  *ctrlat_out = ctrlat * G_RADIUS * G_RADIUS;
-  *ctrlon_out = ctrlon * G_RADIUS * G_RADIUS;
-}
+  if (i1 == n) {
+    *area_io = (area < 0) ? -area * G_RADIUS * G_RADIUS : area * G_RADIUS * G_RADIUS;
+    *ctrlat_io = ctrlat * G_RADIUS * G_RADIUS;
+    *ctrlon_io = ctrlon * G_RADIUS * G_RADIUS;
+  } else { *area_io = area; *ctrlat_io = ctrlat; *ctrlon_io = ctrlon; }
+}
+
+template <int S>
+__device__ inline void d_poly_area_ctr(const double *x, const double *y, int n, double clon,
+                                       double *area_out, double *ctrlon_out, double *ctrlat_out)
+{
+  *area_out = 0.0; *ctrlon_out = 0.0; *ctrlat_out = 0.0;
+  d_poly_area_ctr_edges<S>(x, y, n, clon, 0, n, area_out, ctrlon_out, ctrlat_out);
+}
+
+template <int I0, int CAP>
+__device__ __forceinline__ void d_poly_area_ctr_tail(const double *x, const double *y, int n, double clon,
+                                                     double *area_io, double *ctrlon_io, double *ctrlat_io)
+{
+  double area = *area_io, ctrlat = *ctrlat_io, ctrlon = *ctrlon_io;
+  double f_first, dphi_first, cp_first, f2, dphi2, cp;
+  d_ctr_vertex(x[0], y[0], clon, &f_first, &dphi_first, &cp_first);
+  d_ctr_vertex(x[I0], y[I0], clon, &f2, &dphi2, &cp);
+#pragma unroll
+  for (int i = I0; i < CAP; i++)
+    if (i < n) {
+      const bool last = (i + 1 == n) || (i + 1 == CAP);
+      const double phi1 = last ? x[0] : x[i + 1 < CAP ? i + 1 : 0], lat1 = last ? y[0] : y[i + 1 < CAP ? i + 1 : 0];
+      double f1, dphi1, cp1;
+      if (last) { f1 = f_first; dphi1 = dphi_first; cp1 = cp_first; }
+      else d_ctr_vertex(phi1, lat1, clon, &f1, &dphi1, &cp1);
+      d_area_ctr_edge(phi1, lat1, x[i], y[i], f1, dphi1, cp1, f2, dphi2, area, ctrlon, ctrlat);
+      f2 = f1; dphi2 = dphi1;
+    }
+  *area_io = (area < 0) ? -area * G_RADIUS * G_RADIUS : area * G_RADIUS * G_RADIUS;
+  *ctrlat_io = ctrlat * G_RADIUS * G_RADIUS;
+  *ctrlon_io = ctrlon * G_RADIUS * G_RADIUS;
+}
diff --git a/fre-nctools_amd/csrc/plan.hip b/fre-nctools_amd/csrc/plan.hip
--- a/fre-nctools_amd/csrc/plan.hip
+++ b/fre-nctools_amd/csrc/plan.hip
@@ -487,7 +487,7 @@
   double mean_dlat = 0, mean_dlon = 0;
   int rect_hint = 1;
 };
-struct SearchOpts { bool exact, cull, finalize, rect, dst_frame; int gc_split; bool profile, async; };
+struct SearchOpts { bool exact, cull, finalize, rect, dst_frame; int gc_split; bool profile, async; int tail_cap; };
 __global__ __launch_bounds__(64) void k_counters_out(const unsigned *src, unsigned *dst, int nwords, unsigned long long *mark, unsigned long long seq)
 {
   for (int k = threadIdx.x; k < nwords; k += 64) dst[k] = src[k];
@@ -533,6 +533,8 @@
 struct SearchCaps { unsigned long long entries; int regcap, nreg; bool rect; };
 static int g_search_rect = 1;
 extern "C" void fg_set_search_rect(int on) { g_search_rect = on ? 1 : 0; }
+static int g_clip_tail_cap = -1;
+extern "C" void fg_set_clip_tail_cap(int cap) { g_clip_tail_cap = cap < 0 ? -1 : cap; }
 static int g_dst_frame = 0;
 extern "C" void fg_set_search_frame(int coupler) { g_dst_frame = coupler ? 1 : 0; }
 static thread_local int tl_dst_frame = -1;
@@ -647,6 +649,7 @@
   const size_t z_bin_cnt = z((size_t)(nslots + 1) * sizeof(int)), z_bin_fill = z((size_t)(nslots + 1) * sizeof(int)),
                z_row_cnt = z((size_t)(ndst + 1) * sizeof(int)), z_nacc = z((size_t)(nsrc + 1) * sizeof(int));
   z((16 - (z.n - z_bin_cnt) % 16) % 16);
+  const size_t z_tails = z((gc || boxm) ? 0 : 2 * (size_t)CLIP_TAIL_NSEG * FG_FILL_STRIDE * sizeof(int));
   const size_t z_gc_ntask = z(gc ? zreg : 0), z_gc_ocnt = z(gc ? zreg : 0);
   const size_t zbytes = z.n;
   char *zero_blk = blk.get<char>(zbytes);
@@ -661,6 +664,15 @@
   double *tmp_clon = (order == 2) ? blk.get<double>(npairs + 1) : nullptr;
   double *tmp_clat = (order == 2) ? blk.get<double>(npairs + 1) : nullptr;
   int *defer_list = blk.get<int>(npairs + 1);
+  FgClipTails tails{};
+  if (!gc && !boxm) {
+    const long want = opt.tail_cap < 0 ? npairs / CLIP_TAIL_FRAC : std::min<long>(opt.tail_cap, npairs);
+    fgd_clip_tail_shape(std::min<long>(want, 0x7fffffffL / CLIP_TAIL_VROWS), &tails);
+  }
+  if (tails.cap > 0) {
+    tails.rec = blk.get<int4>((size_t)tails.cap + 1);
+    tails.v = blk.get<double2>(CLIP_TAIL_VROWS * ((size_t)tails.cap + 1));
+  }
   const bool early_rows = !gc && !boxm;
   int *tmp_rowpos = early_rows ? blk.get<int>(npairs + 1) : nullptr;
   const bool gc_split = gc && !gc_poly && opt.gc_split && npairs < (1L << 28);
@@ -682,6 +694,7 @@
   if (!pl->src_idx_f) pl->src_idx_f = blk.keep<int>(nsrc + 1);
   if (!blk.ok) return fg_fail(FG_ERR_HIP, "out of device memory");
   FgCounters *dc = (FgCounters *)(zero_blk + z_dc);
+  tails.cnt = (int *)(zero_blk + z_tails);
   ps.fill = (unsigned *)(zero_blk + z_fill);
   unsigned *tickets = (unsigned *)(zero_blk + z_tick);
   unsigned long long *lb_bins = (unsigned long long *)(zero_blk + z_lb_bins), *lb_rows = (unsigned long long *)(zero_blk + z_lb_rows),
@@ -767,7 +780,8 @@
   } else {
     pt.begin(PH_CLIP_QUAD);
     fgd_clip_quad(order, ps, pl->S, pl->mask_dev, pl->D, tmp_area, tmp_clon, tmp_clat, nacc, defer_list, &dc->defer_cnt, dc->stats, dc->err, st,
-                  rect ? &pl->rect_tab : nullptr, row_cnt, tmp_rowpos);
+                  rect ? &pl->rect_tab : nullptr, row_cnt, tmp_rowpos, tails);
+    fgd_clip_tails(order, tails, &dc->tail_cnt, ps, pl->S, pl->mask_dev, pl->D, tmp_area, tmp_clon, tmp_clat, nacc, dc->stats, st, row_cnt, tmp_rowpos);
     pt.end();
     pt.begin(PH_CLIP_GENERAL);
     fgd_clip_general(order, ps, pl->S, pl->mask_dev, pl->D, tmp_area, tmp_clon, tmp_clat, nacc, defer_list, &dc->defer_cnt, dc->stats, dc->err, st,
@@ -862,6 +876,7 @@
   pl->stats[FG_STAT_DEFERRED] = hc->defer_cnt + hc->gc_list2_cnt;
   pl->stats[FG_STAT_HEAVY] = hc->heavy_cnt;
   pl->stats[FG_STAT_RARE] = hc->rare_cnt;
+  pl->stats[FG_STAT_TAILS] = hc->tail_cnt;
   pl->stats[FG_STAT_BELOW] = (long)hc->stats[FG_STAT_BELOW];
 
   pl->rect_tab.bad = nullptr;
@@ -893,7 +908,7 @@
 {
   static const bool env_exact = getenv("FREGRID_HIP_EXACT_SEARCH") && atoi(getenv("FREGRID_HIP_EXACT_SEARCH")) != 0;
   const SearchOpts opt{.exact = g_search_exact || env_exact, .cull = g_search_cull != 0, .finalize = g_search_finalize != 0,
-                       .rect = g_search_rect != 0, .dst_frame = (tl_dst_frame >= 0 ? tl_dst_frame : g_dst_frame) != 0, .gc_split = g_gc_split, .profile = g_profiling != 0, .async = g_search_async != 0};
+                       .rect = g_search_rect != 0, .dst_frame = (tl_dst_frame >= 0 ? tl_dst_frame : g_dst_frame) != 0, .gc_split = g_gc_split, .profile = g_profiling != 0, .async = g_search_async != 0, .tail_cap = g_clip_tail_cap};
   const long big = std::max((long)pl->nsrc, (long)pl->ndst);
   if (big > (1L << 28)) return fg_fail(FG_ERR_CAPACITY, "grid of %ld cells: more than 2^28 cells per search are not supported", big);
   SearchCaps caps;
@@ -2833,8 +2848,8 @@
 
 extern "C" int fg_poly_op_batch(int op, int npoly, double *lon, double *lat, int *n, const double *clon, double *result)
 {
-  if (op < 0 || op > 6 || npoly < 0 || !lon || !lat || !n) return fg_fail(FG_ERR_ARG, "bad argument");
-  if ((op == 1 || op == 3 || op == 5) && !clon) return fg_fail(FG_ERR_ARG, "clon/tlon array required");
+  if (op < 0 || op > 14 || npoly < 0 || !lon || !lat || !n) return fg_fail(FG_ERR_ARG, "bad argument");
+  if ((op == 1 || op == 3 || op == 5 || op == 8 || op == 11) && !clon) return fg_fail(FG_ERR_ARG, "clon/tlon array required");
   if (op != 3 && !result) return fg_fail(FG_ERR_ARG, "result array required");
   if (npoly == 0) return 0;
   FGCHK(hipSetDevice(fg_env_device()));
diff --git a/fre-nctools_amd/csrc/poly_kernels.hip b/fre-nctools_amd/csrc/poly_kernels.hip
--- a/fre-nctools_amd/csrc/poly_kernels.hip
+++ b/fre-nctools_amd/csrc/poly_kernels.hip
@@ -84,7 +84,22 @@
   if (op == 0) result[p] = d_poly_area<1>(x, y, m);
   else if (op == 1) result[p] = d_poly_ctrlon<1>(x, y, m, clon[p]);
   else if (op == 2) result[p] = d_poly_ctrlat<1>(x, y, m);
-  else if (op >= 4) {
+  else if (op >= 13) {
+    const int h = m < 4 ? m : 4;
+    double pa = d_poly_area_edges<1>(x, y, m, 0, h, 0.0);
+    if (m > 4) pa = (op == 14 && m <= 8) ? d_poly_area_tail<4, 8>(x, y, m, pa) : d_poly_area_edges<1>(x, y, m, 4, m, pa);
+    result[p] = pa;
+  } else if (op >= 7) {
+    const int k = (op - 7) % 3, h = m < 4 ? m : 4;
+    const double cl = (k == 1) ? clon[p] : 0.0;
+    double pa = 0.0, pclon = 0.0, pclat = 0.0;
+    d_poly_area_ctr_edges<1>(x, y, m, cl, 0, h, &pa, &pclon, &pclat);
+    if (m > 4) {
+      if (op >= 10 && m <= 8) d_poly_area_ctr_tail<4, 8>(x, y, m, cl, &pa, &pclon, &pclat);
+      else d_poly_area_ctr_edges<1>(x, y, m, cl, 4, m, &pa, &pclon, &pclat);
+    }
+    result[p] = (k == 0) ? pa : (k == 1) ? pclon : pclat;
+  } else if (op >= 4) {
     double pa, pclon, pclat;
     d_poly_area_ctr<1>(x, y, m, op == 5 ? clon[p] : 0.0, &pa, &pclon, &pclat);
     result[p] = (op == 4) ? pa : (op == 5) ? pclon : pclat;
diff --git a/fre-nctools_amd/csrc/xgrid_device.h b/fre-nctools_amd/csrc/xgrid_device.h
--- a/fre-nctools_amd/csrc/xgrid_device.h
+++ b/fre-nctools_amd/csrc/xgrid_device.h
@@ -68,7 +68,8 @@
   FG_STAT_BELOW = 8,
   FG_STAT_EXACT = 9,
   FG_STAT_RARE = 10,
-  FG_NSTATS = 11
+  FG_STAT_TAILS = 11,
+  FG_NSTATS = 12
 };
 
 #define FG_REG_ALIGN 512
@@ -122,6 +123,7 @@
   int defer_cnt, big_cnt;
   int gc_list2_cnt;
   int rare_cnt;
+  int tail_cnt;
   unsigned long long stats[FG_NSTATS];
 };
 #define G_ERRBIT_LOOKBACK 128u
@@ -176,10 +178,32 @@
               double *tmp_area, double *tmp_clon, double *tmp_clat, int *nacc, int *defer_list, int *defer_cnt,
               unsigned long long *stats, unsigned *err, hipStream_t st, const FgRect *rect = nullptr, int *row_cnt = nullptr,
               int *tmp_rowpos = nullptr);
+#define CLIP_MAIN_EDGES 4
+#define CLIP_TAIL_ROWS 5
+#define CLIP_TAIL_VROWS (CLIP_TAIL_ROWS + 2)
+#define CLIP_TAIL_FRAC 4
+#define CLIP_TAIL_NSEG 64
+#define CLIP_TAIL_SEGMIN 1024
+struct FgClipTails {
+  int4 *rec;
+  double2 *v;
+  int *cnt;
+  int cap, segcap, segcap1, segmask;
+};
+static inline void fgd_clip_tail_shape(long want, FgClipTails *t)
+{
+  int nseg = 1;
+  while (2 * nseg <= CLIP_TAIL_NSEG && (long)(2 * nseg) * CLIP_TAIL_SEGMIN <= want) nseg *= 2;
+  const int w = (int)(want / nseg);
+  t->segcap1 = w / 4; t->segcap = w - t->segcap1; t->segmask = nseg - 1; t->cap = nseg * w;
+}
 void fgd_clip_quad(int order, FgPairSpace ps, FgCells S, const double *mask, FgCells D,
               double *tmp_area, double *tmp_clon, double *tmp_clat, int *nacc, int *defer_list, int *defer_cnt,
               unsigned long long *stats, unsigned *err, hipStream_t st, const FgRect *rect = nullptr, int *row_cnt = nullptr,
-              int *tmp_rowpos = nullptr);
+              int *tmp_rowpos = nullptr, FgClipTails tails = FgClipTails{});
+void fgd_clip_tails(int order, FgClipTails tails, int *total, FgPairSpace ps, FgCells S, const double *mask, FgCells D,
+              double *tmp_area, double *tmp_clon, double *tmp_clat, int *nacc, unsigned long long *stats, hipStream_t st,
+              int *row_cnt = nullptr, int *tmp_rowpos = nullptr);
 struct alignas(8) FgRowEnt { int n, s; };
 struct alignas(16) FgSrcRec { double cen_lon, cen_lat; };
 struct FgCompactIo {
diff --git a/fre-nctools_amd/csrc/xgrid_kernels.hip b/fre-nctools_amd/csrc/xgrid_kernels.hip
--- a/fre-nctools_amd/csrc/xgrid_kernels.hip
+++ b/fre-nctools_amd/csrc/xgrid_kernels.hip
@@ -1318,6 +1318,8 @@
 }
 
 struct ClipOut { double area, clon, clat; };
+__device__ __forceinline__ void d_pair_ratio(double pa, double clon, double clat, double maskv, double area_in, double area_out,
+                                             ClipOut *o, unsigned long long *stats);
 
 template <int ORDER, int S>
 __device__ __forceinline__ void d_finish_pair(const double *px, const double *py, int n_out, double maskv,
@@ -1327,6 +1329,12 @@
   double pa, clon = 0, clat = 0;
   if (ORDER == 2) d_poly_area_ctr<S>(px, py, n_out, lon_in_avg, &pa, &clon, &clat);
   else pa = d_poly_area<S>(px, py, n_out);
+  d_pair_ratio(pa, clon, clat, maskv, area_in, area_out, o, stats);
+}
+
+__device__ __forceinline__ void d_pair_ratio(double pa, double clon, double clat, double maskv, double area_in, double area_out,
+                                             ClipOut *o, unsigned long long *stats)
+{
   double xarea = pa * maskv;
   double min_area = (area_in < area_out) ? area_in : area_out;
   double ratio = xarea / min_area;
@@ -1493,13 +1501,28 @@
 #define CLIP_COMPACT 0
 #endif
 __device__ __forceinline__ int d_row_slot(int *row_cnt, bool take, int d, int lane);
+__device__ __forceinline__ void d_nacc_runs(int *nacc, int s, bool acc, int lane)
+{
+  if (!__ballot(s >= 0)) return;
+  const int s_prev = __shfl_up(s, 1, 64);
+  const bool head = (lane == 0) || (s != s_prev);
+  const unsigned long long hm = __ballot(head), am = __ballot(acc);
+  if (head && s >= 0) {
+    const unsigned long long above = (lane == 63) ? 0ull : (hm >> (lane + 1)) << (lane + 1);
+    const int end = above ? (__ffsll((long long)above) - 1) : 64;
+    const unsigned long long upto = (end == 64) ? ~0ull : ((1ull << end) - 1ull);
+    const int cnt = __popcll(am & upto & ~((1ull << lane) - 1ull));
+    if (cnt) atomicAdd(&nacc[s], cnt);
+  }
+}
 template <int ORDER, bool RECT, bool QSRC = false>
 __global__ __launch_bounds__(CLIP_THREADS) __attribute__((amdgpu_waves_per_eu(CLIP_WAVES, CLIP_WAVES))) void k_clip_quad(FgPairSpace ps, FgCells S, const double *mask, FgCells D, FgRect R,
                                                  double *tmp_area, double *tmp_clon, double *tmp_clat, int *nacc,
                                                  int *defer_list, int *defer_cnt,
-                                                 unsigned long long *stats, unsigned *err, int *row_cnt, int *tmp_rowpos)
+                                                 unsigned long long *stats, unsigned *err, int *row_cnt, int *tmp_rowpos, FgClipTails tl)
 {
   constexpr int T = CLIP_THREADS;
+  static_assert(CLIP_TAIL_ROWS == CLIP_SLOTS - CLIP_MAIN_EDGES + 1, "a tail record holds vertex 0 and the vertices from CLIP_MAIN_EDGES on");
   __shared__ double2 sh_poly[CLIP_SLOTS][T];
 #if CLIP_PAD_LDS
   __shared__ char sh_pad[CLIP_PAD_LDS];
@@ -1547,18 +1570,52 @@
   }
 #endif
   bool below = false, acc = false;
-  int s = -1, d_acc = -1;
+  int s = -1, d_acc = -1, d = -1;
+  const bool longp = n_cur > CLIP_MAIN_EDGES;
+  const bool cls1 = n_cur > CLIP_MAIN_EDGES + 1;
+  const unsigned long long tm1 = tl.cap ? __ballot(longp && cls1) : 0ull, tm0 = tl.cap ? __ballot(longp && !cls1) : 0ull, tm = tm0 | tm1;
+  const int tseg = blockIdx.x & tl.segmask;
+  int tq = 0;
+  if (tm && lane < 2) {
+    const unsigned long long m = lane ? tm1 : tm0;
+    if (m) tq = atomicAdd(&tl.cnt[((lane ? tl.segmask + 1 : 0) + tseg) * FG_FILL_STRIDE], __popcll(m));
+  }
+  double pa = 0, pclon = 0, pclat = 0, maskv = 1.0, area_in = 0, area_out = 0, lon_in_avg = 0;
+  const double *px = (const double *)&sh_poly[0][src];
   if (n_cur > 0) {
     const int p = p0 + src;
     s = CLIP_COMPACT ? ps.src[p] : s_in;
-    const int d = CLIP_COMPACT ? ps.dst[p] : d_in;
+    d = CLIP_COMPACT ? ps.dst[p] : d_in;
+    maskv = mask ? mask[s] : 1.0; area_in = S.area[s]; area_out = D.area[d]; lon_in_avg = S.lon_avg[s];
+    const int n_main = min(n_cur, CLIP_MAIN_EDGES);
+    if (ORDER == 2) d_poly_area_ctr_edges<2 * T>(px, px + 1, n_cur, lon_in_avg, 0, n_main, &pa, &pclon, &pclat);
+    else pa = d_poly_area_edges<2 * T>(px, px + 1, n_cur, 0, n_main, 0.0);
+  }
+  int tslot = -1;
+  if (tm) {
+    const int tq0 = __shfl(tq, 0), tq1 = __shfl(tq, 1);
+    tq = (cls1 ? tq1 : tq0) + __popcll((cls1 ? tm1 : tm0) & ((1ull << lane) - 1ull));
+    const int base = cls1 ? (tl.segmask + 1) * tl.segcap + tseg * tl.segcap1 : tseg * tl.segcap;
+    if (longp && tq < (cls1 ? tl.segcap1 : tl.segcap)) tslot = base + tq;
+  }
+  if (__ballot(longp && tslot < 0)) {
+    if (longp && tslot < 0) {
+      if (ORDER == 2) d_poly_area_ctr_edges<2 * T>(px, px + 1, n_cur, lon_in_avg, CLIP_MAIN_EDGES, n_cur, &pa, &pclon, &pclat);
+      else pa = d_poly_area_edges<2 * T>(px, px + 1, n_cur, CLIP_MAIN_EDGES, n_cur, pa);
+    }
+  }
+  if (tslot >= 0) {
+    tl.rec[tslot] = make_int4(p0 + src, n_cur, s, d);
+    tl.v[(size_t)CLIP_TAIL_ROWS * tl.cap + tslot] = make_double2(pa, pclon);
+    if (ORDER == 2) tl.v[(size_t)(CLIP_TAIL_ROWS + 1) * tl.cap + tslot] = make_double2(pclat, 0.0);
+    tl.v[tslot] = sh_poly[0][src];
+#pragma unroll
+    for (int k = CLIP_MAIN_EDGES; k < CLIP_SLOTS; k++)
+      if (k < n_cur) tl.v[(size_t)(k - CLIP_MAIN_EDGES + 1) * tl.cap + tslot] = sh_poly[k][src];
+  } else if (n_cur > 0) {
+    const int p = p0 + src;
     ClipOut o; o.area = -1.0; o.clon = 0; o.clat = 0;
-    const double *px = (const double *)&sh_poly[0][src];
-#if FG_EXP == 1
-    o.area = n_cur + px[0] + px[1];
-#else
-    d_finish_pair<ORDER, 2 * T>(px, px + 1, n_cur, mask ? mask[s] : 1.0, S.area[s], D.area[d], S.lon_avg[s], &o, stats);
-#endif
+    d_pair_ratio(pa, pclon, pclat, maskv, area_in, area_out, &o, stats);
     if (o.area >= 0) {
       acc = true;
       tmp_area[p] = o.area;
@@ -1573,18 +1630,7 @@
     const int slot = d_row_slot(row_cnt, acc, d_acc, lane);
     if (acc) tmp_rowpos[p0 + src] = slot;
   }
-  if (__ballot(s >= 0)) {
-    const int s_prev = __shfl_up(s, 1, 64);
-    const bool head = (lane == 0) || (s != s_prev);
-    const unsigned long long hm = __ballot(head), am = __ballot(acc);
-    if (head && s >= 0) {
-      const unsigned long long above = (lane == 63) ? 0ull : (hm >> (lane + 1)) << (lane + 1);
-      const int end = above ? (__ffsll((long long)above) - 1) : 64;
-      const unsigned long long upto = (end == 64) ? ~0ull : ((1ull << end) - 1ull);
-      const int cnt = __popcll(am & upto & ~((1ull << lane) - 1ull));
-      if (cnt) atomicAdd(&nacc[s], cnt);
-    }
-  }
+  d_nacc_runs(nacc, s, acc, lane);
   const unsigned long long dm = __ballot(defer), bm = __ballot(below);
   if (dm) {
     int q = 0;
@@ -1592,6 +1638,66 @@
     q = __shfl(q, 0);
     if (defer) defer_list[q + __popcll(dm & ((1ull << lane) - 1ull))] = p0 + tid;
   }
+  if (bm && lane == 0) atomicAdd(&stats[FG_STAT_BELOW], (unsigned long long)__popcll(bm));
+}
+
+#define TAIL_THREADS 256
+template <int ORDER>
+__global__ __launch_bounds__(TAIL_THREADS) void k_clip_tails(FgClipTails tl, int *total, int *pair_dst, FgCells S, const double *mask,
+                                                             const double *dst_area, double *tmp_area, double *tmp_clon, double *tmp_clat,
+                                                             int *nacc, unsigned long long *stats, int *row_cnt, int *tmp_rowpos)
+{
+  const int tid = threadIdx.x, lane = tid & 63;
+  const int nseg = tl.segmask + 1, nb0 = nseg * ((tl.segcap + TAIL_THREADS - 1) / TAIL_THREADS);
+  const int cls = (int)blockIdx.x >= nb0 ? 1 : 0, b = blockIdx.x - (cls ? nb0 : 0), sc = cls ? tl.segcap1 : tl.segcap;
+  const int bps = (sc + TAIL_THREADS - 1) / TAIL_THREADS;
+  const int seg = b / bps, q0 = (b - seg * bps) * TAIL_THREADS;
+  const int cnt = min(tl.cnt[(cls * nseg + seg) * FG_FILL_STRIDE], sc);
+  if (q0 == 0 && tid == 0 && cnt) atomicAdd(total, cnt);
+  if (q0 >= cnt) return;
+  d_load_trig_table();
+  const int q = (cls ? nseg * tl.segcap + seg * tl.segcap1 : seg * tl.segcap) + q0 + tid;
+  bool below = false, acc = false;
+  int s = -1, d_acc = -1, p = 0;
+  if (q0 + tid < cnt) {
+    const int4 rec = tl.rec[q];
+    p = rec.x; s = rec.z;
+    const int n = rec.y, d = rec.w;
+    double2 v[CLIP_TAIL_ROWS];
+    v[0] = tl.v[q];
+#pragma unroll
+    for (int k = 1; k < CLIP_TAIL_ROWS; k++)
+      v[k] = (k + CLIP_MAIN_EDGES - 1 < n) ? tl.v[(size_t)k * tl.cap + q] : make_double2(0.0, 0.0);
+    const double2 s0 = tl.v[(size_t)CLIP_TAIL_ROWS * tl.cap + q];
+    double pa = s0.x, pclon = s0.y, pclat = 0;
+    if (ORDER == 2) pclat = tl.v[(size_t)(CLIP_TAIL_ROWS + 1) * tl.cap + q].x;
+    const double maskv = mask ? mask[s] : 1.0, area_in = S.area[s], area_out = dst_area[d], lon_in_avg = S.lon_avg[s];
+    double x[CLIP_SLOTS], y[CLIP_SLOTS];
+#pragma unroll
+    for (int k = 0; k < CLIP_SLOTS; k++) { x[k] = 0.0; y[k] = 0.0; }
+    x[0] = v[0].x; y[0] = v[0].y;
+#pragma unroll
+    for (int k = 1; k < CLIP_TAIL_ROWS; k++) { x[k + CLIP_MAIN_EDGES - 1] = v[k].x; y[k + CLIP_MAIN_EDGES - 1] = v[k].y; }
+    if (ORDER == 2) d_poly_area_ctr_tail<CLIP_MAIN_EDGES, CLIP_SLOTS>(x, y, n, lon_in_avg, &pa, &pclon, &pclat);
+    else pa = d_poly_area_tail<CLIP_MAIN_EDGES, CLIP_SLOTS>(x, y, n, pa);
+    ClipOut o; o.area = -1.0; o.clon = 0; o.clat = 0;
+    d_pair_ratio(pa, pclon, pclat, maskv, area_in, area_out, &o, stats);
+    if (o.area >= 0) {
+      acc = true;
+      tmp_area[p] = o.area;
+      if (ORDER == 2) { tmp_clon[p] = o.clon; tmp_clat[p] = o.clat; }
+      d_acc = d;
+    } else {
+      pair_dst[p] = -1;
+      below = (o.area == -2.0);
+    }
+  }
+  if (row_cnt) {
+    const int slot = d_row_slot(row_cnt, acc, d_acc, lane);
+    if (acc) tmp_rowpos[p] = slot;
+  }
+  d_nacc_runs(nacc, s, acc, lane);
+  const unsigned long long bm = __ballot(below);
   if (bm && lane == 0) atomicAdd(&stats[FG_STAT_BELOW], (unsigned long long)__popcll(bm));
 }
 
@@ -2020,17 +2126,27 @@
 
 void fgd_clip_quad(int order, FgPairSpace ps, FgCells S, const double *mask, FgCells D,
                    double *tmp_area, double *tmp_clon, double *tmp_clat, int *nacc, int *defer_list, int *defer_cnt,
-                   unsigned long long *stats, unsigned *err, hipStream_t st, const FgRect *rect, int *row_cnt, int *tmp_rowpos)
+                   unsigned long long *stats, unsigned *err, hipStream_t st, const FgRect *rect, int *row_cnt, int *tmp_rowpos, FgClipTails tails)
 {
   const long np = fgd_pairs_total(ps);
   if (np <= 0) return;
   const FgRect R = rect ? *rect : FgRect{};
   const int g = nblk(np, CLIP_THREADS);
-#define FG_LAUNCH_QUAD(O, RC, QS) k_clip_quad<O, RC, QS><<<g, CLIP_THREADS, 0, st>>>(ps, S, mask, D, R, tmp_area, tmp_clon, tmp_clat, nacc, defer_list, defer_cnt, stats, err, row_cnt, tmp_rowpos)
+#define FG_LAUNCH_QUAD(O, RC, QS) k_clip_quad<O, RC, QS><<<g, CLIP_THREADS, 0, st>>>(ps, S, mask, D, R, tmp_area, tmp_clon, tmp_clat, nacc, defer_list, defer_cnt, stats, err, row_cnt, tmp_rowpos, tails)
   const bool qsrc = rect && S.vstride == FG_VSTRIDE_QUAD;
   if (order == 2) { if (qsrc) FG_LAUNCH_QUAD(2, true, true); else if (rect) FG_LAUNCH_QUAD(2, true, false); else FG_LAUNCH_QUAD(2, false, false); }
   else            { if (qsrc) FG_LAUNCH_QUAD(1, true, true); else if (rect) FG_LAUNCH_QUAD(1, true, false); else FG_LAUNCH_QUAD(1, false, false); }
 #undef FG_LAUNCH_QUAD
+}
+
+void fgd_clip_tails(int order, FgClipTails tails, int *total, FgPairSpace ps, FgCells S, const double *mask, FgCells D,
+                    double *tmp_area, double *tmp_clon, double *tmp_clat, int *nacc, unsigned long long *stats, hipStream_t st,
+                    int *row_cnt, int *tmp_rowpos)
+{
+  if (tails.cap <= 0) return;
+  const int g = (tails.segmask + 1) * (nblk(tails.segcap, TAIL_THREADS) + nblk(tails.segcap1, TAIL_THREADS));
+  if (order == 2) k_clip_tails<2><<<g, TAIL_THREADS, 0, st>>>(tails, total, ps.dst, S, mask, D.area, tmp_area, tmp_clon, tmp_clat, nacc, stats, row_cnt, tmp_rowpos);
+  else            k_clip_tails<1><<<g, TAIL_THREADS, 0, st>>>(tails, total, ps.dst, S, mask, D.area, tmp_area, tmp_clon, tmp_clat, nacc, stats, row_cnt, tmp_rowpos);
 }
 
 void fgd_clip_general(int order, FgPairSpace ps, FgCells S, const double *mask, FgCells D,
diff --git a/include/fregrid_hip.h b/include/fregrid_hip.h
--- a/include/fregrid_hip.h
+++ b/include/fregrid_hip.h
@@ -180,6 +180,7 @@
 void fg_set_search_finalize(int on);
 void fg_set_search_async(int on);
 void fg_set_search_rect(int on);
+void fg_set_clip_tail_cap(int cap);
 void fg_set_search_wide_cap(int n);
 void fg_set_search_frame(int coupler);
 void fg_set_apply_ep(int on);
```
